# HiLab-git/WSL4MIS

Hardware: AMD Instinct MI355X
Metric: training slices/sec (256x256, bs64, unet_cct pCE+GatedCRF) (higher is better)
Workload: dtype f32; 1 GPU; unet_cct pce_gatedcrf r=5, 256x256x1 4-class synthetic scribble slices, batch 64/GPU, SGD+poly LR; global_batch=64, parallelism=dp1, crf_radius=5, conv_precision=f32

## Files before the change

include/wsl_hip.h:

```cpp
#ifndef WSL_HIP_H
#define WSL_HIP_H
#include <stddef.h>
#include <stdint.h>

#ifdef __cplusplus
extern "C" {
#endif

#define WSL_OK 0
#define WSL_EINVAL (-1)
#define WSL_EUNSUPPORTED (-2)
#define WSL_EHIP (-3)
#define WSL_EWORKSPACE (-4)

#define WSL_LEAKY_SLOPE 0.01f

int wsl_version(void);
const char* wsl_last_error(void);
const char* wsl_build_info(void);

#define WSL_PROF_FAMILIES 20
typedef struct WslProfRow {
  char name[48];
  int64_t calls;
  double ms, flops, bytes;
  double issued_flops;
} WslProfRow;
int wsl_prof_enable(int on);
int wsl_prof_report(WslProfRow* rows, int max_rows);

typedef struct WslSrc {
  const float* x;
  int64_t bs;
  int32_t C;
  int32_t _pad0;
  const float* scale;
  const float* shift;
  const uint8_t* emask;
  float emask_scale;
  float _pad1;
  const float* cmask;
} WslSrc;

int wsl_conv2d_fwd(const WslSrc* a, const WslSrc* b, const float* w, const float* bias, float* y, int64_t y_bs,
                   int N, int H, int W, int Co, int ks, int wmode, float* stat_part, float* stat_cnt, void* stream);
int wsl_conv2d_stat_blocks(int N, int H, int W, int Ci, int Co, int ks);
int wsl_conv2d_pack_weights(const float* w, float* packed, int Co, int Ci, int ks, int wmode_raw, void* stream);
int wsl_conv2d_fast_ok(const WslSrc* a, const WslSrc* b, const float* y, int64_t y_bs, int W);
int wsl_conv2d_wino_ok(int N, int H, int W, int Ca, int Cb, int Co, int ks);
int wsl_net_concurrent(int on);

int wsl_conv2d_wgrad(const WslSrc* a, const WslSrc* b, const float* dy, int64_t dy_bs, float* dw, float* db,
                     int N, int H, int W, int Co, int ks, void* ws, size_t ws_bytes, void* stream);
size_t wsl_conv2d_wgrad_ws_bytes(int N, int H, int W, int Ci, int Co, int ks);
typedef struct WslWgradPending {
  const float* part_dw;
  const float* part_db;
  float* dw;
  float* db;
  int Co, Ci, KK, nsplit;
} WslWgradPending;
int wsl_conv2d_wgrad_partial(const WslSrc* a, const WslSrc* b, const float* dy, int64_t dy_bs, float* dw, float* db, int N, int H,
                             int W, int Co, int ks, void* ws, size_t ws_bytes, WslWgradPending* pending, void* stream);
int wsl_wgrad_reduce_batch(const WslWgradPending* items, int n, void* stream);

int wsl_bn_stats_finalize(const float* stat_part, const float* stat_cnt, int nblk, int C, const float* gamma,
                          const float* beta, float eps, float momentum, float* running_mean, float* running_var,
                          int64_t* num_batches_tracked, float* mean, float* invstd, float* scale, float* shift,
                          void* stream);
int wsl_bn_eval_affine(const float* gamma, const float* beta, const float* running_mean, const float* running_var,
                       float eps, int C, float* scale, float* shift, void* stream);
int wsl_src_materialize(const WslSrc* s, float* out, int64_t out_bs, int N, int H, int W, void* stream);
int wsl_pool2_fwd(const WslSrc* s, float* out, int N, int H, int W, void* stream);

int wsl_feat_grad_combine(const WslSrc* f, const float* ga, int64_t ga_bs, const float* gb, int64_t gb_bs,
                          const float* gb_cmask, const float* gp, float* g, int N, int H, int W, void* stream);

int wsl_bnact_bwd(const float* g, int64_t g_bs, const float* y, const float* mean, const float* invstd,
                  const float* gamma, const float* beta, const uint8_t* emask, float emask_scale, float* dy,
                  float* dgamma, float* dbeta, int N, int C, int H, int W, void* ws, size_t ws_bytes, void* stream);
size_t wsl_bnact_bwd_ws_bytes(int N, int C, int H, int W);

int wsl_conv2d_dgrad_bn(const WslSrc* dy, const float* w, float* g, int64_t g_bs, int N, int H, int W, int Co, int ks,
                        int wmode, const float* bn_y, const float* bn_st, const uint8_t* bn_emask, float bn_emask_scale,
                        float* bn_part, int* fused, void* stream);
int wsl_feat_grad_combine_blocks(int N, int H, int W);
int wsl_feat_grad_combine_bn(const WslSrc* f, const float* ga, int64_t ga_bs, const float* gb, int64_t gb_bs,
                             const float* gb_cmask, const float* gp, float* g, int N, int H, int W, const float* bn_mean,
                             const float* bn_invstd, float* bn_part, void* stream);
int wsl_bnact_bwd_finish(const float* g, int64_t g_bs, const float* y, const float* mean, const float* invstd,
                         const float* gamma, const float* beta, const uint8_t* emask, float emask_scale, float* dy,
                         float* dgamma, float* dbeta, int N, int C, int H, int W, const float* part, int nblk,
                         int channel_major, void* ws, size_t ws_bytes, void* stream);
int wsl_conv2d_dgrad_bn_d(const WslSrc* dy, const float* w, float* g, int64_t g_bs, int N, int H, int W, int Co, int ks,
                          int wmode, const float* bn_y, const float* bn_st, const uint8_t* bn_emask, float bn_emask_scale,
                          float* bn_part, int* fused, void* stream);
int wsl_bnact_bwd_finish_d_amax(const float* dz, int64_t dz_bs, const float* y, const float* mean, const float* invstd,
                                const float* gamma, const float* beta, float* dy, float* dgamma, float* dbeta, int N, int C, int H,
                                int W, const float* part, int nblk, int channel_major, void* ws, size_t ws_bytes, uint32_t* dy_amax,
                                void* stream);

#define WSL_SP_ACT_EXP 4
#define WSL_SP_AMAX_SLOTS 64
int wsl_sp_conv2d_ok(const WslSrc* a, const WslSrc* b, const float* y, int64_t y_bs, int N, int H, int W, int Co, int ks);
size_t wsl_sp_weight_image_bytes(int Co, int Ci);
int wsl_sp_pack_weights(const float* w, void* image, uint32_t* w_amax, int Co, int Ci, int dgrad, void* stream);
int wsl_sp_conv2d_fwd(const WslSrc* a, const WslSrc* b, const void* image, const uint32_t* w_amax, const uint32_t* in_amax,
                      const float* bias, float* y, int64_t y_bs, int N, int H, int W, int Co, float* stat_part, float* stat_cnt,
                      void* stream);
int wsl_sp_conv2d_stat_blocks(int N, int H, int W, int Ci, int Co);
int wsl_sp_conv2d_dgrad_bn(const WslSrc* dy, const uint32_t* dy_amax, const void* image, const uint32_t* w_amax, float* g,
                           int64_t g_bs, int N, int H, int W, int Co, const float* bn_y, const float* bn_st,
                           const uint8_t* bn_emask, float bn_emask_scale, float* bn_part, int* fused, void* stream);
size_t wsl_sp_conv2d_wgrad_ws_bytes(int N, int H, int W, int Ci, int Co);
int wsl_sp_conv2d_wgrad_partial(const WslSrc* a, const WslSrc* b, const float* dy, int64_t dy_bs, const uint32_t* dy_amax,
                                float* dw, float* db, int N, int H, int W, int Co, void* ws, size_t ws_bytes,
                                WslWgradPending* pending, void* stream);
size_t wsl_bilinear_up2_fwd_amax_ws_bytes(int N, int C, int h, int w);
int wsl_bilinear_up2_fwd_amax(const float* u, float* out, int64_t out_bs, int N, int C, int h, int w, void* ws, size_t ws_bytes,
                              uint32_t* amax_slots, void* stream);
int wsl_sp_conv2d_wgrad_partial_amax(const WslSrc* a, const WslSrc* b, const float* dy, int64_t dy_bs, const uint32_t* dy_amax,
                                     const uint32_t* in_amax, float* dw, float* db, int N, int H, int W, int Co, void* ws,
                                     size_t ws_bytes, WslWgradPending* pending, void* stream);
size_t wsl_bnact_bwd_finish_ws_bytes(int N, int C, int H, int W, int with_amax);
int wsl_bnact_bwd_amax(const float* g, int64_t g_bs, const float* y, const float* mean, const float* invstd, const float* gamma,
                       const float* beta, const uint8_t* emask, float emask_scale, float* dy, float* dgamma, float* dbeta, int N,
                       int C, int H, int W, void* ws, size_t ws_bytes, uint32_t* dy_amax, void* stream);
int wsl_bnact_bwd_finish_amax(const float* g, int64_t g_bs, const float* y, const float* mean, const float* invstd,
                              const float* gamma, const float* beta, const uint8_t* emask, float emask_scale, float* dy,
                              float* dgamma, float* dbeta, int N, int C, int H, int W, const float* part, int nblk,
                              int channel_major, void* ws, size_t ws_bytes, uint32_t* dy_amax, void* stream);

int wsl_bilinear_up2_fwd(const float* u, float* out, int64_t out_bs, int N, int C, int h, int w, void* stream);
int wsl_bilinear_up2_bwd(const float* dout, int64_t dout_bs, float* du, int N, int C, int h, int w, void* stream);

int wsl_softmax_fwd(const float* z, float* s, int N, int C, int HW, void* stream);
int wsl_softmax_bwd(const float* s, const float* ds, float* dz, int N, int C, int HW, void* stream);

int wsl_ce_fwd_bwd(const float* z, const void* label, int label_i64, int ignore, float* loss, float* dz, float gscale,
                   int N, int C, int HW, void* ws, size_t ws_bytes, void* stream);
int wsl_mix_argmax(const float* s1, const float* s2, double beta, int64_t* pseudo, int N, int C, int HW, void* stream);
int wsl_pdice_fwd(const float* s, const void* target, int target_i64, int ignore, float* loss, float* sums, int N,
                  int C, int HW, void* ws, size_t ws_bytes, void* stream);
int wsl_pdice_bwd(const float* s, const void* target, int target_i64, int ignore, const float* sums,
                  const float* gout , float* ds, int N, int C, int HW, void* stream);

int wsl_head_fwd_bwd(const float* z1, const float* z2, const uint8_t* label, int ignore, double beta, float w_pse,
                     float gscale, float* out, int64_t* pseudo, float* dz1, float* dz2, int N, int C, int HW,
                     void* ws, size_t ws_bytes, void* stream);
size_t wsl_loss_ws_bytes(int N, int C, int HW);
int wsl_head_gatedcrf_fwd_bwd(const float* z1, const float* z2, const uint8_t* label, int ignore, double beta, const float* img,
                              int radius, float sigma_xy, float sigma_rgb, float weight, float crf_weight, float* out,
                              float* dz1, float* dz2, float* y, float* msg, int N, int C, int H, int W, void* ws,
                              size_t ws_bytes, void* stream);

int wsl_mixprob_fwd(const float* z1, const float* z2, double beta, float* y, int N, int C, int HW, void* stream);
int wsl_mixprob_bwd(const float* z1, const float* z2, double beta, const float* dy, float k, float* dz1, float* dz2,
                    int accumulate, int N, int C, int HW, void* stream);

int wsl_gatedcrf_fwd(const float* y, const float* img, float* msg, float* loss, int N, int C, int H, int W, int radius,
                     float sigma_xy, float sigma_rgb, float weight, void* ws, size_t ws_bytes, void* stream);
int wsl_gatedcrf_bwd(const float* msg, const float* gout, float gscale, float* dy, int N, int C, int H, int W,
                     void* stream);
#define WSL_REG_TV 1
#define WSL_REG_MS 2
#define WSL_REG_ENTROPY 3
#define WSL_REG_CLASS_VAR 4
int wsl_head_reg_fwd_bwd(const float* z, const uint8_t* label, int ignore, float w_ce, int reg_kind, float reg_weight,
                         const float* img, const float* zt, float cons_weight, float* out, float* dz, float* s, float* ds, int N,
                         int C, int H, int W, void* ws, size_t ws_bytes, void* stream);
int wsl_tv_fwd_bwd(const float* p, int n0, float* loss, float* dp, float gscale, int N, int C, int H, int W, void* ws,
                   size_t ws_bytes, void* stream);
int wsl_mumford_shah_fwd_bwd(const float* img, const float* p, float* loss, float* dp, float gscale, int N, int C, int H,
                             int W, void* ws, size_t ws_bytes, void* stream);
int wsl_class_variance_fwd_bwd(const float* img, const float* p, float* loss ,
                               float* dp, float w_inter, float w_intra, int N, int C, int H, int W,
                               void* ws, size_t ws_bytes, void* stream);
int wsl_softmax_mse_fwd_bwd(const float* a, const float* b, float* loss, float* da, float gscale, int N, int C, int HW,
                            void* ws, size_t ws_bytes, void* stream);

int wsl_rot90(const float* x, float* y, int planes, int H, int W, int k, void* stream);
int wsl_softmax_accum(const float* z, float* acc, float scale, int init, int N, int C, int HW, void* stream);
int wsl_ustm_consistency_fwd_bwd(const float* a, const float* b, const float* pmean, float threshold, float* loss, float* da,
                                 float gscale, int N, int C, int HW, void* ws, size_t ws_bytes, void* stream);
int wsl_entropy_fwd_bwd(const float* p, float* loss, float* dp, float gscale, int N, int C, int HW, int norm_classes,
                        void* ws, size_t ws_bytes, void* stream);
int wsl_axpy(float* dst, const float* src, float k, int64_t n, void* stream);

int wsl_sup_head_fwd_bwd(const float* z, const uint8_t* label, int ignore, float w_ce, float w_dice, float gscale, float* out,
                         float* dz, int N, int C, int HW, void* ws, size_t ws_bytes, void* stream);
int wsl_entropy_logits_fwd_bwd(const float* z, float* loss, float* dz, float gscale, int N, int C, int HW, int norm_classes,
                               void* ws, size_t ws_bytes, void* stream);

int wsl_sgd_step(float* p, const float* grad, float* buf, int64_t n, float lr, float momentum, float wd, int first,
                 float grad_scale, float* ema, float ema_alpha, void* stream);

typedef struct {
  const float* img;
  const uint8_t* lab;
  int h, w;
  int op, k, axis;
  int lab_cval;
  float img_cval;
  double m00, m01, m10, m11, off0, off1;
} WslAugSample;
int wsl_augment_batch(const WslAugSample* samples, int n, float* out_img, uint8_t* out_lab, int Ho, int Wo, void* stream);

size_t wsl_s2l_head_ws_bytes(int N, int C, int HW);
int wsl_s2l_head_fwd_bwd(const float* z, const uint8_t* scribble, const float* weight, int ignore, float thr_conf, float w_u,
                         float gscale, float* out, uint8_t* u_labels, float* dz, int N, int C, int HW, void* ws, size_t ws_bytes,
                         void* stream);
typedef struct WslS2lSlot {
  float* weight;
  int h, w;
} WslS2lSlot;
int wsl_s2l_ensemble_update(const float* z, const WslS2lSlot* slots, int n, int C, int Hn, int Wn, double alpha, void* stream);
typedef struct {
  const float* img;
  const uint8_t* mask;
  const uint8_t* scr;
  const float* weight;
  int h, w;
  int op, k, axis;
  int _pad;
  double m00, m01, m10, m11, off0, off1;
} WslAugSampleS2l;
int wsl_augment_batch_s2l(const WslAugSampleS2l* samples, int n, int C, float* out_img, uint8_t* out_mask, uint8_t* out_scr,
                          float* out_weight, int Ho, int Wo, void* stream);

size_t wsl_random_walker_ws_bytes(int N, int H, int W, int n_class);
int wsl_random_walker(const float* img, const uint8_t* seed, uint8_t* label_out, float* prob_out, int* iters_out, float* resid_out,
                      int N, int H, int W, int n_class, float beta, float tol, int max_iter, void* ws, size_t ws_bytes, void* stream);

int wsl_surface_u8(const uint8_t* vol, uint8_t* border, int D, int H, int W, void* stream);
int wsl_nearest_dist2(const int64_t* a_zyx, int na, const int64_t* b_zyx, int nb, int64_t* out, void* stream);

int wsl_nearest_dist2_sp(const int64_t* a_zyx, int na, const int64_t* b_zyx, int nb, double sz, double sy, double sx, double* out,
                         void* stream);

int wsl_noisy_copy(const float* x, const float* noise, float* out, int64_t n, int reps, float sigma, float clip, uint64_t seed,
                   void* stream);

int wsl_draw_masks(int n_masks, void* const* outs, const int64_t* numels, const float* keep_probs, const float* scales,
                   const int* is_f32, uint64_t seed, void* stream);

typedef struct WslNetDesc {
  int32_t in_chns, n_class;
  int32_t n_dec;
  int32_t N, H, W;
  int32_t precision;
  int32_t _pad;
} WslNetDesc;

typedef struct WslNetEntry {
  char name[96];
  int32_t kind;
  int32_t ndim;
  int64_t shape[4];
  int64_t offset;
} WslNetEntry;

int wsl_net_num_entries(const WslNetDesc* d);
int wsl_net_entry(const WslNetDesc* d, int i, WslNetEntry* out);
int64_t wsl_net_param_count(const WslNetDesc* d);
int64_t wsl_net_encoder_param_count(const WslNetDesc* d);
int64_t wsl_net_buffer_count(const WslNetDesc* d);
size_t wsl_net_ws_bytes(const WslNetDesc* d);

int wsl_net_forward(const WslNetDesc* d, const float* params, float* buffers, int64_t* nbt, const float* x,
                    const uint8_t* const* emasks, const float* const* cmasks, int training, float* logits_main,
                    float* logits_aux, void* ws, size_t ws_bytes, void* stream);
int wsl_net_backward(const WslNetDesc* d, const float* params, const float* x, const uint8_t* const* emasks,
                     const float* const* cmasks, const float* dlogits_main, const float* dlogits_aux, float* grads,
                     void* ws, size_t ws_bytes, int phase, void* stream);

int wsl_conv2d_dil_fwd(const WslSrc* a, const WslSrc* b, const float* w, const float* bias, float* y, int64_t y_bs, int N, int H,
                       int W, int Co, int ks, int dil, int wmode, float* stat_part, float* stat_cnt, void* stream);
int wsl_conv2d_dil_stat_blocks(int N, int H, int W, int Ci, int Co, int dil);
int wsl_conv2d_dil_wgrad(const WslSrc* a, const WslSrc* b, const float* dy, int64_t dy_bs, float* dw, float* db, int N, int H, int W,
                         int Co, int ks, int dil, void* ws, size_t ws_bytes, void* stream);
size_t wsl_conv2d_dil_wgrad_ws_bytes(int N, int H, int W, int Ci, int Co, int ks, int dil);
int wsl_conv2d_dil_wgrad_partial(const WslSrc* a, const WslSrc* b, const float* dy, int64_t dy_bs, float* dw, float* db, int N, int H,
                                 int W, int Co, int ks, int dil, void* ws, size_t ws_bytes, WslWgradPending* pending, void* stream);

typedef struct WslPNetDesc {
// ... 69 lines not shown
```

wsl4mis_amd/_lib.py:

```python
import ctypes as C
import os

import torch

_HERE = os.path.dirname(os.path.abspath(__file__))
LIB_PATH = os.path.join(_HERE, "csrc", "libwslhip.so")

c_fp = C.c_void_p


class WslSrc(C.Structure):
    _fields_ = [("x", c_fp), ("bs", C.c_int64), ("C", C.c_int32), ("_pad0", C.c_int32), ("scale", c_fp),
                ("shift", c_fp), ("emask", c_fp), ("emask_scale", C.c_float), ("_pad1", C.c_float), ("cmask", c_fp)]


WSL_PROF_FAMILIES = 20


class WslProfRow(C.Structure):
    _fields_ = [("name", C.c_char * 48), ("calls", C.c_int64), ("ms", C.c_double), ("flops", C.c_double),
                ("bytes", C.c_double), ("issued_flops", C.c_double)]


class WslNetDesc(C.Structure):
    _fields_ = [("in_chns", C.c_int32), ("n_class", C.c_int32), ("n_dec", C.c_int32), ("N", C.c_int32),
                ("H", C.c_int32), ("W", C.c_int32), ("precision", C.c_int32), ("_pad", C.c_int32)]


class WslWgradPending(C.Structure):
    _fields_ = [("part_dw", c_fp), ("part_db", c_fp), ("dw", c_fp), ("db", c_fp), ("Co", C.c_int32), ("Ci", C.c_int32),
                ("KK", C.c_int32), ("nsplit", C.c_int32)]


class WslUpBlockDesc(C.Structure):
    _fields_ = [("C1", C.c_int32), ("C2", C.c_int32), ("Co", C.c_int32), ("N", C.c_int32), ("h", C.c_int32), ("w", C.c_int32),
                ("dropout_p", C.c_float)]


class WslPNetDesc(C.Structure):
    _fields_ = [("in_chns", C.c_int32), ("n_class", C.c_int32), ("num_filters", C.c_int32), ("ratios", C.c_int32 * 5),
                ("N", C.c_int32), ("H", C.c_int32), ("W", C.c_int32)]


class WslDanDesc(C.Structure):
    _fields_ = [("num_classes", C.c_int32), ("n_channel", C.c_int32), ("ndf", C.c_int32), ("pool", C.c_int32),
                ("N", C.c_int32), ("H", C.c_int32), ("W", C.c_int32), ("_pad", C.c_int32)]


class WslNetEntry(C.Structure):
    _fields_ = [("name", C.c_char * 96), ("kind", C.c_int32), ("ndim", C.c_int32), ("shape", C.c_int64 * 4),
                ("offset", C.c_int64)]


class WslAugSample(C.Structure):
    _fields_ = [("img", c_fp), ("lab", c_fp), ("h", C.c_int32), ("w", C.c_int32), ("op", C.c_int32), ("k", C.c_int32),
                ("axis", C.c_int32), ("lab_cval", C.c_int32), ("img_cval", C.c_float), ("m00", C.c_double),
                ("m01", C.c_double), ("m10", C.c_double), ("m11", C.c_double), ("off0", C.c_double), ("off1", C.c_double)]


class WslS2lSlot(C.Structure):
    _fields_ = [("weight", c_fp), ("h", C.c_int32), ("w", C.c_int32)]


class WslAugSampleS2l(C.Structure):
    _fields_ = [("img", c_fp), ("mask", c_fp), ("scr", c_fp), ("weight", c_fp), ("h", C.c_int32), ("w", C.c_int32),
                ("op", C.c_int32), ("k", C.c_int32), ("axis", C.c_int32), ("_pad", C.c_int32), ("m00", C.c_double),
                ("m01", C.c_double), ("m10", C.c_double), ("m11", C.c_double), ("off0", C.c_double), ("off1", C.c_double)]


i32, i64, f32, f64, sz = C.c_int, C.c_int64, C.c_float, C.c_double, C.c_size_t
PS, PD, PE = C.POINTER(WslSrc), C.POINTER(WslNetDesc), C.POINTER(WslNetEntry)
PP = C.POINTER(c_fp)
PQ = C.POINTER(WslPNetDesc)
PDAN = C.POINTER(WslDanDesc)

_PROTOS = {
    "wsl_version": (i32, []),
    "wsl_last_error": (C.c_char_p, []),
    "wsl_build_info": (C.c_char_p, []),
    "wsl_prof_enable": (i32, [i32]),
    "wsl_prof_report": (i32, [C.POINTER(WslProfRow), i32]),
    "wsl_net_concurrent": (i32, [i32]),
    "wsl_conv2d_fwd": (i32, [PS, PS, c_fp, c_fp, c_fp, i64, i32, i32, i32, i32, i32, i32, c_fp, c_fp, c_fp]),
    "wsl_conv2d_stat_blocks": (i32, [i32, i32, i32, i32, i32, i32]),
    "wsl_conv2d_pack_weights": (i32, [c_fp, c_fp, i32, i32, i32, i32, c_fp]),
    "wsl_conv2d_fast_ok": (i32, [PS, PS, c_fp, i64, i32]),
    "wsl_conv2d_wino_ok": (i32, [i32, i32, i32, i32, i32, i32, i32]),
    "wsl_conv2d_wgrad": (i32, [PS, PS, c_fp, i64, c_fp, c_fp, i32, i32, i32, i32, i32, c_fp, sz, c_fp]),
    "wsl_conv2d_wgrad_ws_bytes": (sz, [i32, i32, i32, i32, i32, i32]),
    "wsl_conv2d_wgrad_partial": (i32, [PS, PS, c_fp, i64, c_fp, c_fp, i32, i32, i32, i32, i32, c_fp, sz,
                                       C.POINTER(WslWgradPending), c_fp]),
    "wsl_wgrad_reduce_batch": (i32, [C.POINTER(WslWgradPending), i32, c_fp]),
    "wsl_bn_stats_finalize": (i32, [c_fp, c_fp, i32, i32, c_fp, c_fp, f32, f32, c_fp, c_fp, c_fp, c_fp, c_fp, c_fp,
                                    c_fp, c_fp]),
    "wsl_bn_eval_affine": (i32, [c_fp, c_fp, c_fp, c_fp, f32, i32, c_fp, c_fp, c_fp]),
    "wsl_src_materialize": (i32, [PS, c_fp, i64, i32, i32, i32, c_fp]),
    "wsl_pool2_fwd": (i32, [PS, c_fp, i32, i32, i32, c_fp]),
    "wsl_feat_grad_combine": (i32, [PS, c_fp, i64, c_fp, i64, c_fp, c_fp, c_fp, i32, i32, i32, c_fp]),
    "wsl_bnact_bwd": (i32, [c_fp, i64, c_fp, c_fp, c_fp, c_fp, c_fp, c_fp, f32, c_fp, c_fp, c_fp, i32, i32, i32, i32,
                            c_fp, sz, c_fp]),
    "wsl_bnact_bwd_ws_bytes": (sz, [i32, i32, i32, i32]),
    "wsl_conv2d_dgrad_bn": (i32, [PS, c_fp, c_fp, i64, i32, i32, i32, i32, i32, i32, c_fp, c_fp, c_fp, f32, c_fp, C.POINTER(C.c_int), c_fp]),
    "wsl_conv2d_dgrad_bn_d": (i32, [PS, c_fp, c_fp, i64, i32, i32, i32, i32, i32, i32, c_fp, c_fp, c_fp, f32, c_fp, C.POINTER(C.c_int), c_fp]),
    "wsl_bnact_bwd_finish_d_amax": (i32, [c_fp, i64, c_fp, c_fp, c_fp, c_fp, c_fp, c_fp, c_fp, c_fp, i32, i32, i32, i32,
                                          c_fp, i32, i32, c_fp, sz, c_fp, c_fp]),
    "wsl_feat_grad_combine_blocks": (i32, [i32, i32, i32]),
    "wsl_feat_grad_combine_bn": (i32, [PS, c_fp, i64, c_fp, i64, c_fp, c_fp, c_fp, i32, i32, i32, c_fp, c_fp, c_fp, c_fp]),
    "wsl_bnact_bwd_finish": (i32, [c_fp, i64, c_fp, c_fp, c_fp, c_fp, c_fp, c_fp, f32, c_fp, c_fp, c_fp, i32, i32, i32, i32,
                                   c_fp, i32, i32, c_fp, sz, c_fp]),
    "wsl_sp_conv2d_ok": (i32, [PS, PS, c_fp, i64, i32, i32, i32, i32, i32]),
    "wsl_sp_weight_image_bytes": (sz, [i32, i32]),
    "wsl_sp_pack_weights": (i32, [c_fp, c_fp, c_fp, i32, i32, i32, c_fp]),
    "wsl_sp_conv2d_fwd": (i32, [PS, PS, c_fp, c_fp, c_fp, c_fp, c_fp, i64, i32, i32, i32, i32, c_fp, c_fp, c_fp]),
    "wsl_sp_conv2d_stat_blocks": (i32, [i32, i32, i32, i32, i32]),
    "wsl_sp_conv2d_dgrad_bn": (i32, [PS, c_fp, c_fp, c_fp, c_fp, i64, i32, i32, i32, i32, c_fp, c_fp, c_fp, f32, c_fp,
                                     C.POINTER(C.c_int), c_fp]),
    "wsl_sp_conv2d_wgrad_ws_bytes": (sz, [i32, i32, i32, i32, i32]),
    "wsl_sp_conv2d_wgrad_partial": (i32, [PS, PS, c_fp, i64, c_fp, c_fp, c_fp, i32, i32, i32, i32, c_fp, sz,
                                          C.POINTER(WslWgradPending), c_fp]),
    "wsl_sp_conv2d_wgrad_partial_amax": (i32, [PS, PS, c_fp, i64, c_fp, c_fp, c_fp, c_fp, i32, i32, i32, i32, c_fp, sz,
                                               C.POINTER(WslWgradPending), c_fp]),
    "wsl_bilinear_up2_fwd_amax_ws_bytes": (sz, [i32, i32, i32, i32]),
    "wsl_bilinear_up2_fwd_amax": (i32, [c_fp, c_fp, i64, i32, i32, i32, i32, c_fp, sz, c_fp, c_fp]),
    "wsl_bnact_bwd_finish_ws_bytes": (sz, [i32, i32, i32, i32, i32]),
    "wsl_bnact_bwd_amax": (i32, [c_fp, i64, c_fp, c_fp, c_fp, c_fp, c_fp, c_fp, f32, c_fp, c_fp, c_fp, i32, i32, i32, i32,
                                 c_fp, sz, c_fp, c_fp]),
    "wsl_bnact_bwd_finish_amax": (i32, [c_fp, i64, c_fp, c_fp, c_fp, c_fp, c_fp, c_fp, f32, c_fp, c_fp, c_fp, i32, i32, i32, i32,
                                        c_fp, i32, i32, c_fp, sz, c_fp, c_fp]),
    "wsl_bilinear_up2_fwd": (i32, [c_fp, c_fp, i64, i32, i32, i32, i32, c_fp]),
    "wsl_bilinear_up2_bwd": (i32, [c_fp, i64, c_fp, i32, i32, i32, i32, c_fp]),
    "wsl_softmax_fwd": (i32, [c_fp, c_fp, i32, i32, i32, c_fp]),
    "wsl_softmax_bwd": (i32, [c_fp, c_fp, c_fp, i32, i32, i32, c_fp]),
    "wsl_ce_fwd_bwd": (i32, [c_fp, c_fp, i32, i32, c_fp, c_fp, f32, i32, i32, i32, c_fp, sz, c_fp]),
    "wsl_mix_argmax": (i32, [c_fp, c_fp, f64, c_fp, i32, i32, i32, c_fp]),
    "wsl_pdice_fwd": (i32, [c_fp, c_fp, i32, i32, c_fp, c_fp, i32, i32, i32, c_fp, sz, c_fp]),
    "wsl_pdice_bwd": (i32, [c_fp, c_fp, i32, i32, c_fp, c_fp, c_fp, i32, i32, i32, c_fp]),
    "wsl_head_fwd_bwd": (i32, [c_fp, c_fp, c_fp, i32, f64, f32, f32, c_fp, c_fp, c_fp, c_fp, i32, i32, i32, c_fp, sz,
                               c_fp]),
    "wsl_loss_ws_bytes": (sz, [i32, i32, i32]),
    "wsl_mixprob_fwd": (i32, [c_fp, c_fp, f64, c_fp, i32, i32, i32, c_fp]),
    "wsl_mixprob_bwd": (i32, [c_fp, c_fp, f64, c_fp, f32, c_fp, c_fp, i32, i32, i32, i32, c_fp]),
    "wsl_gatedcrf_fwd": (i32, [c_fp, c_fp, c_fp, c_fp, i32, i32, i32, i32, i32, f32, f32, f32, c_fp, sz, c_fp]),
    "wsl_gatedcrf_bwd": (i32, [c_fp, c_fp, f32, c_fp, i32, i32, i32, i32, c_fp]),
    "wsl_head_reg_fwd_bwd": (i32, [c_fp, c_fp, i32, f32, i32, f32, c_fp, c_fp, f32, c_fp, c_fp, c_fp, c_fp, i32, i32, i32, i32, c_fp, sz, c_fp]),
    "wsl_tv_fwd_bwd": (i32, [c_fp, i32, c_fp, c_fp, f32, i32, i32, i32, i32, c_fp, sz, c_fp]),
    "wsl_mumford_shah_fwd_bwd": (i32, [c_fp, c_fp, c_fp, c_fp, f32, i32, i32, i32, i32, c_fp, sz, c_fp]),
    "wsl_class_variance_fwd_bwd": (i32, [c_fp, c_fp, c_fp, c_fp, f32, f32, i32, i32, i32, i32, c_fp, sz, c_fp]),
    "wsl_softmax_mse_fwd_bwd": (i32, [c_fp, c_fp, c_fp, c_fp, f32, i32, i32, i32, c_fp, sz, c_fp]),
    "wsl_rot90": (i32, [c_fp, c_fp, i32, i32, i32, i32, c_fp]),
    "wsl_softmax_accum": (i32, [c_fp, c_fp, f32, i32, i32, i32, i32, c_fp]),
    "wsl_ustm_consistency_fwd_bwd": (i32, [c_fp, c_fp, c_fp, f32, c_fp, c_fp, f32, i32, i32, i32, c_fp, sz, c_fp]),
    "wsl_entropy_fwd_bwd": (i32, [c_fp, c_fp, c_fp, f32, i32, i32, i32, i32, c_fp, sz, c_fp]),
    "wsl_axpy": (i32, [c_fp, c_fp, f32, i64, c_fp]),
    "wsl_sup_head_fwd_bwd": (i32, [c_fp, c_fp, i32, f32, f32, f32, c_fp, c_fp, i32, i32, i32, c_fp, sz, c_fp]),
    "wsl_entropy_logits_fwd_bwd": (i32, [c_fp, c_fp, c_fp, f32, i32, i32, i32, i32, c_fp, sz, c_fp]),
    "wsl_sgd_step": (i32, [c_fp, c_fp, c_fp, i64, f32, f32, f32, i32, f32, c_fp, f32, c_fp]),
    "wsl_surface_u8": (i32, [c_fp, c_fp, i32, i32, i32, c_fp]),
    "wsl_nearest_dist2": (i32, [c_fp, i32, c_fp, i32, c_fp, c_fp]),
    "wsl_nearest_dist2_sp": (i32, [c_fp, i32, c_fp, i32, f64, f64, f64, c_fp, c_fp]),
    "wsl_augment_batch": (i32, [C.POINTER(WslAugSample), i32, c_fp, c_fp, i32, i32, c_fp]),
    "wsl_s2l_head_ws_bytes": (sz, [i32, i32, i32]),
    "wsl_s2l_head_fwd_bwd": (i32, [c_fp, c_fp, c_fp, i32, f32, f32, f32, c_fp, c_fp, c_fp, i32, i32, i32, c_fp, sz, c_fp]),
    "wsl_s2l_ensemble_update": (i32, [c_fp, C.POINTER(WslS2lSlot), i32, i32, i32, i32, f64, c_fp]),
    "wsl_augment_batch_s2l": (i32, [C.POINTER(WslAugSampleS2l), i32, i32, c_fp, c_fp, c_fp, c_fp, i32, i32, c_fp]),
    "wsl_random_walker_ws_bytes": (sz, [i32, i32, i32, i32]),
    "wsl_random_walker": (i32, [c_fp, c_fp, c_fp, c_fp, c_fp, c_fp, i32, i32, i32, i32, f32, f32, i32, c_fp, sz, c_fp]),
    "wsl_noisy_copy": (i32, [c_fp, c_fp, c_fp, i64, i32, f32, f32, C.c_uint64, c_fp]),
    "wsl_head_gatedcrf_fwd_bwd": (i32, [c_fp, c_fp, c_fp, i32, f64, c_fp, i32, f32, f32, f32, f32, c_fp, c_fp, c_fp, c_fp, c_fp,
                                        i32, i32, i32, i32, c_fp, sz, c_fp]),
    "wsl_draw_masks": (i32, [i32, PP, C.POINTER(C.c_int64), C.POINTER(C.c_float), C.POINTER(C.c_float),
                             C.POINTER(C.c_int), C.c_uint64, c_fp]),
    "wsl_convt2x2_fwd": (i32, [c_fp, c_fp, c_fp, c_fp, i32, i32, i32, i32, i32, c_fp]),
    "wsl_convt2x2_dgrad": (i32, [c_fp, i64, c_fp, c_fp, i32, i32, i32, i32, i32, c_fp]),
    "wsl_convt2x2_wgrad_ws_bytes": (sz, [i32, i32, i32]),
    "wsl_convt2x2_wgrad": (i32, [c_fp, c_fp, i64, c_fp, c_fp, i32, i32, i32, i32, i32, c_fp, sz, c_fp]),
    "wsl_upblock_t_param_count": (i64, [C.POINTER(WslUpBlockDesc)]),
    "wsl_upblock_t_ws_bytes": (sz, [C.POINTER(WslUpBlockDesc)]),
    "wsl_upblock_t_forward": (i32, [C.POINTER(WslUpBlockDesc), c_fp, c_fp, c_fp, c_fp, c_fp, c_fp, i32, c_fp, c_fp, sz, c_fp]),
    "wsl_upblock_t_backward": (i32, [C.POINTER(WslUpBlockDesc), c_fp, c_fp, c_fp, c_fp, c_fp, c_fp, c_fp, c_fp, c_fp, sz, c_fp]),
    "wsl_conv2d_dil_fwd": (i32, [PS, PS, c_fp, c_fp, c_fp, i64, i32, i32, i32, i32, i32, i32, i32, c_fp, c_fp, c_fp]),
    "wsl_conv2d_dil_stat_blocks": (i32, [i32, i32, i32, i32, i32, i32]),
    "wsl_conv2d_dil_wgrad": (i32, [PS, PS, c_fp, i64, c_fp, c_fp, i32, i32, i32, i32, i32, i32, c_fp, sz, c_fp]),
    "wsl_conv2d_dil_wgrad_ws_bytes": (sz, [i32, i32, i32, i32, i32, i32, i32]),
    "wsl_conv2d_dil_wgrad_partial": (i32, [PS, PS, c_fp, i64, c_fp, c_fp, i32, i32, i32, i32, i32, i32, c_fp, sz,
                                           C.POINTER(WslWgradPending), c_fp]),
    "wsl_pnet_num_entries": (i32, [PQ]),
    "wsl_pnet_entry": (i32, [PQ, i32, PE]),
    "wsl_pnet_param_count": (i64, [PQ]),
    "wsl_pnet_block_param_count": (i64, [PQ]),
    "wsl_pnet_buffer_count": (i64, [PQ]),
    "wsl_pnet_ws_bytes": (sz, [PQ]),
    "wsl_pnet_forward": (i32, [PQ, c_fp, c_fp, c_fp, c_fp, PP, i32, c_fp, c_fp, sz, c_fp]),
    "wsl_pnet_backward": (i32, [PQ, c_fp, c_fp, PP, c_fp, c_fp, c_fp, sz, i32, c_fp]),
    "wsl_conv4s2_fwd": (i32, [c_fp, i32, c_fp, i32, i32, c_fp, c_fp, c_fp, c_fp, c_fp, c_fp, i32, i32, i32, i32, c_fp]),
    "wsl_conv4s2_dgrad": (i32, [c_fp, c_fp, c_fp, c_fp, c_fp, i32, i32, i32, i32, i32, c_fp]),
    "wsl_conv4s2_wgrad_ws_bytes": (sz, [i32, i32, i32, i32, i32]),
    "wsl_conv4s2_wgrad": (i32, [c_fp, i32, c_fp, c_fp, c_fp, c_fp, c_fp, c_fp, i32, i32, i32, i32, i32, c_fp, sz, c_fp]),
    "wsl_dan_head_ws_bytes": (sz, [i32, i32]),
    "wsl_dan_head_fwd_bwd": (i32, [c_fp, c_fp, c_fp, c_fp, i32, f32, c_fp, c_fp, c_fp, c_fp, c_fp, i32, i32, i32, i32, c_fp, sz, c_fp]),
    "wsl_adam_step": (i32, [c_fp, c_fp, c_fp, c_fp, i64, f32, f32, f32, f32, i32, f32, c_fp]),
    "wsl_dan_num_entries": (i32, [PDAN]),
    "wsl_dan_entry": (i32, [PDAN, i32, PE]),
    "wsl_dan_param_count": (i64, [PDAN]),
    "wsl_dan_buffer_count": (i64, [PDAN]),
    "wsl_dan_ws_bytes": (sz, [PDAN]),
    "wsl_dan_forward": (i32, [PDAN, c_fp, c_fp, c_fp, PP, i32, c_fp, f32, c_fp, c_fp, c_fp, sz, c_fp]),
    "wsl_dan_backward": (i32, [PDAN, c_fp, c_fp, c_fp, PP, c_fp, i32, c_fp, c_fp, c_fp, sz, c_fp]),
    "wsl_net_num_entries": (i32, [PD]),
    "wsl_net_entry": (i32, [PD, i32, PE]),
    "wsl_net_param_count": (i64, [PD]),
    "wsl_net_encoder_param_count": (i64, [PD]),
    "wsl_net_buffer_count": (i64, [PD]),
    "wsl_net_ws_bytes": (sz, [PD]),
    "wsl_net_forward": (i32, [PD, c_fp, c_fp, c_fp, c_fp, PP, PP, i32, c_fp, c_fp, c_fp, sz, c_fp]),
    "wsl_net_backward": (i32, [PD, c_fp, c_fp, PP, PP, c_fp, c_fp, c_fp, c_fp, sz, i32, c_fp]),
}


_DEBUG_PROTOS = {
    "wsl_debug_conv_plan": (i32, [i32, i32, i32]),
    "wsl_debug_conv_wino": (i32, [i32]),
    "wsl_debug_wgrad_workgroups": (i32, [i32]),
    "wsl_debug_net_decisions": (i32, [PD, c_fp, sz, i32, i32, c_fp, c_fp]),
    "wsl_debug_mfma4_probe": (i32, [c_fp, c_fp, c_fp, c_fp]),
    "wsl_debug_lds_dma_probe": (i32, [c_fp, c_fp, c_fp]),
    "wsl_debug_pk_probe": (i32, [c_fp, c_fp, c_fp]),
    "wsl_debug_mfma_stream": (i32, [i32, i32, i32, c_fp, c_fp]),
}


class WslError(RuntimeError):
    pass


def bind(cdll, strict=True):
    missing = []
    for name, (res, args) in _PROTOS.items():
        try:
            fn = getattr(cdll, name)
        except AttributeError:
            missing.append(name)
            continue
        fn.restype, fn.argtypes = res, args
    for name, (res, args) in _DEBUG_PROTOS.items():
        if hasattr(cdll, name):
            fn = getattr(cdll, name)
            fn.restype, fn.argtypes = res, args
    if missing and strict:
        raise WslError(f"library lacks symbols declared in include/wsl_hip.h: {missing}")
    return missing


_lib = None


def lib():
    global _lib
    if _lib is None:
        if not os.path.exists(LIB_PATH):
            raise WslError(f"{LIB_PATH} not found: run wsl4mis_amd/csrc/build.sh (hipcc, gfx950). "
                           "There is no CPU fallback.")
        cdll = C.CDLL(LIB_PATH)
        bind(cdll, strict=os.path.abspath(LIB_PATH) == os.path.join(_HERE, "csrc", "libwslhip.so"))
        if b"HOST-EMULATION" in cdll.wsl_build_info():
            raise WslError("refusing to use a host-emulation build as the product library")
        _lib = cdll
    return _lib


_test_emul = False


def use_library_for_tests(cdll):
    global _lib, _test_emul
    bind(cdll, strict=False)
    if b"HOST-EMULATION" not in cdll.wsl_build_info():
        raise WslError("use_library_for_tests expects the emulation build")
    _lib, _test_emul = cdll, True


def _reset_for_tests():
    global _lib, _test_emul
    _lib, _test_emul = None, False


def is_test_emulation():
    return _test_emul


def check(rc, cdll=None):
    if rc != 0:
        l = cdll or lib()
        raise WslError(f"wsl error {rc}: {l.wsl_last_error().decode()}")


def source_sha256():
    import hashlib
    cs = os.path.join(_HERE, "csrc")
    names = sorted(f for f in os.listdir(cs) if f.endswith((".hip", ".h")))
    h = hashlib.sha256()
    for f in [os.path.join(cs, n) for n in names] + [os.path.join(os.path.dirname(_HERE), "include", "wsl_hip.h")]:
        with open(f, "rb") as fh:
            h.update(fh.read())
    return h.hexdigest()


def library_sha256(cdll=None):
    info = (cdll or lib()).wsl_build_info().decode()
    return info.rsplit("sha256:", 1)[1].strip() if "sha256:" in info else None


def declared_symbols():
    return list(_PROTOS)
```

wsl4mis_amd/csrc/wsl_bn.hip:

```cpp
#include <stdlib.h>

#include "wsl_rt.h"

namespace wsl {

constexpr int kChunk = 4096;

constexpr int kFinalizeWideFrom = 2048;
static inline int finalize_threads(int nblk) { return nblk >= kFinalizeWideFrom ? 1024 : kThreads; }
template <int NV>
__device__ __forceinline__ void finalize_merge_waves(double (&v)[NV], double* red) {
  const int nw = blockDim.x >> 6, w = threadIdx.x >> 6;
#pragma unroll
  for (int m = 32; m >= 1; m >>= 1)
#pragma unroll
    for (int k = 0; k < NV; ++k) v[k] += __shfl_xor(v[k], m);
  if ((threadIdx.x & 63) == 0)
#pragma unroll
    for (int k = 0; k < NV; ++k) red[k * 16 + w] = v[k];
  __syncthreads();
#pragma unroll
  for (int k = 0; k < NV; ++k) {
    double t[16];
#pragma unroll
// ... 216 lines not shown
    float* dst = bn_part + (((int64_t)n * gridDim.x + blockIdx.x) * f.C + c) * 2;
    dst[0] = s1;
    dst[1] = s2;
  }
}

struct BnBwdP {
  const float* g;
  int64_t g_bs;
  const float* y;
  const float* mean;
  const float* invstd;
  const float* gamma;
  const float* beta;
  const uint8_t* emask;
  float es;
  int C, HW, chunks;
  int g_is_d = 0;
};

__device__ __forceinline__ float bn_dz(const BnBwdP& p, int n, int c, int i, float sc, float sh, float mean, float invstd,
                                       float* xhat) {
  const int64_t idx = ((int64_t)n * p.C + c) * p.HW + i;
  const float yv = p.y[idx];
  float d = p.g[n * p.g_bs + (int64_t)c * p.HW + i];
  *xhat = (yv - mean) * invstd;
  if (p.g_is_d) return d;
  if (p.emask) d = p.emask[idx] ? d * p.es : 0.f;
  const float z = fmaf(yv, sc, sh);
  return z > 0.f ? d : WSL_LEAKY_SLOPE * d;
}

__global__ __launch_bounds__(256) void bnact_bwd_reduce_kernel(BnBwdP p, float* part) {
  __shared__ float red[8];
  const int c = blockIdx.y, n = blockIdx.z;
  const float mean = p.mean[c], invstd = p.invstd[c];
  const float sc = p.gamma[c] * invstd, sh = fmaf(-mean, sc, p.beta[c]);
  float s1 = 0.f, s2 = 0.f;
  const int base = blockIdx.x * kChunk;
  for (int i = base + threadIdx.x; i < base + kChunk && i < p.HW; i += kThreads) {
    float xh;
    const float d = bn_dz(p, n, c, i, sc, sh, mean, invstd, &xh);
    s1 += d;
    s2 = fmaf(d, xh, s2);
  }
  s1 = block_sum(s1, red);
  s2 = block_sum(s2, red + 4);
  if (threadIdx.x == 0) {
    float* dst = part + (((int64_t)n * p.chunks + blockIdx.x) * p.C + c) * 2;
    dst[0] = s1;
    dst[1] = s2;
  }
}

__device__ __forceinline__ void bn_dz4(const BnBwdP& p, int n, int c, int i, float sc, float sh, float mean, float invstd,
                                       float (&d)[4], float (&xh)[4]) {
  const int64_t idx = ((int64_t)n * p.C + c) * p.HW + i;
  const float4 yv = *reinterpret_cast<const float4*>(p.y + idx);
  const float4 gv = *reinterpret_cast<const float4*>(p.g + n * p.g_bs + (int64_t)c * p.HW + i);
  const float y4[4] = {yv.x, yv.y, yv.z, yv.w};
  float g4[4] = {gv.x, gv.y, gv.z, gv.w};
  if (p.g_is_d) {
#pragma unroll
    for (int k = 0; k < 4; ++k) xh[k] = (y4[k] - mean) * invstd, d[k] = g4[k];
    return;
  }
  if (p.emask) {
    const uint32_t m = *reinterpret_cast<const uint32_t*>(p.emask + idx);
#pragma unroll
    for (int k = 0; k < 4; ++k) g4[k] = ((m >> (8 * k)) & 0xffu) ? g4[k] * p.es : 0.f;
  }
#pragma unroll
  for (int k = 0; k < 4; ++k) {
    const float z = fmaf(y4[k], sc, sh);
    xh[k] = (y4[k] - mean) * invstd;
    d[k] = z > 0.f ? g4[k] : WSL_LEAKY_SLOPE * g4[k];
  }
}

__global__ __launch_bounds__(256) void bnact_bwd_reduce4_kernel(BnBwdP p, float* part) {
  __shared__ float red[8];
  const int c = blockIdx.y, n = blockIdx.z;
  const float mean = p.mean[c], invstd = p.invstd[c];
  const float sc = p.gamma[c] * invstd, sh = fmaf(-mean, sc, p.beta[c]);
  float s1 = 0.f, s2 = 0.f;
  const int base = blockIdx.x * kChunk;
  for (int i = base + 4 * threadIdx.x; i < base + kChunk && i < p.HW; i += 4 * kThreads) {
    float d[4], xh[4];
    bn_dz4(p, n, c, i, sc, sh, mean, invstd, d, xh);
#pragma unroll
    for (int k = 0; k < 4; ++k) {
      s1 += d[k];
      s2 = fmaf(d[k], xh[k], s2);
    }
  }
  s1 = block_sum(s1, red);
  s2 = block_sum(s2, red + 4);
  if (threadIdx.x == 0) {
    float* dst = part + (((int64_t)n * p.chunks + blockIdx.x) * p.C + c) * 2;
    dst[0] = s1;
    dst[1] = s2;
  }
}

__device__ __forceinline__ void amax_block_store(float m, uint32_t* pmax) {
  __shared__ float mred[4];
#pragma unroll
  for (int k = 32; k >= 1; k >>= 1) m = fmaxf(m, __shfl_xor(m, k));
  if ((threadIdx.x & 63) == 0) mred[threadIdx.x >> 6] = m;
  __syncthreads();
  if (threadIdx.x == 0) {
    m = fmaxf(fmaxf(mred[0], mred[1]), fmaxf(mred[2], mred[3]));
    uint32_t u;
    memcpy(&u, &m, 4);
    pmax[((int64_t)blockIdx.z * gridDim.y + blockIdx.y) * gridDim.x + blockIdx.x] = u;
  }
}
__global__ __launch_bounds__(256) void amax_fold_kernel(const uint32_t* pmax, int n, uint32_t* slots) {
  __shared__ uint32_t ured[4];
  uint32_t u = 0u;
  for (int i = blockIdx.x + WSL_SP_AMAX_SLOTS * threadIdx.x; i < n; i += WSL_SP_AMAX_SLOTS * kThreads) {
    const uint32_t v = pmax[i];
    u = v > u ? v : u;
  }
#pragma unroll
  for (int k = 32; k >= 1; k >>= 1) {
    const uint32_t o = (uint32_t)__shfl_xor((int)u, k);
    u = o > u ? o : u;
  }
  if ((threadIdx.x & 63) == 0) ured[threadIdx.x >> 6] = u;
  __syncthreads();
  if (threadIdx.x == 0) {
    const uint32_t a = ured[0] > ured[1] ? ured[0] : ured[1], b = ured[2] > ured[3] ? ured[2] : ured[3];
    slots[blockIdx.x] = a > b ? a : b;
  }
}

__global__ __launch_bounds__(256) void bnact_bwd_apply4_kernel(BnBwdP p, const float* coef, float* dy, uint32_t* pmax) {
  const int c = blockIdx.y, n = blockIdx.z;
  const float mean = p.mean[c], invstd = p.invstd[c];
  const float sc = p.gamma[c] * invstd, sh = fmaf(-mean, sc, p.beta[c]);
  const float c1 = coef[2 * c], c2 = coef[2 * c + 1];
  const int base = blockIdx.x * kChunk;
  float m = 0.f;
  for (int i = base + 4 * threadIdx.x; i < base + kChunk && i < p.HW; i += 4 * kThreads) {
    float d[4], xh[4];
    bn_dz4(p, n, c, i, sc, sh, mean, invstd, d, xh);
    const float4 v = make_float4(sc * (d[0] - c1 - xh[0] * c2), sc * (d[1] - c1 - xh[1] * c2), sc * (d[2] - c1 - xh[2] * c2),
                                 sc * (d[3] - c1 - xh[3] * c2));
    *reinterpret_cast<float4*>(dy + ((int64_t)n * p.C + c) * p.HW + i) = v;
    if (pmax) m = fmaxf(fmaxf(m, fmaxf(fabsf(v.x), fabsf(v.y))), fmaxf(fabsf(v.z), fabsf(v.w)));
  }
  if (pmax) amax_block_store(m, pmax);
}

__global__ __launch_bounds__(1024) void bnact_bwd_finalize_kernel(const float* part, int nblk, int C, int64_t sb, int64_t sc,
                                                                  double count, float* dgamma, float* dbeta, float* coef) {
  __shared__ double red[2 * 16];
  const int c = blockIdx.x;
  double acc[2] = {0, 0};
#pragma unroll 8
  for (int b = threadIdx.x; b < nblk; b += blockDim.x) {
    const float2 v = *reinterpret_cast<const float2*>(part + ((int64_t)b * sb + (int64_t)c * sc) * 2);
    acc[0] += v.x;
    acc[1] += v.y;
  }
  finalize_merge_waves<2>(acc, red);
  const double s1 = acc[0], s2 = acc[1];
  if (threadIdx.x == 0) {
    if (dbeta) dbeta[c] = (float)s1;
    if (dgamma) dgamma[c] = (float)s2;
    coef[2 * c] = (float)(s1 / count);
    coef[2 * c + 1] = (float)(s2 / count);
  }
}

__global__ __launch_bounds__(256) void bnact_bwd_apply_kernel(BnBwdP p, const float* coef, float* dy, uint32_t* pmax) {
  const int c = blockIdx.y, n = blockIdx.z;
  const float mean = p.mean[c], invstd = p.invstd[c];
  const float sc = p.gamma[c] * invstd, sh = fmaf(-mean, sc, p.beta[c]);
  const float c1 = coef[2 * c], c2 = coef[2 * c + 1];
  const int base = blockIdx.x * kChunk;
  float m = 0.f;
  for (int i = base + threadIdx.x; i < base + kChunk && i < p.HW; i += kThreads) {
    float xh;
    const float d = bn_dz(p, n, c, i, sc, sh, mean, invstd, &xh);
    const float v = sc * (d - c1 - xh * c2);
    dy[((int64_t)n * p.C + c) * p.HW + i] = v;
    m = fmaxf(m, fabsf(v));
  }
  if (pmax) amax_block_store(m, pmax);
}

__device__ __forceinline__ void lerp_coord(int dst, float scale, int in, int* i0, int* i1, float* l) {
  const float src = scale * (float)dst;
  int a = (int)src;
  if (a > in - 1) a = in - 1;
  *i0 = a;
  *i1 = a + (a < in - 1 ? 1 : 0);
  *l = src - (float)a;
}

__global__ __launch_bounds__(256) void bilinear_up2_fwd_kernel(const float* u, float* out, int64_t out_bs, int C, int h,
                                                               int w) {
  const int c = blockIdx.y, n = blockIdx.z, Ho = 2 * h, Wo = 2 * w;
  const float sy = Ho > 1 ? (float)(h - 1) / (float)(Ho - 1) : 0.f, sx = Wo > 1 ? (float)(w - 1) / (float)(Wo - 1) : 0.f;
  const float* src = u + ((int64_t)n * C + c) * h * w;
  const int base = blockIdx.x * kChunk;
  for (int o = base + threadIdx.x; o < base + kChunk && o < Ho * Wo; o += kThreads) {
    const int oy = o / Wo, ox = o - oy * Wo;
    int y0, y1, x0, x1;
    float ly, lx;
    lerp_coord(oy, sy, h, &y0, &y1, &ly);
    lerp_coord(ox, sx, w, &x0, &x1, &lx);
    const float top = (1.f - lx) * src[y0 * w + x0] + lx * src[y0 * w + x1];
    const float bot = (1.f - lx) * src[y1 * w + x0] + lx * src[y1 * w + x1];
    out[n * out_bs + (int64_t)c * Ho * Wo + o] = (1.f - ly) * top + ly * bot;
  }
}

__global__ __launch_bounds__(256) void bilinear_up2_bwd_kernel(const float* dout, int64_t dout_bs, float* du, int C,
                                                               int h, int w) {
  const int c = blockIdx.y, n = blockIdx.z, Ho = 2 * h, Wo = 2 * w;
  const float sy = Ho > 1 ? (float)(h - 1) / (float)(Ho - 1) : 0.f, sx = Wo > 1 ? (float)(w - 1) / (float)(Wo - 1) : 0.f;
  const float* g = dout + n * dout_bs + (int64_t)c * Ho * Wo;
  const int base = blockIdx.x * kChunk;
  for (int e = base + threadIdx.x; e < base + kChunk && e < h * w; e += kThreads) {
    const int i = e / w, j = e - i * w;
    float wy[5], wx[5];
#pragma unroll
    for (int k = 0; k < 5; ++k) {
      const int Y = 2 * i - 2 + k, X = 2 * j - 2 + k;
      wy[k] = 0.f, wx[k] = 0.f;
      if (Y >= 0 && Y < Ho) {
        int a, b;
        float l;
        lerp_coord(Y, sy, h, &a, &b, &l);
        wy[k] = (a == i ? 1.f - l : 0.f) + (b == i ? l : 0.f);
      }
      if (X >= 0 && X < Wo) {
        int a, b;
        float l;
        lerp_coord(X, sx, w, &a, &b, &l);
        wx[k] = (a == j ? 1.f - l : 0.f) + (b == j ? l : 0.f);
      }
    }
    float acc = 0.f;
#pragma unroll
    for (int ky = 0; ky < 5; ++ky) {
      if (wy[ky] != 0.f) {
        const int Y = 2 * i - 2 + ky;
        float row = 0.f;
#pragma unroll
        for (int kx = 0; kx < 5; ++kx)
          if (wx[kx] != 0.f) row = fmaf(wx[kx], g[(int64_t)Y * Wo + 2 * j - 2 + kx], row);
        acc = fmaf(wy[ky], row, acc);
      }
    }
    du[((int64_t)n * C + c) * h * w + e] = acc;
  }
}

__global__ __launch_bounds__(256) void bilinear_up2_fwdc_kernel(const float* u, float* out, int64_t out_bs, int C, int h,
                                                                int w, int lw, int rows_per_wg) {
  const int c = blockIdx.y, n = blockIdx.z, Ho = 2 * h, Wo = 2 * w;
  const float sy = Ho > 1 ? (float)(h - 1) / (float)(Ho - 1) : 0.f, sx = Wo > 1 ? (float)(w - 1) / (float)(Wo - 1) : 0.f;
  const float* src = u + ((int64_t)n * C + c) * h * w;
  float* dst = out + n * out_bs + (int64_t)c * Ho * Wo;
  const int ox = threadIdx.x & (Wo - 1), r0 = threadIdx.x >> lw, rgroups = kThreads >> lw;
  int x0, x1;
  float lx;
  lerp_coord(ox, sx, w, &x0, &x1, &lx);
  const int per = (rows_per_wg + rgroups - 1) / rgroups;
  const int base = blockIdx.x * rows_per_wg + r0 * per;
  int end = base + per;
  if (end > blockIdx.x * rows_per_wg + rows_per_wg) end = blockIdx.x * rows_per_wg + rows_per_wg;
  if (end > Ho) end = Ho;
  int ya = -1, yb = -1;
  float ha = 0.f, hb = 0.f;
  for (int oy = base; oy < end; ++oy) {
    int y0, y1;
    float ly;
    lerp_coord(oy, sy, h, &y0, &y1, &ly);
    float top, bot;
    if (y0 == ya) top = ha;
    else if (y0 == yb) top = hb;
    else {
      const float* s0 = src + y0 * w;
      top = (1.f - lx) * s0[x0] + lx * s0[x1];
    }
    if (y1 == y0) bot = top;
    else if (y1 == yb) bot = hb;
    else if (y1 == ya) bot = ha;
    else {
      const float* s1 = src + y1 * w;
      bot = (1.f - lx) * s1[x0] + lx * s1[x1];
    }
    ya = y0, ha = top, yb = y1, hb = bot;
    dst[(int64_t)oy * Wo + ox] = (1.f - ly) * top + ly * bot;
  }
}

constexpr int kUpFR = 32;
__global__ __launch_bounds__(256) void bilinear_up2_fwd4_kernel(const float* u, float* out, int64_t out_bs, int C, int h, int w,
                                                                int lq, uint32_t* pmax) {
  __shared__ __attribute__((aligned(16))) float st[(kUpFR / 2 + 3) * 128];
// ... 130 lines not shown
  int l = 0;
  while ((1 << l) < v) ++l;
  return l;
}

}

using namespace wsl;

extern "C" int wsl_bn_stats_finalize(const float* stat_part, const float* stat_cnt, int nblk, int C, const float* gamma,
                                     const float* beta, float eps, float momentum, float* running_mean,
                                     float* running_var, int64_t* nbt, float* mean, float* invstd, float* scale,
                                     float* shift, void* stream) {
  WSL_REQUIRE(stat_part && stat_cnt && gamma && beta && mean && invstd && scale && shift, "bn_stats_finalize: null");
  WSL_REQUIRE(nblk > 0 && C > 0, "bn_stats_finalize: bad sizes");
  ProfScope ps(PF_BN_FINALIZE, 0.0, 4.0 * (3.0 * nblk * C + 8.0 * C), stream);
  WSL_LAUNCH(bn_finalize_kernel, dim3(C), dim3(finalize_threads(nblk)), 0, stream, stat_part, stat_cnt, nblk, C, gamma, beta, eps,
             momentum, running_mean, running_var, nbt, mean, invstd, scale, shift);
  return check_launch("bn_finalize_kernel");
}

extern "C" int wsl_bn_eval_affine(const float* gamma, const float* beta, const float* running_mean,
                                  const float* running_var, float eps, int C, float* scale, float* shift, void* stream) {
  WSL_REQUIRE(gamma && beta && running_mean && running_var && scale && shift && C > 0, "bn_eval_affine: bad args");
  WSL_LAUNCH(bn_eval_affine_kernel, dim3(cdiv(C, 256)), dim3(256), 0, stream, gamma, beta, running_mean, running_var,
             eps, C, scale, shift);
  return check_launch("bn_eval_affine_kernel");
}

extern "C" int wsl_src_materialize(const WslSrc* s, float* out, int64_t out_bs, int N, int H, int W, void* stream) {
  WSL_REQUIRE(s && s->x && out && N > 0 && H > 0 && W > 0 && s->C > 0, "src_materialize: bad args");
  WSL_LAUNCH(src_materialize_kernel, dim3(cdiv(H * W, kChunk), s->C, N), dim3(kThreads), 0, stream, *s, out, out_bs,
             H * W);
  return check_launch("src_materialize_kernel");
}

extern "C" int wsl_pool2_fwd(const WslSrc* s, float* out, int N, int H, int W, void* stream) {
  WSL_REQUIRE(s && s->x && out && N > 0 && H > 1 && W > 1 && s->C > 0, "pool2_fwd: bad args");
  ProfScope ps(PF_POOL_FANIN, 0.0, 5.0 * (double)N * s->C * H * W, stream);
  WSL_LAUNCH(pool2_fwd_kernel, dim3(cdiv((H / 2) * (W / 2), kChunk), s->C, N), dim3(kThreads), 0, stream, *s, out, H, W);
  return check_launch("pool2_fwd_kernel");
}

extern "C" int wsl_feat_grad_combine(const WslSrc* f, const float* ga, int64_t ga_bs, const float* gb, int64_t gb_bs,
                                     const float* gb_cmask, const float* gp, float* g, int N, int H, int W, void* stream) {
  WSL_REQUIRE(f && g && N > 0 && H > 0 && W > 0 && f->C > 0, "feat_grad_combine: bad args");
  WSL_REQUIRE(!gp || f->x, "feat_grad_combine: pool routing needs the feature map");
  ProfScope ps(PF_POOL_FANIN, 0.0, (double)N * f->C * H * W * (4.0 * (ga ? 1 : 0) + 4.0 * (gb ? 1 : 0) + (gp ? 5.0 : 0.0) + 4.0), stream);
  WSL_LAUNCH(feat_grad_combine_kernel, dim3(cdiv(((H + 1) / 2) * ((W + 1) / 2), kChunk), f->C, N), dim3(kThreads), 0,
             stream, *f, ga, ga_bs, gb, gb_bs, gb_cmask, gp, g, H, W);
  return check_launch("feat_grad_combine_kernel");
}

extern "C" size_t wsl_bnact_bwd_ws_bytes(int N, int C, int H, int W) {
  if (N <= 0 || C <= 0 || H <= 0 || W <= 0) return 0;
  return sizeof(float) * ((size_t)N * cdiv(H * W, 256) * C * 2 + 2 * (size_t)C);
}

extern "C" int wsl_bnact_bwd_amax(const float* g, int64_t g_bs, const float* y, const float* mean, const float* invstd,
                                  const float* gamma, const float* beta, const uint8_t* emask, float emask_scale, float* dy,
                                  float* dgamma, float* dbeta, int N, int C, int H, int W, void* ws, size_t ws_bytes,
                                  uint32_t* dy_amax, void* stream) {
  WSL_REQUIRE(g && y && mean && invstd && gamma && beta && dy && ws, "bnact_bwd: null argument");
  WSL_REQUIRE(N > 0 && C > 0 && H > 0 && W > 0, "bnact_bwd: bad shape");
  if (ws_bytes < wsl_bnact_bwd_ws_bytes(N, C, H, W)) {
    set_error("bnact_bwd: workspace %zu < %zu", ws_bytes, wsl_bnact_bwd_ws_bytes(N, C, H, W));
    return WSL_EWORKSPACE;
  }
  BnBwdP p{g, g_bs, y, mean, invstd, gamma, beta, emask, emask_scale, C, H * W, cdiv(H * W, kChunk)};
  ProfScope ps(PF_BN_BWD, 0.0, (double)N * C * H * W * (20.0 + (emask ? 2.0 : 0.0)), stream);
  float* part = static_cast<float*>(ws);
  float* coef = part + (size_t)N * p.chunks * C * 2;
  dim3 grid(p.chunks, C, N);
  auto al16 = [](const void* q) { return (reinterpret_cast<uintptr_t>(q) & 15) == 0; };
  static const bool vec_on = (WSL_TUNE("WSL_BN_VEC", 1) != 0);
  const bool vec = vec_on && (H * W) % 4 == 0 && (g_bs % 4) == 0 && al16(g) && al16(y) && al16(dy) &&
                   (!emask || (reinterpret_cast<uintptr_t>(emask) & 3) == 0);
  if (vec) WSL_LAUNCH(bnact_bwd_reduce4_kernel, grid, dim3(kThreads), 0, stream, p, part);
  else WSL_LAUNCH(bnact_bwd_reduce_kernel, grid, dim3(kThreads), 0, stream, p, part);
  WSL_LAUNCH(bnact_bwd_finalize_kernel, dim3(C), dim3(finalize_threads(N * p.chunks)), 0, stream, part, N * p.chunks, C, (int64_t)C, (int64_t)1,
             (double)N * H * W, dgamma, dbeta, coef);
  uint32_t* pmax = dy_amax ? reinterpret_cast<uint32_t*>(part) : nullptr;
  if (vec) WSL_LAUNCH(bnact_bwd_apply4_kernel, grid, dim3(kThreads), 0, stream, p, coef, dy, pmax);
  else WSL_LAUNCH(bnact_bwd_apply_kernel, grid, dim3(kThreads), 0, stream, p, coef, dy, pmax);
  if (dy_amax) WSL_LAUNCH(amax_fold_kernel, dim3(WSL_SP_AMAX_SLOTS), dim3(kThreads), 0, stream, pmax, N * p.chunks * C, dy_amax);
  return check_launch("bnact_bwd");
}

extern "C" int wsl_bnact_bwd(const float* g, int64_t g_bs, const float* y, const float* mean, const float* invstd,
                             const float* gamma, const float* beta, const uint8_t* emask, float emask_scale, float* dy,
                             float* dgamma, float* dbeta, int N, int C, int H, int W, void* ws, size_t ws_bytes,
                             void* stream) {
  return wsl_bnact_bwd_amax(g, g_bs, y, mean, invstd, gamma, beta, emask, emask_scale, dy, dgamma, dbeta, N, C, H, W, ws, ws_bytes,
                            nullptr, stream);
}

extern "C" size_t wsl_bnact_bwd_finish_ws_bytes(int N, int C, int H, int W, int with_amax) {
  if (N <= 0 || C <= 0 || H <= 0 || W <= 0) return 0;
  return sizeof(float) * (2 * (size_t)C + (with_amax ? (size_t)N * cdiv(H * W, kChunk) * C : 0));
}

static int bnact_bwd_finish_impl(const float* g, int64_t g_bs, const float* y, const float* mean, const float* invstd,
                                 const float* gamma, const float* beta, const uint8_t* emask, float emask_scale, float* dy,
                                 float* dgamma, float* dbeta, int N, int C, int H, int W, const float* part, int nblk,
                                 int channel_major, void* ws, size_t ws_bytes, uint32_t* dy_amax, int g_is_d, void* stream) {
  WSL_REQUIRE(g && y && mean && invstd && gamma && beta && dy && ws && part, "bnact_bwd_finish: null argument");
  WSL_REQUIRE(N > 0 && C > 0 && H > 0 && W > 0 && nblk > 0, "bnact_bwd_finish: bad shape");
  if (ws_bytes < wsl_bnact_bwd_finish_ws_bytes(N, C, H, W, dy_amax != nullptr)) {
    set_error("bnact_bwd_finish: workspace %zu < %zu", ws_bytes, wsl_bnact_bwd_finish_ws_bytes(N, C, H, W, dy_amax != nullptr));
    return WSL_EWORKSPACE;
  }
  BnBwdP p{g, g_bs, y, mean, invstd, gamma, beta, emask, emask_scale, C, H * W, cdiv(H * W, kChunk)};
  p.g_is_d = g_is_d;
  ProfScope ps(PF_BN_BWD, 0.0, (double)N * C * H * W * (12.0 + (emask && !g_is_d ? 1.0 : 0.0)), stream);
  float* coef = static_cast<float*>(ws);
  dim3 grid(p.chunks, C, N);
  auto al16 = [](const void* q) { return (reinterpret_cast<uintptr_t>(q) & 15) == 0; };
  const bool vec = (H * W) % 4 == 0 && (g_bs % 4) == 0 && al16(g) && al16(y) && al16(dy) &&
                   (!emask || (reinterpret_cast<uintptr_t>(emask) & 3) == 0);
  WSL_LAUNCH(bnact_bwd_finalize_kernel, dim3(C), dim3(finalize_threads(nblk)), 0, stream, part, nblk, C,
             channel_major ? (int64_t)1 : (int64_t)C, channel_major ? (int64_t)nblk : (int64_t)1, (double)N * H * W, dgamma, dbeta,
             coef);
  uint32_t* pmax = dy_amax ? reinterpret_cast<uint32_t*>(coef + 2 * (size_t)C) : nullptr;
  if (vec) WSL_LAUNCH(bnact_bwd_apply4_kernel, grid, dim3(kThreads), 0, stream, p, coef, dy, pmax);
  else WSL_LAUNCH(bnact_bwd_apply_kernel, grid, dim3(kThreads), 0, stream, p, coef, dy, pmax);
  if (dy_amax) WSL_LAUNCH(amax_fold_kernel, dim3(WSL_SP_AMAX_SLOTS), dim3(kThreads), 0, stream, pmax, N * p.chunks * C, dy_amax);
  return check_launch("bnact_bwd_finish");
}

extern "C" int wsl_bnact_bwd_finish_amax(const float* g, int64_t g_bs, const float* y, const float* mean, const float* invstd,
                                         const float* gamma, const float* beta, const uint8_t* emask, float emask_scale, float* dy,
                                         float* dgamma, float* dbeta, int N, int C, int H, int W, const float* part, int nblk,
                                         int channel_major, void* ws, size_t ws_bytes, uint32_t* dy_amax, void* stream) {
  return bnact_bwd_finish_impl(g, g_bs, y, mean, invstd, gamma, beta, emask, emask_scale, dy, dgamma, dbeta, N, C, H, W, part, nblk,
                               channel_major, ws, ws_bytes, dy_amax, 0, stream);
}

extern "C" int wsl_bnact_bwd_finish_d_amax(const float* d, int64_t d_bs, const float* y, const float* mean, const float* invstd,
                                           const float* gamma, const float* beta, float* dy, float* dgamma, float* dbeta, int N, int C,
                                           int H, int W, const float* part, int nblk, int channel_major, void* ws, size_t ws_bytes,
                                           uint32_t* dy_amax, void* stream) {
  return bnact_bwd_finish_impl(d, d_bs, y, mean, invstd, gamma, beta, nullptr, 1.f, dy, dgamma, dbeta, N, C, H, W, part, nblk,
                               channel_major, ws, ws_bytes, dy_amax, 1, stream);
}

extern "C" int wsl_bnact_bwd_finish(const float* g, int64_t g_bs, const float* y, const float* mean, const float* invstd,
                                    const float* gamma, const float* beta, const uint8_t* emask, float emask_scale, float* dy,
                                    float* dgamma, float* dbeta, int N, int C, int H, int W, const float* part, int nblk,
                                    int channel_major, void* ws, size_t ws_bytes, void* stream) {
  return wsl_bnact_bwd_finish_amax(g, g_bs, y, mean, invstd, gamma, beta, emask, emask_scale, dy, dgamma, dbeta, N, C, H, W, part,
                                   nblk, channel_major, ws, ws_bytes, nullptr, stream);
}

extern "C" int wsl_feat_grad_combine_blocks(int N, int H, int W) {
  return N > 0 && H > 0 && W > 0 ? N * cdiv(((H + 1) / 2) * ((W + 1) / 2), kChunk) : 0;
}

extern "C" int wsl_feat_grad_combine_bn(const WslSrc* f, const float* ga, int64_t ga_bs, const float* gb, int64_t gb_bs,
                                        const float* gb_cmask, const float* gp, float* g, int N, int H, int W,
                                        const float* bn_mean, const float* bn_invstd, float* bn_part, void* stream) {
  WSL_REQUIRE(f && f->x && f->scale && f->shift && !f->emask && !f->cmask && g && N > 0 && H > 0 && W > 0 && f->C > 0,
              "feat_grad_combine_bn: the feature must be a plain BatchNorm + LeakyReLU source");
  WSL_REQUIRE(bn_mean && bn_invstd && bn_part, "feat_grad_combine_bn: null BatchNorm argument");
  ProfScope ps(PF_POOL_FANIN, 0.0, (double)N * f->C * H * W * (4.0 * (ga ? 1 : 0) + 4.0 * (gb ? 1 : 0) + (gp ? 1.0 : 0.0) + 8.0), stream);
  WSL_LAUNCH(feat_grad_combine_bn_kernel, dim3(cdiv(((H + 1) / 2) * ((W + 1) / 2), kChunk), f->C, N), dim3(kThreads), 0,
             stream, *f, ga, ga_bs, gb, gb_bs, gb_cmask, gp, g, H, W, bn_mean, bn_invstd, bn_part);
  return check_launch("feat_grad_combine_bn_kernel");
}

extern "C" size_t wsl_bilinear_up2_fwd_amax_ws_bytes(int N, int C, int h, int w) {
  return N > 0 && C > 0 && h > 0 && w > 0 ? sizeof(uint32_t) * (size_t)N * C * cdiv(2 * h, kUpFR) : 0;
}

extern "C" int wsl_bilinear_up2_fwd_amax(const float* u, float* out, int64_t out_bs, int N, int C, int h, int w, void* ws, size_t ws_bytes,
                                         uint32_t* amax_slots, void* stream) {
  WSL_REQUIRE(u && out && N > 0 && C > 0 && h > 0 && w > 0, "bilinear_up2_fwd: bad args");
  WSL_REQUIRE(out_bs >= (int64_t)C * 4 * h * w, "bilinear_up2_fwd: out batch stride too small");
  if (amax_slots && (!ws || ws_bytes < wsl_bilinear_up2_fwd_amax_ws_bytes(N, C, h, w))) {
    set_error("bilinear_up2_fwd_amax: workspace %zu < %zu", ws ? ws_bytes : (size_t)0, wsl_bilinear_up2_fwd_amax_ws_bytes(N, C, h, w));
    return WSL_EWORKSPACE;
  }
  ProfScope ps(PF_BILINEAR, 0.0, 20.0 * (double)N * C * h * w, stream);
  if (up2_fast_ok(out, out_bs, w) && (reinterpret_cast<uintptr_t>(u) & 15) == 0) {
    const dim3 grid(cdiv(2 * h, kUpFR), C, N);
    uint32_t* pmax = amax_slots ? static_cast<uint32_t*>(ws) : nullptr;
    WSL_LAUNCH(bilinear_up2_fwd4_kernel, grid, dim3(kThreads), 0, stream, u, out, out_bs, C, h, w, ilog2(2 * w) - 2, pmax);
    if (amax_slots) WSL_LAUNCH(amax_fold_kernel, dim3(WSL_SP_AMAX_SLOTS), dim3(kThreads), 0, stream, pmax, (int)(grid.x * grid.y * grid.z), amax_slots);
    return check_launch("bilinear_up2_fwd4_kernel");
  }
  if (amax_slots) {
    WSL_REQUIRE(((int64_t)N * C * h * w) % 4 == 0 && (reinterpret_cast<uintptr_t>(u) & 15) == 0, "bilinear_up2_fwd_amax: source not float4-aligned");
    if (hipMemsetAsync(amax_slots, 0, WSL_SP_AMAX_SLOTS * sizeof(uint32_t), (hipStream_t)stream) != hipSuccess) {
      set_error("bilinear_up2_fwd_amax: clearing the slots failed");
      return WSL_EHIP;
    }
    WSL_LAUNCH(amax_tensor_kernel, dim3(256), dim3(kThreads), 0, stream, u, (int64_t)N * C * h * w / 4, amax_slots);
  }
  if (up2_fast_ok(out, out_bs, w)) {
    const int lw = ilog2(2 * w);
    int rows = 8192 / (2 * w);
    if (rows < (kThreads >> lw)) rows = kThreads >> lw;
    WSL_LAUNCH(bilinear_up2_fwdc_kernel, dim3(cdiv(2 * h, rows), C, N), dim3(kThreads), 0, stream, u, out, out_bs, C, h, w,
               lw, rows);
    return check_launch("bilinear_up2_fwdc_kernel");
  }
  WSL_LAUNCH(bilinear_up2_fwd_kernel, dim3(cdiv(4 * h * w, kChunk), C, N), dim3(kThreads), 0, stream, u, out, out_bs, C,
             h, w);
  return check_launch("bilinear_up2_fwd_kernel");
}

extern "C" int wsl_bilinear_up2_fwd(const float* u, float* out, int64_t out_bs, int N, int C, int h, int w, void* stream) {
  return wsl_bilinear_up2_fwd_amax(u, out, out_bs, N, C, h, w, nullptr, 0, nullptr, stream);
}

extern "C" int wsl_bilinear_up2_bwd(const float* dout, int64_t dout_bs, float* du, int N, int C, int h, int w,
                                    void* stream) {
  WSL_REQUIRE(dout && du && N > 0 && C > 0 && h > 0 && w > 0, "bilinear_up2_bwd: bad args");
  WSL_REQUIRE(dout_bs >= (int64_t)C * 4 * h * w, "bilinear_up2_bwd: dout batch stride too small");
  ProfScope ps(PF_BILINEAR, 0.0, 20.0 * (double)N * C * h * w, stream);
  if (up2_fast_ok(dout, dout_bs, w)) {
    const int ltj = ilog2(w < 64 ? w : 64);
    if (h % 32 == 0) {
      WSL_LAUNCH(bilinear_up2_bwd4_kernel<32>, dim3((w >> ltj) * (h / 32), C, N), dim3(kThreads), 0, stream, dout, dout_bs, du, C, h, w, ltj);
    } else {
      WSL_LAUNCH(bilinear_up2_bwd4_kernel<16>, dim3((w >> ltj) * cdiv(h, 16), C, N), dim3(kThreads), 0, stream, dout, dout_bs, du, C, h, w, ltj);
    }
    return check_launch("bilinear_up2_bwd4_kernel");
  }
  WSL_LAUNCH(bilinear_up2_bwd_kernel, dim3(cdiv(h * w, kChunk), C, N), dim3(kThreads), 0, stream, dout, dout_bs, du, C,
             h, w);
  return check_launch("bilinear_up2_bwd_kernel");
}
```

wsl4mis_amd/csrc/wsl_conv.hip:

```cpp
#include <stdio.h>
#include <stdlib.h>

#include "wsl_rt.h"

namespace wsl {

struct TileSrc {
  WslSrc a, b;
  int H, W, Ci;
};

__device__ __forceinline__ float tile_value(const TileSrc& t, int n, int c, int gy, int gx) {
  if (c >= t.Ci || gy < 0 || gy >= t.H || gx < 0 || gx >= t.W) return 0.f;
  const int64_t hw = (int64_t)t.H * t.W;
  const int64_t off = (int64_t)gy * t.W + gx;
  if (c < t.a.C) return src_value(t.a, n, c, n * t.a.bs + c * hw + off, ((int64_t)n * t.a.C + c) * hw + off);
  c -= t.a.C;
  return src_value(t.b, n, c, n * t.b.bs + c * hw + off, ((int64_t)n * t.b.C + c) * hw + off);
}

struct ConvP {
  TileSrc in;
  const float* w;
  const float* bias;
// ... 361 lines not shown
    constexpr int PER = C::PP * (C::KK + 1) * 4;
    float* mine = red + (wave * 64 + lane) * PER;
#pragma unroll
    for (int j = 0; j < C::PP; ++j) {
#pragma unroll
      for (int t = 0; t < C::KK; ++t)
#pragma unroll
        for (int r = 0; r < 4; ++r) mine[(j * (C::KK + 1) + t) * 4 + r] = acc[j][t][r];
#pragma unroll
      for (int r = 0; r < 4; ++r) mine[(j * (C::KK + 1) + C::KK) * 4 + r] = accb[j][r];
    }
    __syncthreads();
    if (wk == 0) {
#pragma unroll
      for (int j = 0; j < C::PP; ++j) {
#pragma unroll
        for (int t = 0; t <= C::KK; ++t)
#pragma unroll
          for (int r = 0; r < 4; ++r) {
            float s = 0.f;
            for (int k = 0; k < WK; ++k) s += red[((k * C::WP + wp) * 64 + lane) * PER + (j * (C::KK + 1) + t) * 4 + r];
            if (t < C::KK) acc[j][t][r] = s; else accb[j][r] = s;
          }
      }
    }
  }
  if (wk == 0) {
#pragma unroll
    for (int j = 0; j < C::PP; ++j) {
      const int pr = wp * C::PP + j, cot = pr / C::IBT, cit = pr % C::IBT;
      const int ci = ci0 + cit * 16 + (lane & 15);
#pragma unroll
      for (int r = 0; r < 4; ++r) {
        const int co = co0 + cot * 16 + (lane >> 4) * 4 + r;
        if (co < p.Co && ci < Ci) {
#pragma unroll
          for (int t = 0; t < C::KK; ++t)
            p.part_dw[(((int64_t)split * C::KK + t) * p.Co + co) * Ci + ci] = acc[j][t][r];
        }
        if (want_db && cit == 0 && (lane & 15) == 0 && co < p.Co) p.part_db[(int64_t)split * p.Co + co] = accb[j][r];
      }
    }
  }
}

template <int SG>
__global__ __launch_bounds__(256) void wgrad_reduce_kernel(const float* part_dw, const float* part_db, float* dw,
                                                           float* db, int Co, int Ci, int KK, int nsplit) {
  __shared__ float red[kThreads];
  constexpr int EPB = kThreads / SG;
  const int64_t E = (int64_t)KK * Co * Ci;
  const int64_t total = E + (db ? Co : 0);
  const int el = threadIdx.x % EPB, sg = threadIdx.x / EPB;
  const int64_t e = (int64_t)blockIdx.x * EPB + el;
  float s = 0.f;
  if (e < total) {
    const float* src = e < E ? part_dw + e : part_db + (e - E);
    const int64_t stride = e < E ? E : Co;
    for (int k = sg; k < nsplit; k += SG) s += src[k * stride];
  }
  red[threadIdx.x] = s;
  __syncthreads();
  if (sg == 0 && e < total) {
    float t = 0.f;
#pragma unroll
    for (int k = 0; k < SG; ++k) t += red[k * EPB + el];
    if (e < E) {
      const int tap = (int)(e / ((int64_t)Co * Ci));
      const int64_t rem = e - (int64_t)tap * Co * Ci;
      dw[rem * KK + tap] = t;
    } else {
      db[e - E] = t;
    }
  }
}

#ifdef WSL_EXPERIMENTS
static std::atomic<int> g_forced_wgrad_wgs{0};
int forced_wgrad_wgs() { return g_forced_wgrad_wgs.load(); }
#endif
struct WgPlan {
  int th, tw, cb, ib, wk, nsplit, items, tiles_x, tiles_y, co_blocks, ci_blocks;
};
static WgPlan wgrad_plan(int N, int H, int W, int Ci, int Co, bool v2 = false, bool wide = false) {
  WgPlan g;
  const bool small = (Co <= 16 || Ci <= 16);
  if (small) {
    g.cb = g.ib = 16, g.wk = 4;
    if (W >= 64) g.th = v2 ? 4 : 8, g.tw = 64; else if (W >= 32) g.th = v2 ? 4 : 8, g.tw = 32; else g.th = v2 ? 8 : 16, g.tw = 16;
  } else {
    g.cb = g.ib = 32, g.wk = 1;
    if (wide) g.cb = 64;
    if (W >= 32) g.th = v2 ? 4 : 8, g.tw = 32; else g.th = v2 ? 8 : 16, g.tw = 16;
  }
  g.tiles_x = cdiv(W, g.tw), g.tiles_y = cdiv(H, g.th);
  g.items = N * g.tiles_x * g.tiles_y;
  g.co_blocks = cdiv(Co, g.cb), g.ci_blocks = cdiv(Ci, g.ib);
  static const int wgs = WSL_TUNE("WSL_WGRAD_WGS", 768);
  int want = (forced_wgrad_wgs() > 0 ? forced_wgrad_wgs() : wide ? 512 : wgs) / (g.co_blocks * g.ci_blocks);
  if (want < 1) want = 1;
  g.nsplit = g.items < want ? g.items : want;
  return g;
}

template <int KS, int TH, int TW, int CB, int IB, int WK>
static int launch_wgrad(WgradP& p, const WgPlan& g, void* stream) {
  using C = WgradCfg<KS, TH, TW, CB, IB, WK>;
  auto kern = wgrad_mfma_kernel<KS, TH, TW, CB, IB, WK>;
  static bool attr_done = false;
  if (!attr_done) {
    (void)WSL_SET_MAX_DYN_SMEM(kern, C::SMEM);
    attr_done = true;
  }
  dim3 grid(g.co_blocks * g.ci_blocks, g.nsplit);
  const double px = (double)p.N * p.in.H * p.in.W;
  void* tok = prof_begin(PF_WGRAD_DIRECT, 2.0 * px * p.Co * p.in.Ci * KS * KS, 4.0 * px * (p.Co + p.in.Ci), stream);
  WSL_LAUNCH(kern, grid, dim3(kThreads), C::SMEM, stream, p);
  prof_end(tok, stream);
  return check_launch("wgrad_mfma_kernel");
}

template <int KS>
static int dispatch_wgrad(WgradP& p, const WgPlan& g, void* stream) {
#define WSL_CASE(TH_, TW_, CB_, WK_) \
  if (g.th == TH_ && g.tw == TW_ && g.cb == CB_) return launch_wgrad<KS, TH_, TW_, CB_, CB_, WK_>(p, g, stream);
  WSL_CASE(8, 64, 16, 4)
  WSL_CASE(8, 32, 16, 4)
  WSL_CASE(16, 16, 16, 4)
  WSL_CASE(8, 32, 32, 1)
  WSL_CASE(16, 16, 32, 1)
#undef WSL_CASE
  set_error("wgrad: no kernel for tile %dx%d cb %d", g.th, g.tw, g.cb);
  return WSL_EUNSUPPORTED;
}

}

namespace wsl {
bool conv2_eligible(const WslSrc& a, const WslSrc* b, const float* y, int64_t y_bs, int W, int Ci);
int conv2_pack(const float* w, float* wp, int Co, int Ci, int ks, int wmode, void* stream);
int conv2_fwd(const WslSrc& a, const WslSrc* b, const float* wp, const float* bias, float* y, int64_t y_bs, int N, int H,
              int W, int Co, int ks, int is_dgrad, int th, int tw, int co_t, float* stat_part, float* stat_cnt,
              int slots, void* stream, const BnBwdEpi* bn = nullptr, int* bn_done = nullptr);
int wgrad_small_kind(const WslSrc& a, const WslSrc* b, int H, int W, int Co, int ks);
int wgrad_small_launch(int kind, const WslSrc& a, const float* dy, int64_t dy_bs, float* part_dw, float* part_db, int N,
                       int H, int W, int nsplit, void* stream);
bool conv_cls_eligible(const WslSrc& a, const WslSrc* b, const float* y, int64_t y_bs, int H, int W, int Co, int ks,
                       const float* stat_part);
bool conv_nk16_eligible(const WslSrc& a, const WslSrc* b, const float* y, int64_t y_bs, int H, int W, int Co, int ks, int th, int tw);
int conv_nk16_launch(const WslSrc& a, const float* wp, const float* bias, float* y, int64_t y_bs, int N, int H, int W, bool dgrad,
                     float* stat_part, float* stat_cnt, int slots, const BnBwdEpi* bn, int* bn_done, void* stream);
int conv_cls_launch(const WslSrc& a, const float* wp, const float* bias, float* y, int64_t y_bs, int N, int H, int W,
                    void* stream);
int wino_pack(const float* w, float* u, int Co, int Ci, int dgrad, void* stream);
int wino_fwd(const WslSrc& a, const WslSrc* b, const float* u, const float* bias, float* y, int64_t y_bs, int N, int H,
             int W, int Co, int is_dgrad, float* stat_part, float* stat_cnt, int slots, void* stream,
             const BnBwdEpi* bn = nullptr, int* bn_done = nullptr);
bool wgrad2_eligible(const WslSrc& a, const WslSrc* b, const float* dy, int64_t dy_bs, int W);
bool wgrad2s_wide_ok(const WslSrc& a, const WslSrc* b, int H, int W, int Co, int ks);
bool wgrad_wino_ok(const WslSrc& a, const WslSrc* b, int H, int W, int Co, int ks, int th, int tw, int cb, int ib);
int wgrad2_launch(const WslSrc& a, const WslSrc* b, const float* dy, int64_t dy_bs, float* part_dw, float* part_db, int N,
                  int H, int W, int Co, int ks, int th, int tw, int cb, int ib, int nsplit, int items, int tiles_x,
                  int tiles_y, int co_blocks, int ci_blocks, void* stream);
}

using namespace wsl;

#ifdef WSL_EXPERIMENTS
extern "C" int wsl_debug_conv_plan(int th, int tw, int co_t) {
  g_forced_plan[1] = tw, g_forced_plan[2] = co_t, g_forced_plan[0] = th > 0 ? th : 0;
  return WSL_OK;
}

extern "C" int wsl_debug_wgrad_workgroups(int n) {
  g_forced_wgrad_wgs = n > 0 ? n : 0;
  return WSL_OK;
}

extern "C" int wsl_debug_conv_wino(int on) {
  g_wino = on < 0 ? -1 : (on > 2 ? 2 : on);
  return WSL_OK;
}
#endif

extern "C" int wsl_conv2d_wino_ok(int N, int H, int W, int Ca, int Cb, int Co, int ks) {
  if (N <= 0 || Ca <= 0 || Cb < 0) return 0;
  if (Cb > 0 && (Ca % 8)) return 0;
  return fwd_plan(N, H, W, Co, Ca + Cb, ks).wino ? 1 : 0;
}

extern "C" int wsl_conv2d_pack_weights(const float* w, float* packed, int Co, int Ci, int ks, int wmode_raw, void* stream) {
  WSL_REQUIRE(w && packed && Co > 0 && Ci > 0 && (ks == 1 || ks == 3) && wmode_raw >= 0 && wmode_raw <= 3,
              "conv2d_pack_weights: bad args");
  if (wmode_raw >= 2) {
    WSL_REQUIRE(ks == 3, "conv2d_pack_weights: the Winograd image exists for 3x3 filters only");
    return wino_pack(w, packed, Co, Ci, wmode_raw == 3, stream);
  }
  return conv2_pack(w, packed, Co, Ci, ks, wmode_raw, stream);
}

extern "C" int wsl_conv2d_fast_ok(const WslSrc* a, const WslSrc* b, const float* y, int64_t y_bs, int W) {
  if (!a) return 0;
  const int Ci = a->C + ((b && b->C > 0) ? b->C : 0);
  return conv2_eligible(*a, b, y, y_bs, W, Ci) ? 1 : 0;
}

extern "C" int wsl_conv2d_stat_blocks(int N, int H, int W, int Ci, int Co, int ks) {
  if (N <= 0 || H <= 0 || W <= 0 || Co <= 0) return 0;
  const FwdPlan f = fwd_plan(N, H, W, Co, Ci, ks);
  return N * cdiv(H, f.th) * cdiv(W, f.tw);
}

static int conv2d_fwd_impl(const WslSrc* a, const WslSrc* b, const float* w, const float* bias, float* y, int64_t y_bs, int N,
                           int H, int W, int Co, int ks, int wmode, float* stat_part, float* stat_cnt, void* stream,
                           const BnBwdEpi* bn, int* bn_done) {
  if (bn_done) *bn_done = 0;
  WSL_REQUIRE(a && w && y, "conv2d_fwd: null argument");
  WSL_REQUIRE(N > 0 && H > 0 && W > 0 && Co > 0, "conv2d_fwd: bad shape N=%d H=%d W=%d Co=%d", N, H, W, Co);
  WSL_REQUIRE(ks == 1 || ks == 3, "conv2d_fwd: kernel size %d not built (1 and 3 are)", ks);
  WSL_REQUIRE(wmode >= 0 && wmode <= 5, "conv2d_fwd: wmode %d", wmode);
  WSL_REQUIRE((stat_part == nullptr) == (stat_cnt == nullptr), "conv2d_fwd: stat_part and stat_cnt come together");
  if (int rc = check_src(a, H * W, "conv2d_fwd(a)")) return rc;
  ConvP p;
  p.in.a = *a;
  if (b && b->C > 0) {
    if (int rc = check_src(b, H * W, "conv2d_fwd(b)")) return rc;
    p.in.b = *b;
  } else {
    p.in.b = WslSrc{};
  }
  p.in.H = H, p.in.W = W, p.in.Ci = a->C + p.in.b.C;
  WSL_REQUIRE(y_bs >= (int64_t)Co * H * W, "conv2d_fwd: y batch stride too small");
  p.w = w, p.bias = bias, p.y = y, p.y_bs = y_bs, p.N = N, p.Co = Co, p.wmode = wmode;
  p.stat_part = stat_part, p.stat_cnt = stat_cnt;
  p.slots = 1;
  const FwdPlan f = fwd_plan(N, H, W, Co, p.in.Ci, ks);
  if (wmode >= 2) {
    if (!conv2_eligible(p.in.a, &p.in.b, y, y_bs, W, p.in.Ci)) {
      set_error("conv2d_fwd: packed weights (wmode %d) need W %% 4 == 0 and 16-byte aligned tensors", wmode);
      return WSL_EINVAL;
    }
    if (wmode >= 4) {
      WSL_REQUIRE(f.wino, "conv2d_fwd: wmode %d needs wsl_conv2d_wino_ok() != 0 for this layer", wmode);
      return wino_fwd(p.in.a, &p.in.b, w, bias, y, y_bs, N, H, W, Co, wmode == 5, stat_part, stat_cnt, p.slots, stream, bn, bn_done);
    }
    static const bool nk_on = (WSL_TUNE("WSL_CONV_NK16", 1) != 0);
    if (nk_on && conv_nk16_eligible(p.in.a, &p.in.b, y, y_bs, H, W, Co, ks, f.th, f.tw))
      return conv_nk16_launch(p.in.a, w, bias, y, y_bs, N, H, W, wmode == 3, stat_part, stat_cnt, p.slots, bn, bn_done,
                              stream);
    static const bool cls_on = (WSL_TUNE("WSL_CONV_CLS", 1) != 0);
    if (cls_on && wmode == 2 && conv_cls_eligible(p.in.a, &p.in.b, y, y_bs, H, W, Co, ks, stat_part))
      return conv_cls_launch(p.in.a, w, bias, y, y_bs, N, H, W, stream);
    return conv2_fwd(p.in.a, &p.in.b, w, bias, y, y_bs, N, H, W, Co, ks, wmode == 3, f.th, f.tw, f.co_t, stat_part,
                     stat_cnt, p.slots, stream, bn, bn_done);
  }
  p.tiles_x = cdiv(W, f.tw), p.tiles_y = cdiv(H, f.th);
  p.vec_ok = (W % 4 == 0) && (y_bs % 4 == 0) && ((reinterpret_cast<uintptr_t>(y) & 15) == 0);
  return ks == 3 ? dispatch_conv<3>(p, f, stream) : dispatch_conv<1>(p, f, stream);
}

extern "C" int wsl_conv2d_fwd(const WslSrc* a, const WslSrc* b, const float* w, const float* bias, float* y,
                              int64_t y_bs, int N, int H, int W, int Co, int ks, int wmode, float* stat_part,
                              float* stat_cnt, void* stream) {
  return conv2d_fwd_impl(a, b, w, bias, y, y_bs, N, H, W, Co, ks, wmode, stat_part, stat_cnt, stream, nullptr, nullptr);
}

static int dgrad_bn_impl(const WslSrc* dy, const float* w, float* g, int64_t g_bs, int N, int H, int W, int Co, int ks, int wmode,
                         const float* bn_y, const float* bn_st, const uint8_t* bn_emask, float bn_emask_scale, float* bn_part, int* fused,
                         bool allow_d, void* stream) {
  WSL_REQUIRE(bn_y && bn_st && bn_part && fused, "conv2d_dgrad_bn: null BatchNorm argument");
  WSL_REQUIRE(wmode == 1 || wmode == 3 || wmode == 5, "conv2d_dgrad_bn: wmode %d is not a data-gradient mode", wmode);
  BnBwdEpi e;
  e.y = bn_y, e.st = bn_st, e.emask = bn_emask, e.es = bn_emask_scale, e.part = bn_part, e.store_d = allow_d;
  if (g_bs != (int64_t)Co * H * W || (W & 3) || (reinterpret_cast<uintptr_t>(bn_y) & 15) ||
      (bn_emask && (reinterpret_cast<uintptr_t>(bn_emask) & 3)))
    e.part = nullptr;
  return conv2d_fwd_impl(dy, nullptr, w, nullptr, g, g_bs, N, H, W, Co, ks, wmode, nullptr, nullptr, stream, &e, fused);
}

extern "C" int wsl_conv2d_dgrad_bn(const WslSrc* dy, const float* w, float* g, int64_t g_bs, int N, int H, int W, int Co,
                                   int ks, int wmode, const float* bn_y, const float* bn_st, const uint8_t* bn_emask,
                                   float bn_emask_scale, float* bn_part, int* fused, void* stream) {
  return dgrad_bn_impl(dy, w, g, g_bs, N, H, W, Co, ks, wmode, bn_y, bn_st, bn_emask, bn_emask_scale, bn_part, fused, false, stream);
}

extern "C" int wsl_conv2d_dgrad_bn_d(const WslSrc* dy, const float* w, float* g, int64_t g_bs, int N, int H, int W, int Co,
                                     int ks, int wmode, const float* bn_y, const float* bn_st, const uint8_t* bn_emask,
                                     float bn_emask_scale, float* bn_part, int* fused, void* stream) {
  return dgrad_bn_impl(dy, w, g, g_bs, N, H, W, Co, ks, wmode, bn_y, bn_st, bn_emask, bn_emask_scale, bn_part, fused, true, stream);
}

extern "C" size_t wsl_conv2d_wgrad_ws_bytes(int N, int H, int W, int Ci, int Co, int ks) {
  if (N <= 0 || H <= 0 || W <= 0 || Ci <= 0 || Co <= 0) return 0;
  const WgPlan g = wgrad_plan(N, H, W, Ci, Co), g2 = wgrad_plan(N, H, W, Ci, Co, true), g3 = wgrad_plan(N, H, W, Ci, Co, true, true);
  int ns = g.nsplit > g2.nsplit ? g.nsplit : g2.nsplit;
  if (g3.nsplit > ns) ns = g3.nsplit;
  return sizeof(float) * (size_t)ns * ((size_t)ks * ks * Co * Ci + Co);
}

static int wgrad_stage1(const WslSrc* a, const WslSrc* b, const float* dy, int64_t dy_bs, float* dw, float* db, int N, int H, int W,
                        int Co, int ks, void* ws, size_t ws_bytes, void* stream, WslWgradPending* out) {
  WSL_REQUIRE(a && dy && dw && ws, "conv2d_wgrad: null argument");
  WSL_REQUIRE(N > 0 && H > 0 && W > 0 && Co > 0, "conv2d_wgrad: bad shape");
  WSL_REQUIRE(ks == 1 || ks == 3, "conv2d_wgrad: kernel size %d not built (1 and 3 are)", ks);
  if (int rc = check_src(a, H * W, "conv2d_wgrad(a)")) return rc;
  WgradP p;
  p.in.a = *a;
  if (b && b->C > 0) {
    if (int rc = check_src(b, H * W, "conv2d_wgrad(b)")) return rc;
    p.in.b = *b;
  } else {
    p.in.b = WslSrc{};
  }
  p.in.H = H, p.in.W = W, p.in.Ci = a->C + p.in.b.C;
  const int Ci = p.in.Ci;
  WSL_REQUIRE(dy_bs >= (int64_t)Co * H * W, "conv2d_wgrad: dy batch stride too small");
  const bool v2 = wgrad2_eligible(p.in.a, &p.in.b, dy, dy_bs, W);
  const bool wide = v2 && wgrad2s_wide_ok(p.in.a, &p.in.b, H, W, Co, ks);
  WgPlan g = wgrad_plan(N, H, W, Ci, Co, v2, wide);
  if (v2 && g.cb == 32 && wgrad_wino_ok(p.in.a, &p.in.b, H, W, Co, ks, g.th, g.tw, g.cb, g.ib)) {
    static const int wgs_env = WSL_TUNE("WSL_WGRAD_WINO_WGS", 0);
    const int wgs = wgs_env > 0 ? wgs_env : 512;
    int want = wgs / (g.co_blocks * g.ci_blocks);
    if (want < 1) want = 1;
    if (want < g.nsplit) g.nsplit = want;
  }
  const size_t need = wsl_conv2d_wgrad_ws_bytes(N, H, W, Ci, Co, ks);
  if (ws_bytes < need) {
    set_error("conv2d_wgrad: workspace %zu < %zu", ws_bytes, need);
    return WSL_EWORKSPACE;
  }
  const int KK = ks * ks;
  WSL_REQUIRE(sizeof(float) * (size_t)g.nsplit * ((size_t)KK * Co * Ci + Co) <= ws_bytes, "conv2d_wgrad: %d splits do not fit the workspace", g.nsplit);
  p.dy = dy, p.dy_bs = dy_bs, p.N = N, p.Co = Co;
  p.part_dw = static_cast<float*>(ws);
  p.part_db = p.part_dw + (size_t)g.nsplit * KK * Co * Ci;
  p.tiles_x = g.tiles_x, p.tiles_y = g.tiles_y, p.items = g.items, p.nsplit = g.nsplit, p.co_blocks = g.co_blocks;
  static const bool small_on = (WSL_TUNE("WSL_WGRAD_SMALL", 1) != 0);
  const int small_kind = (v2 && small_on) ? wgrad_small_kind(p.in.a, &p.in.b, H, W, Co, ks) : 0;
  if (small_kind) {
    if (int rc = wgrad_small_launch(small_kind, p.in.a, dy, dy_bs, p.part_dw, p.part_db, N, H, W, g.nsplit, stream)) return rc;
  } else if (v2) {
    if (int rc = wgrad2_launch(p.in.a, &p.in.b, dy, dy_bs, p.part_dw, p.part_db, N, H, W, Co, ks, g.th, g.tw, g.cb, g.ib,
                               g.nsplit, g.items, g.tiles_x, g.tiles_y, g.co_blocks, g.ci_blocks, stream))
      return rc;
  } else if (int rc = (ks == 3 ? dispatch_wgrad<3>(p, g, stream) : dispatch_wgrad<1>(p, g, stream))) {
    return rc;
  }
  out->part_dw = p.part_dw, out->part_db = p.part_db, out->dw = dw, out->db = db;
  out->Co = Co, out->Ci = Ci, out->KK = KK, out->nsplit = g.nsplit;
  return WSL_OK;
}

extern "C" int wsl_conv2d_wgrad_partial(const WslSrc* a, const WslSrc* b, const float* dy, int64_t dy_bs, float* dw, float* db,
                                        int N, int H, int W, int Co, int ks, void* ws, size_t ws_bytes, WslWgradPending* pending,
                                        void* stream) {
  WSL_REQUIRE(pending, "conv2d_wgrad_partial: null pending record");
  return wgrad_stage1(a, b, dy, dy_bs, dw, db, N, H, W, Co, ks, ws, ws_bytes, stream, pending);
}

namespace wsl {
constexpr int kReduceMax = 40;
struct ReduceTable {
  int n;
  int _pad;
  struct E {
    const float* pdw;
    const float* pdb;
    float* dw;
    float* db;
    int Co, Ci, KK, nsplit;
    int64_t blk0;
  } e[kReduceMax];
};

__global__ __launch_bounds__(256) void wgrad_reduce_batch_kernel(ReduceTable t) {
  __shared__ float red[kThreads];
  constexpr int SG = 8, EPB = kThreads / SG;
  int li = 0;
  for (int i = 1; i < t.n; ++i) li = (int64_t)blockIdx.x >= t.e[i].blk0 ? i : li;
  const ReduceTable::E& L = t.e[li];
  const int64_t E = (int64_t)L.KK * L.Co * L.Ci;
  const int64_t total = E + (L.db ? L.Co : 0);
  const int el = threadIdx.x % EPB, sg = threadIdx.x / EPB;
  const int64_t e = ((int64_t)blockIdx.x - L.blk0) * EPB + el;
  float s = 0.f;
  if (e < total) {
    const float* src = e < E ? L.pdw + e : L.pdb + (e - E);
    const int64_t stride = e < E ? E : L.Co;
    for (int k = sg; k < L.nsplit; k += SG) s += src[k * stride];
  }
  red[threadIdx.x] = s;
  __syncthreads();
  if (sg == 0 && e < total) {
    float v = 0.f;
#pragma unroll
    for (int k = 0; k < SG; ++k) v += red[k * EPB + el];
    if (e < E) {
      const int tap = (int)(e / ((int64_t)L.Co * L.Ci));
      const int64_t rem = e - (int64_t)tap * L.Co * L.Ci;
      L.dw[rem * L.KK + tap] = v;
    } else {
      L.db[e - E] = v;
    }
  }
}

__global__ __launch_bounds__(256) void wgrad_reduce_batch4_kernel(ReduceTable t) {
  __shared__ float4 red[kThreads];
  constexpr int SG = 8, EPB = kThreads / SG;
  int li = 0;
  for (int i = 1; i < t.n; ++i) li = (int64_t)blockIdx.x >= t.e[i].blk0 ? i : li;
  const ReduceTable::E& L = t.e[li];
  const int64_t E = (int64_t)L.KK * L.Co * L.Ci;
  const int64_t total = E + (L.db ? L.Co : 0);
  const int el = threadIdx.x % EPB, sg = threadIdx.x / EPB;
  const int64_t e = (((int64_t)blockIdx.x - L.blk0) * EPB + el) * 4;
  float4 s = make_float4(0.f, 0.f, 0.f, 0.f);
  if (e < total) {
    const float* src = e < E ? L.pdw + e : L.pdb + (e - E);
    const int64_t stride = e < E ? E : L.Co;
#pragma unroll 4
    for (int k = sg; k < L.nsplit; k += SG) {
      const float4 v = *reinterpret_cast<const float4*>(src + k * stride);
      s.x += v.x, s.y += v.y, s.z += v.z, s.w += v.w;
    }
  }
  red[threadIdx.x] = s;
  __syncthreads();
  if (sg == 0 && e < total) {
    float v[4] = {0.f, 0.f, 0.f, 0.f};
#pragma unroll
    for (int k = 0; k < SG; ++k) {
      const float4 r = red[k * EPB + el];
      v[0] += r.x, v[1] += r.y, v[2] += r.z, v[3] += r.w;
    }
    if (e < E) {
      const int64_t CC = (int64_t)L.Co * L.Ci;
      const int tap = (int)(e / CC);
      const int64_t rem = e - (int64_t)tap * CC;
#pragma unroll
      for (int q = 0; q < 4; ++q) L.dw[(rem + q) * L.KK + tap] = v[q];
// ... 55 lines not shown
```

wsl4mis_amd/csrc/wsl_conv4.hip:

```cpp
#include <type_traits>

#include "wsl_rt.h"

namespace wsl {

struct WgSmallP {
  const float* a;
  int64_t a_bs;
  const float* a_scale;
  const float* a_shift;
  const float* b;
  int64_t b_bs;
  float* part_dw;
  float* part_db;
  int N, H, W, tiles_x, tiles_y, items, nsplit;
};

template <int CBN>
struct WgSmallCfg {
  static constexpr int TH = 8, TW = 64, ROWP = TW + 8, ROWS = TH + 2, ROWP4 = ROWP / 4, S = TH * TW;
  static constexpr int PD = S / 4, GD = 256 / PD, ND = 16 / GD;
  static constexpr int PB = ROWS * ROWP4, NBF4 = CBN * PB, NB = (NBF4 + 255) / 256;
  static constexpr int PLA = ((S - 2 + 31) / 32) * 32 + 2;
  static constexpr int PLB = ROWS * ROWP + 4;
// ... 219 lines not shown
  const float* bias;
  float* y;
  int64_t y_bs;
  int N, H, W, tiles_x, tiles_y, items;
};

struct ClsCfg {
  static constexpr int TH = 8, TW = 64, ROWP = TW + 8, ROWS = TH + 2, ROWP4 = ROWP / 4, POS = ROWS * ROWP4, KC = 8;
  static constexpr int PLANE = ROWS * ROWP;
  static constexpr size_t SMEM = sizeof(float) * (2 * KC * PLANE + 32);
  static_assert(POS <= 256, "one float4 position per thread");
};

__global__ __launch_bounds__(256, 2) void conv_cls_kernel(ClsP p) {
  using C = ClsCfg;
  WSL_DYN_SMEM(smem);
  float* in_b = reinterpret_cast<float*>(smem);
  float2* tab = reinterpret_cast<float2*>(in_b + 2 * C::KC * C::PLANE);
  const int tid = threadIdx.x, lane = tid & 63, wave = tid >> 6;
  const int H = p.H, W = p.W, HW = H * W;
  const bool has_scale = p.scale != nullptr;
  if (tid < 16) tab[tid] = has_scale ? make_float2(p.scale[tid], p.shift[tid]) : make_float2(1.f, 0.f);

  float wreg[9 * 16];
#pragma unroll
  for (int k = 0; k < 9 * 16; ++k) wreg[k] = p.wp[k * 4 + (lane & 3)];
  const float bias = p.bias ? p.bias[lane & 3] : 0.f;

  const int pty = tid / C::ROWP4, ptx4 = tid - pty * C::ROWP4;
  const bool owner = tid < C::POS;
  const int loff = pty * C::ROWP + ptx4 * 4;
  const int nwg = (int)gridDim.x, bx = (int)blockIdx.x;
  const bool interleaved = (nwg & 7) == 0;
  const int it0 = interleaved ? (bx & 7) * (nwg >> 3) + (bx >> 3) : (int)((int64_t)bx * p.items / nwg);
  const int it1 = interleaved ? p.items : (int)((int64_t)(bx + 1) * p.items / nwg);
  const int step = interleaved ? nwg : 1;

  float4 pre[C::KC];
  bool pok = false;
  auto tile_of = [&](int item, int& n, int& y0, int& x0) {
    int q = item;
    const int tx = q % p.tiles_x;
    q /= p.tiles_x;
    const int ty = q % p.tiles_y;
    n = q / p.tiles_y, y0 = ty * C::TH, x0 = tx * C::TW;
  };
  auto issue = [&](int item, int ch) __attribute__((always_inline)) {
    int n, y0, x0;
    tile_of(item, n, y0, x0);
    const int gy = y0 + pty - 1, gx = x0 + ptx4 * 4 - 4;
    pok = owner && gy >= 0 && gy < H && gx >= 0 && gx < W;
    const uint32_t off = pok ? (uint32_t)(gy * W + gx) : 0u;
    const float* xb = p.x + n * p.x_bs + (int64_t)ch * C::KC * HW;
#pragma unroll
    for (int i = 0; i < C::KC; ++i) pre[i] = *reinterpret_cast<const float4*>(xb + (int64_t)i * HW + off);
  };
  auto commit = [&](int ch) __attribute__((always_inline)) {
    float* in_t = in_b + ch * (C::KC * C::PLANE);
    if (owner) {
#pragma unroll
      for (int i = 0; i < C::KC; ++i) {
        wsl_v2f lo = {pre[i].x, pre[i].y}, hi = {pre[i].z, pre[i].w};
        if (has_scale) {
          const float2 t = tab[ch * C::KC + i];
          xform_bn_leaky(lo, hi, t.x, t.y);
        }
        if (!pok) lo = wsl_v2f{0.f, 0.f}, hi = wsl_v2f{0.f, 0.f};
        *reinterpret_cast<float4*>(in_t + i * C::PLANE + loff) = make_float4(lo[0], lo[1], hi[0], hi[1]);
      }
    }
  };

  v4f acc[2];
  auto mfma_half = [&](auto ch_tag) __attribute__((always_inline)) {
    constexpr int CH = decltype(ch_tag)::value;
    const float* in_t = in_b + CH * (C::KC * C::PLANE);
#pragma unroll
    for (int cc = 0; cc < C::KC; ++cc)
#pragma unroll
      for (int ky = 0; ky < 3; ++ky) {
        float av[2][3];
#pragma unroll
        for (int rr = 0; rr < 2; ++rr)
#pragma unroll
          for (int kx = 0; kx < 3; ++kx) av[rr][kx] = in_t[cc * C::PLANE + (wave * 2 + rr + ky) * C::ROWP + lane + kx + 3];
#pragma unroll
        for (int kx = 0; kx < 3; ++kx)
#pragma unroll
          for (int rr = 0; rr < 2; ++rr) acc[rr] = WSL_MFMA4(av[rr][kx], wreg[(ky * 3 + kx) * 16 + CH * C::KC + cc], acc[rr]);
      }
  };

  if (it0 < it1) issue(it0, 0);
  __syncthreads();
  for (int item = it0; item < it1; item += step) {
    acc[0] = v4f{bias, bias, bias, bias}, acc[1] = acc[0];
    commit(0);
    issue(item, 1);
    __syncthreads();
    mfma_half(std::integral_constant<int, 0>{});
    commit(1);
    if (item + step < it1) issue(item + step, 0);
    __syncthreads();
    mfma_half(std::integral_constant<int, 1>{});
    int n, y0, x0;
    tile_of(item, n, y0, x0);
    float* yb = p.y + n * p.y_bs + (int64_t)(lane & 3) * HW + (int64_t)(y0 + wave * 2) * W + x0 + (lane >> 2) * 4;
#pragma unroll
    for (int rr = 0; rr < 2; ++rr)
      *reinterpret_cast<float4*>(yb + rr * W) = make_float4(acc[rr][0], acc[rr][1], acc[rr][2], acc[rr][3]);
  }
}

bool conv_cls_eligible(const WslSrc& a, const WslSrc* b, const float* y, int64_t y_bs, int H, int W, int Co, int ks,
                       const float* stat_part) {
  if (ks != 3 || Co != 4 || a.C != 16 || (b && b->C > 0) || a.emask || a.cmask || stat_part) return false;
  if ((H % 8) || (W % 64) || (reinterpret_cast<uintptr_t>(a.x) & 15) || (a.bs & 3)) return false;
  return (reinterpret_cast<uintptr_t>(y) & 15) == 0 && (y_bs & 3) == 0;
}

int conv_cls_launch(const WslSrc& a, const float* wp, const float* bias, float* y, int64_t y_bs, int N, int H, int W,
                    void* stream) {
  ClsP p;
  p.x = a.x, p.x_bs = a.bs, p.scale = a.scale, p.shift = a.shift, p.wp = wp, p.bias = bias, p.y = y, p.y_bs = y_bs;
  p.N = N, p.H = H, p.W = W, p.tiles_x = W / 64, p.tiles_y = H / 8, p.items = N * p.tiles_x * p.tiles_y;
  static bool attr_done = false;
  if (!attr_done) {
    (void)WSL_SET_MAX_DYN_SMEM(conv_cls_kernel, ClsCfg::SMEM);
    attr_done = true;
  }
  int wgs = forced_wgrad_wgs() > 0 ? forced_wgrad_wgs() : 2 * device_cu_count();
  if (wgs > p.items) wgs = p.items;
  const double px = (double)N * H * W;
  void* tok = prof_begin(0, 2.0 * px * 4 * 16 * 9, 4.0 * px * (16 + 4), stream);
  WSL_LAUNCH(conv_cls_kernel, dim3(wgs), dim3(kThreads), ClsCfg::SMEM, stream, p);
  prof_end(tok, stream);
  return check_launch("conv_cls_kernel");
}

struct NkP {
  const float* x;
  int64_t x_bs;
  const float* wp;
  const float* bias;
  float* y;
  int64_t y_bs;
  int N, H, W, tiles_x, tiles_y, items;
  float* stat_part;
  float* stat_cnt;
  int slots;
  BnBwdEpi bn;
};

template <int CI, int TH_ = 8, int TW_ = 64>
struct NkCfg {
  static constexpr int TH = TH_, TW = TW_, SEGW = TW / 16;
  static constexpr int PADL = 4, ROWP = TW + 2 * PADL, ROWS = TH + 2, ROWP4 = ROWP / 4, POS = ROWS * ROWP4;
  static constexpr int PLANE = ((ROWS * ROWP - 16 + 31) / 32) * 32 + 16;
  static constexpr int NG = CI == 4 ? 9 : 3;
  static constexpr size_t SMEM = sizeof(float) * (CI * PLANE + 8 * 16);
  static_assert(POS <= 256 && (CI == 1 || CI == 4) && TH * TW == 512, "one float4 position per thread");
};

constexpr int kNk16MinW = 2;
template <int CI, int TH = 8, int TW = 64, bool NHWC = false>
__global__ __launch_bounds__(256, kNk16MinW) void conv_nk16_kernel(NkP p) {
  using C = NkCfg<CI, TH, TW>;
  WSL_DYN_SMEM(smem);
  float* in_t = reinterpret_cast<float*>(smem);
  float* red = in_t + CI * C::PLANE;
  const int tid = threadIdx.x, lane = tid & 63, wave = tid >> 6;
  const int H = p.H, W = p.W, HW = H * W;
  const int c16 = lane & 15, k4 = lane >> 4;

  float bw[C::NG];
  int aoff[C::NG];
#pragma unroll
  for (int g = 0; g < C::NG; ++g) {
    if (CI == 4) {
      bw[g] = p.wp[(g * 4 + k4) * 16 + c16];
      aoff[g] = k4 * C::PLANE + (g / 3) * C::ROWP + (g % 3);
    } else {
      const int tap = 4 * g + k4;
      bw[g] = tap < 9 ? p.wp[tap * 16 + c16] : 0.f;
      aoff[g] = tap < 9 ? (tap / 3) * C::ROWP + (tap % 3) : 0;
    }
  }
  const float bias = p.bias ? p.bias[c16] : 0.f;

  const int pty = tid / C::ROWP4, ptx4 = tid - pty * C::ROWP4;
  const bool owner = tid < C::POS;
  const int loff = pty * C::ROWP + ptx4 * 4;
  const int it0 = (int)((int64_t)blockIdx.x * p.items / gridDim.x), it1 = (int)((int64_t)(blockIdx.x + 1) * p.items / gridDim.x);
  float4 pre[CI];
  bool pok = false;
  auto tile_of = [&](int item, int& n, int& y0, int& x0) {
    int q = item;
    const int tx = q % p.tiles_x;
    q /= p.tiles_x;
    const int ty = q % p.tiles_y;
    n = q / p.tiles_y, y0 = ty * C::TH, x0 = tx * C::TW;
  };
  auto issue = [&](int item) __attribute__((always_inline)) {
    int n, y0, x0;
    tile_of(item, n, y0, x0);
    const int gy = y0 + pty - 1, gx = x0 + ptx4 * 4 - C::PADL;
    pok = owner && gy >= 0 && gy < H && gx >= 0 && gx < W;
    const uint32_t off = pok ? (uint32_t)(gy * W + gx) : 0u;
    const float* xb = p.x + n * p.x_bs;
#pragma unroll
    for (int i = 0; i < CI; ++i) pre[i] = *reinterpret_cast<const float4*>(xb + (int64_t)i * HW + off);
  };
  auto commit = [&]() __attribute__((always_inline)) {
    if (owner) {
#pragma unroll
      for (int i = 0; i < CI; ++i)
        *reinterpret_cast<float4*>(in_t + i * C::PLANE + loff) = pok ? pre[i] : make_float4(0.f, 0.f, 0.f, 0.f);
    }
  };

  if (it0 < it1) issue(it0);
  for (int item = it0; item < it1; ++item) {
    commit();
    __syncthreads();
    if (item + 1 < it1) issue(item + 1);
    int n, y0, x0;
    tile_of(item, n, y0, x0);
    v4f acc[8];
#pragma unroll
    for (int sg = 0; sg < 8; ++sg) {
      acc[sg] = v4f{bias, bias, bias, bias};
      const float* ab = in_t + ((8 * wave + sg) / C::SEGW) * C::ROWP + (C::PADL - 1) + 16 * ((8 * wave + sg) % C::SEGW) + c16;
#pragma unroll
      for (int g = 0; g < C::NG; ++g) acc[sg] = WSL_MFMA16(ab[aoff[g]], bw[g], acc[sg]);
    }
    if constexpr (NHWC) {
      float* yb = p.y + n * p.y_bs + ((int64_t)y0 * W + x0 + 4 * k4) * 16 + c16;
#pragma unroll
      for (int sg = 0; sg < 8; ++sg)
#pragma unroll
        for (int r = 0; r < 4; ++r)
          yb[((int64_t)((8 * wave + sg) / C::SEGW) * W + 16 * ((8 * wave + sg) % C::SEGW) + r) * 16] = acc[sg][r];
    } else {
    float* yb = p.y + n * p.y_bs + (int64_t)c16 * HW + (int64_t)y0 * W + x0 + 4 * k4;
#pragma unroll
    for (int sg = 0; sg < 8; ++sg)
      *reinterpret_cast<float4*>(yb + ((8 * wave + sg) / C::SEGW) * W + 16 * ((8 * wave + sg) % C::SEGW)) =
          make_float4(acc[sg][0], acc[sg][1], acc[sg][2], acc[sg][3]);
    }

    if (p.bn.part) {
      const float mean = p.bn.st[c16], invstd = p.bn.st[16 + c16], sc = p.bn.st[32 + c16], sh = p.bn.st[48 + c16];
      const int64_t base = ((int64_t)n * 16 + c16) * HW + (int64_t)y0 * W + x0 + 4 * k4;
      BnBwdAcc ba;
#pragma unroll
      for (int sg = 0; sg < 8; ++sg)
        bn_bwd_acc4(p.bn, base + ((8 * wave + sg) / C::SEGW) * W + 16 * ((8 * wave + sg) % C::SEGW), acc[sg][0], acc[sg][1], acc[sg][2], acc[sg][3], mean, invstd, sc,
                    sh, ba);
      float s1[1], s2[1];
      bn_bwd_fold(ba, s1[0], s2[0]);
      bn_bwd_store<1, 16>(p.bn, s1, s2, red, 0, 16, item, p.items);
    } else if (p.stat_part) {
      constexpr float cnt = (float)(C::TH * C::TW);
      float* red1 = red;
      float* red2 = red + 64;
      float bs = 0.f;
#pragma unroll
      for (int sg = 0; sg < 8; ++sg) bs += (acc[sg][0] + acc[sg][1]) + (acc[sg][2] + acc[sg][3]);
      bs += __shfl_xor(bs, 16);
      bs += __shfl_xor(bs, 32);
      if (lane < 16) red1[wave * 16 + lane] = bs;
      __syncthreads();
      const float mean_b = (red1[c16] + red1[16 + c16] + red1[32 + c16] + red1[48 + c16]) / cnt;
      float q = 0.f;
#pragma unroll
      for (int sg = 0; sg < 8; ++sg)
#pragma unroll
        for (int e = 0; e < 4; ++e) {
          const float d = acc[sg][e] - mean_b;
          q = fmaf(d, d, q);
        }
      q += __shfl_xor(q, 16);
      q += __shfl_xor(q, 32);
      if (lane < 16) red2[wave * 16 + lane] = q;
      __syncthreads();
      if (wave == 0 && lane < 16) {
        float* dst = p.stat_part + ((int64_t)lane * ((int64_t)p.items * p.slots) + (int64_t)item * p.slots) * 2;
        dst[0] = red1[lane] + red1[16 + lane] + red1[32 + lane] + red1[48 + lane];
        dst[1] = red2[lane] + red2[16 + lane] + red2[32 + lane] + red2[48 + lane];
        if (lane < p.slots) p.stat_cnt[item * p.slots + lane] = lane == 0 ? cnt : 0.f;
      }
    }
    __syncthreads();
  }
}

bool conv_nk16_eligible(const WslSrc& a, const WslSrc* b, const float* y, int64_t y_bs, int H, int W, int Co, int ks, int th, int tw) {
  if (ks != 3 || Co != 16 || (a.C != 1 && a.C != 4) || (b && b->C > 0) || a.scale || a.emask || a.cmask) return false;
  if (th != 8 || tw != 64 || (H % 8) || (W % 64) || (reinterpret_cast<uintptr_t>(a.x) & 15) || (a.bs & 3)) return false;
  return (reinterpret_cast<uintptr_t>(y) & 15) == 0 && (y_bs & 3) == 0 && (int64_t)16 * H * W < (int64_t(1) << 31);
}

template <int CI, int TH, int TW>
static int launch_nk16(NkP& p, bool dgrad, void* stream) {
  using C = NkCfg<CI, TH, TW>;
  auto kern = conv_nk16_kernel<CI, TH, TW>;
  p.tiles_x = p.W / TW, p.tiles_y = p.H / TH;
  static bool attr_done = false;
  if (!attr_done) {
    (void)WSL_SET_MAX_DYN_SMEM(kern, C::SMEM);
    attr_done = true;
  }
  int wgs = kNk16MinW * device_cu_count();
  if (wgs > p.items) wgs = p.items;
  const double px = (double)p.N * p.H * p.W;
  void* tok = prof_begin(dgrad ? PF_CONV_DGRAD : PF_CONV_FWD, 2.0 * px * CI * 16 * 9, 4.0 * px * (16 + CI) + bn_epi_bytes(p.bn, px * 16), stream);
  WSL_LAUNCH(kern, dim3(wgs), dim3(kThreads), C::SMEM, stream, p);
  prof_end(tok, stream);
  return check_launch("conv_nk16_kernel");
}

int conv_nk16_launch(const WslSrc& a, const float* wp, const float* bias, float* y, int64_t y_bs, int N, int H, int W, bool dgrad,
                     float* stat_part, float* stat_cnt, int slots, const BnBwdEpi* bn, int* bn_done, void* stream) {
  NkP p;
  p.x = a.x, p.x_bs = a.bs, p.wp = wp, p.bias = bias, p.y = y, p.y_bs = y_bs;
  p.N = N, p.H = H, p.W = W, p.tiles_x = W / 64, p.tiles_y = H / 8, p.items = N * p.tiles_x * p.tiles_y;
  p.stat_part = stat_part, p.stat_cnt = stat_cnt, p.slots = slots;
  const bool bn_ok = bn && bn->part;
  if (bn_ok) p.bn = *bn;
  if (bn_done) *bn_done = bn_ok ? 1 : 0;
#ifdef WSL_EXPERIMENTS
  static const int nhwc = WSL_TUNE("WSL_NK16_NHWC", 0);
  if (nhwc) {
    auto kern = a.C == 4 ? conv_nk16_kernel<4, 8, 64, true> : conv_nk16_kernel<1, 8, 64, true>;
    p.tiles_x = W / 64, p.tiles_y = H / 8;
    int wgs = kNk16MinW * device_cu_count();
    if (wgs > p.items) wgs = p.items;
    WSL_LAUNCH(kern, dim3(wgs), dim3(kThreads), (a.C == 4 ? NkCfg<4>::SMEM : NkCfg<1>::SMEM), stream, p);
    return check_launch("conv_nk16_kernel(nhwc probe)");
  }
  static const int wide = WSL_TUNE("WSL_NK16_WIDE", 0);
  if (wide && W % 128 == 0) return a.C == 4 ? launch_nk16<4, 4, 128>(p, dgrad, stream) : launch_nk16<1, 4, 128>(p, dgrad, stream);
#endif
  return a.C == 4 ? launch_nk16<4, 8, 64>(p, dgrad, stream) : launch_nk16<1, 8, 64>(p, dgrad, stream);
}

#ifdef WSL_EXPERIMENTS
#ifndef WSL_HOST_EMUL
template <int SHAPE>
__global__ __launch_bounds__(256) void mfma_stream_kernel(float* out, int iters) {
  typedef float v4 __attribute__((ext_vector_type(4)));
  typedef float v16 __attribute__((ext_vector_type(16)));
  const float a = 1.0f + threadIdx.x * 1e-6f, b = 0.5f;
  float r = 0.f;
  if (SHAPE == 1) {
    v16 acc[4];
    for (int i = 0; i < 4; ++i) for (int k = 0; k < 16; ++k) acc[i][k] = 0.f;
    for (int it = 0; it < iters; ++it) {
#pragma unroll
      for (int u = 0; u < 4; ++u)
#pragma unroll
        for (int i = 0; i < 4; ++i) acc[i] = __builtin_amdgcn_mfma_f32_32x32x2f32(a, b, acc[i], 0, 0, 0);
    }
    for (int i = 0; i < 4; ++i) r += acc[i][0];
  } else {
    v4 acc[16];
    for (int i = 0; i < 16; ++i) acc[i] = v4{0.f, 0.f, 0.f, 0.f};
    for (int it = 0; it < iters; ++it) {
#pragma unroll
      for (int i = 0; i < 16; ++i)
        acc[i] = SHAPE == 0 ? __builtin_amdgcn_mfma_f32_16x16x4f32(a, b, acc[i], 0, 0, 0) : __builtin_amdgcn_mfma_f32_4x4x1f32(a, b, acc[i], 0, 0, 0);
    }
    for (int i = 0; i < 16; ++i) r += acc[i][0];
  }
  if (r == 123.456f) out[0] = r;
}

template <int MODE, int K>
__global__ __launch_bounds__(512) void mfma_valu_mix_kernel(float* out, int iters) {
  typedef float v4 __attribute__((ext_vector_type(4)));
  const float a = 1.0f + threadIdx.x * 1e-6f, b = 0.5f;
  v4 acc[16];
  for (int i = 0; i < 16; ++i) acc[i] = v4{0.f, 0.f, 0.f, 0.f};
  float x[8];
  for (int i = 0; i < 8; ++i) x[i] = a + i;
  const bool mfma_wave = MODE == 0 || (threadIdx.x >> 6) < 4;
  const bool valu_wave = MODE == 0 || (threadIdx.x >> 6) >= 4;
  if (mfma_wave && valu_wave) {
    for (int it = 0; it < iters; ++it) {
#pragma unroll
      for (int i = 0; i < 16; ++i) {
        acc[i] = __builtin_amdgcn_mfma_f32_16x16x4f32(a, b, acc[i], 0, 0, 0);
#pragma unroll
        for (int k = 0; k < K; ++k) x[k & 7] = __builtin_fmaf(x[k & 7], 1.0001f, 0.5f);
        __builtin_amdgcn_sched_group_barrier(0x008, 1, 0);
        __builtin_amdgcn_sched_group_barrier(0x002, K, 0);
      }
    }
  } else if (mfma_wave) {
    for (int it = 0; it < iters; ++it) {
#pragma unroll
      for (int i = 0; i < 16; ++i) acc[i] = __builtin_amdgcn_mfma_f32_16x16x4f32(a, b, acc[i], 0, 0, 0);
    }
  } else {
    for (int it = 0; it < iters; ++it) {
#pragma unroll
      for (int i = 0; i < 16 * K; ++i) x[i & 7] = __builtin_fmaf(x[i & 7], 1.0001f, 0.5f);
    }
  }
  float r = 0.f;
  for (int i = 0; i < 16; ++i) r += acc[i][0];
  for (int i = 0; i < 8; ++i) r += x[i];
  if (r == 123.456f) out[0] = r;
}

template <int K>
__global__ __launch_bounds__(256) void mfma_pk_mix_kernel(float* out, int iters) {
  typedef float v4 __attribute__((ext_vector_type(4)));
  const float a = 1.0f + threadIdx.x * 1e-6f, b = 0.5f;
  v4 acc[16];
  for (int i = 0; i < 16; ++i) acc[i] = v4{0.f, 0.f, 0.f, 0.f};
  wsl_v2f x[8];
  for (int i = 0; i < 8; ++i) x[i] = wsl_v2f{a + i, a - i};
  for (int it = 0; it < iters; ++it) {
#pragma unroll
    for (int i = 0; i < 16; ++i) {
      acc[i] = __builtin_amdgcn_mfma_f32_16x16x4f32(a, b, acc[i], 0, 0, 0);
#pragma unroll
      for (int k = 0; k < K; ++k)
        asm volatile("v_pk_add_f32 %0, %0, %0 op_sel:[0,1] op_sel_hi:[0,1] neg_hi:[0,1]" : "+v"(x[k & 7]));
      __builtin_amdgcn_sched_group_barrier(0x008, 1, 0);
      __builtin_amdgcn_sched_group_barrier(0x002, K, 0);
    }
  }
  float r = 0.f;
  for (int i = 0; i < 16; ++i) r += acc[i][0];
  for (int i = 0; i < 8; ++i) r += x[i][0] + x[i][1];
  if (r == 123.456f) out[0] = r;
}
#endif

#ifndef WSL_HOST_EMUL
__global__ void lds_dma_probe_kernel(const float* g, float* out) {
  __shared__ __attribute__((aligned(16))) float lds[2048];
  typedef __attribute__((address_space(1))) const void* gptr_t;
  typedef __attribute__((address_space(3))) void* lptr_t;
  for (int i = threadIdx.x; i < 2048; i += 256) lds[i] = -1.f;
  __syncthreads();
  const int wave = threadIdx.x >> 6;
  if ((threadIdx.x & 63) != 5)
    __builtin_amdgcn_global_load_lds((gptr_t)(g + threadIdx.x * 4), (lptr_t)(lds + wave * 256 + 8), 16, 0, 0);
  __builtin_amdgcn_s_waitcnt(0);
  __syncthreads();
  for (int i = threadIdx.x; i < 2048; i += 256) out[i] = lds[i];
}
#endif

#ifndef WSL_HOST_EMUL
__global__ void pk_probe_kernel(const float* in, float* out) {
  const int t = threadIdx.x;
  const float* d = in + 20 * t;
  wsl_v2f lo[4], hi[4], a[4], b[4], q1, q2, m[4];
  for (int i = 0; i < 4; ++i) lo[i] = wsl_v2f{d[4 * i], d[4 * i + 1]}, hi[i] = wsl_v2f{d[4 * i + 2], d[4 * i + 3]};
  const wsl_v2f r0 = {d[16], d[17]}, r1 = {d[18], d[19]};
  wino_btdb_pk(lo, hi, a, b);
  wino_aya_pk(r0, r1, q1, q2, m);
  const wsl_v2f q[4] = {r0, q1, q2, r1};
  float* o = out + 32 * t;
  for (int xi = 0; xi < 16; ++xi) o[xi] = wino_pick(a, b, xi), o[16 + xi] = wino_pick(q, m, xi);
}
#endif

#ifndef WSL_HOST_EMUL
__global__ void mfma4_probe_kernel(const float* a, const float* b, float* d) {
  typedef float v4 __attribute__((ext_vector_type(4)));
  v4 acc = {0.f, 0.f, 0.f, 0.f};
  acc = __builtin_amdgcn_mfma_f32_4x4x1f32(a[threadIdx.x], b[threadIdx.x], acc, 0, 0, 0);
  for (int r = 0; r < 4; ++r) d[threadIdx.x * 4 + r] = acc[r];
}
#endif

#endif

}

#ifdef WSL_EXPERIMENTS
extern "C" int wsl_debug_lds_dma_probe(const float* g, float* out, void* stream) {
#ifndef WSL_HOST_EMUL
  WSL_LAUNCH(wsl::lds_dma_probe_kernel, dim3(1), dim3(256), 0, stream, g, out);
  return wsl::check_launch("lds_dma_probe_kernel");
#else
  (void)g, (void)out, (void)stream;
  return WSL_EUNSUPPORTED;
#endif
}

extern "C" int wsl_debug_mfma_stream(int shape, int blocks, int iters, float* out, void* stream) {
// ... 48 lines not shown
```

wsl4mis_amd/csrc/wsl_debug.h:

```cpp
#pragma once
#ifdef __cplusplus
extern "C" {
#endif

struct WslNetDesc;
int wsl_debug_net_decisions(const struct WslNetDesc* d, const void* ws, size_t ws_bytes, int which, int index, unsigned char* out,
                            void* stream);

int wsl_debug_net_ws_region(const struct WslNetDesc* d, int index, char* name, size_t name_len, size_t* off_floats, size_t* n_floats);

int wsl_debug_sp_conv_residency(int N, int H, int W, int Ci, int Co, int want_bn_epilogue, int* tile_h, int* tile_w, int* co_t,
                                size_t* lds_bytes, int* per_cu);

int wsl_debug_conv_plan(int th, int tw, int co_t);
int wsl_debug_conv_wino(int on);
int wsl_debug_wgrad_workgroups(int n);

int wsl_debug_mfma4_probe(const float* a, const float* b, float* d, void* stream);
int wsl_debug_mfma_stream(int shape, int blocks, int iters, float* out, void* stream);
int wsl_debug_pk_probe(const float* in, float* out, void* stream);
int wsl_debug_lds_dma_probe(const float* g, float* out, void* stream);
#ifdef __cplusplus
}
#endif
```

wsl4mis_amd/csrc/wsl_net.hip:

```cpp
#include <initializer_list>

#include "wsl_seq.h"

namespace wsl {

int sp_pack_table(const PackTable& t, const int64_t* img_off_bytes, const float* params, void* imgf, void* imgd, uint32_t* amax,
                  int with_dgrad, void* stream);

static const int kFt[5] = {16, 32, 64, 128, 256};
static const float kDrop[5] = {0.05f, 0.1f, 0.2f, 0.3f, 0.5f};
constexpr int kSpMaxLayers = 40;

struct BlockRef { ConvRef c1, c2; BnRef b1, b2; };
struct BlkWs { size_t y1, y2, st1, st2; };

struct Plan {
  WslNetDesc d;
  int H[5], W[5];
  BlockRef enc[5];
  struct Dec { ConvRef c1x1[4]; BlockRef blk[4]; ConvRef out; } dec[2];
  int64_t n_param, n_enc_param, n_buf, n_bn;
  BlkWs wenc[5];
  size_t pooled[5];
  struct DecWs { size_t u[4], up[4], dcat[4], glow4; BlkWs blk[4]; } wdec[2];
  struct Scratch { size_t tmp_g, tmp_g1, tmp_dy, tmp_du, tmp_gpool, stat_part, stat_cnt, wg_ws, bn_ws, bn_coef; } scr[2];
  size_t packf, packd;
  size_t winof, winod;
  size_t spf, spd, sp_wmax, sp_dymax, sp_upmax;
  int sp;
  size_t wg_bytes, bn_bytes, bn_coef_bytes, total_floats;
  struct Region { char name[48]; size_t off, n; } regs[192];
  int nregs;
  bool want_regions = false, regs_overflow = false;
};

static void plan_block(BlockRef& k, int Ci, int Co, int64_t& po, int64_t& bo, int64_t& nbn) {
  plan_conv(k.c1, Ci, Co, 3, po);
  plan_bn(k.b1, Co, po, bo, nbn);
  plan_conv(k.c2, Co, Co, 3, po);
  plan_bn(k.b2, Co, po, bo, nbn);
}

static size_t layer_need(const Plan& P, const ConvRef& c, int l, size_t& max_stat, size_t& max_cnt, size_t& nb) {
  const int N = P.d.N, H = P.H[l], W = P.W[l];
  nb = wsl_conv2d_stat_blocks(N, H, W, c.Ci, c.Co, 3);
  size_t wgb = wsl_conv2d_wgrad_ws_bytes(N, H, W, c.Ci, c.Co, 3);
  if (P.sp) {
    const size_t nb2 = wsl_sp_conv2d_stat_blocks(N, H, W, c.Ci, c.Co);
    const size_t wgb2 = wsl_sp_conv2d_wgrad_ws_bytes(N, H, W, c.Ci, c.Co);
    nb = nb2 > nb ? nb2 : nb, wgb = wgb2 > wgb ? wgb2 : wgb;
  }
  if (nb * c.Co * 2 > max_stat) max_stat = nb * c.Co * 2;
  if (nb > max_cnt) max_cnt = nb;
  return (wgb + 255) & ~(size_t)255;
}

template <class B>
static void plan_scratch(B& b, Plan& P, int k, size_t big, size_t small, size_t max_stat, size_t max_cnt) {
  Plan::Scratch& S = P.scr[k];
  S.tmp_g = b.take(big, "tmp_g"), S.tmp_g1 = b.take(big, "tmp_g1"), S.tmp_dy = b.take(big, "tmp_dy");
  S.tmp_du = b.take(small, "tmp_du"), S.tmp_gpool = b.take(small, "tmp_gpool");
  S.stat_part = b.take(max_stat, "stat_part"), S.stat_cnt = b.take(max_cnt, "stat_cnt");
  S.wg_ws = b.take((P.wg_bytes + 3) / 4, "wg_ws"), S.bn_ws = b.take((P.bn_bytes + 3) / 4, "bn_ws");
  S.bn_coef = b.take((P.bn_coef_bytes + 3) / 4, "bn_coef");
}

static int make_plan(const WslNetDesc* d, Plan& P) {
  WSL_REQUIRE(d, "net: null descriptor");
  WSL_REQUIRE(d->n_dec == 1 || d->n_dec == 2, "net: n_dec must be 1 (unet) or 2 (unet_cct)");
  WSL_REQUIRE(d->in_chns > 0 && d->n_class > 0 && d->n_class <= 8, "net: bad channel counts");
  WSL_REQUIRE(d->N > 0 && d->H >= 16 && d->W >= 16 && d->H % 16 == 0 && d->W % 16 == 0,
              "net: N=%d H=%d W=%d (H, W must be multiples of 16)", d->N, d->H, d->W);
  WSL_REQUIRE(d->precision == 0 || d->precision == 1, "net: precision %d (0 = f32, 1 = split f16 x 3)", d->precision);
  P.d = *d;
  P.sp = d->precision;
  for (int l = 0; l < 5; ++l) P.H[l] = d->H >> l, P.W[l] = d->W >> l;
  int64_t po = 0, bo = 0, nbn = 0;
  plan_block(P.enc[0], d->in_chns, kFt[0], po, bo, nbn);
  for (int l = 1; l < 5; ++l) plan_block(P.enc[l], kFt[l - 1], kFt[l], po, bo, nbn);
  P.n_enc_param = po;
  for (int k = 0; k < d->n_dec; ++k) {
    for (int i = 0; i < 4; ++i) {
      const int c1 = kFt[4 - i], c2 = kFt[3 - i];
      plan_conv(P.dec[k].c1x1[i], c1, c2, 1, po);
      plan_block(P.dec[k].blk[i], 2 * c2, c2, po, bo, nbn);
    }
    plan_conv(P.dec[k].out, kFt[0], d->n_class, 3, po);
  }
  P.n_param = po, P.n_buf = bo, P.n_bn = nbn;
  {
    int li = 0;
    for (int l = 0; l < 5; ++l) P.enc[l].c1.li = li++, P.enc[l].c2.li = li++;
    for (int k = 0; k < d->n_dec; ++k) {
      for (int i = 0; i < 4; ++i) P.dec[k].c1x1[i].li = li++, P.dec[k].blk[i].c1.li = li++, P.dec[k].blk[i].c2.li = li++;
      P.dec[k].out.li = li++;
    }
  }

  Bump B0;
  P.nregs = 0;
  struct Named {
    Bump& b;
    Plan& P;
    const char* tag = "";
    int i0 = 0, i1 = 0;
    size_t& off;
    size_t take(size_t n, const char* what = "") {
      const size_t o = b.take(n);
      if (P.want_regions) {
        if (P.nregs < 192) {
          Plan::Region& r = P.regs[P.nregs++];
          snprintf(r.name, sizeof(r.name), "%s[%d,%d].%s", tag, i0, i1, what);
          r.off = o, r.n = n;
        } else {
          P.regs_overflow = true;
        }
      }
      return o;
    }
  } B{B0, P, "", 0, 0, B0.off};
  const size_t N = d->N;
  size_t max_stat = 0, max_cnt = 0;
  size_t wg_enc = 0, wg_dec = 0;
  P.bn_bytes = 0;
  auto wg_add = [](size_t& acc, size_t bytes) { acc += (bytes + 255) & ~(size_t)255; };
  size_t* wg_acc = &wg_enc;
  auto plan_blkws = [&](BlkWs& w, const BlockRef& k, int l) {
    const size_t e = N * k.c1.Co * P.H[l] * P.W[l];
    w.y1 = B.take(e, "y1"), w.y2 = B.take(e, "y2");
    w.st1 = B.take(4 * k.c1.Co, "st1"), w.st2 = B.take(4 * k.c1.Co, "st2");
    for (const ConvRef* c : {&k.c1, &k.c2}) {
      size_t nb;
      *wg_acc += layer_need(P, *c, l, max_stat, max_cnt, nb);
      size_t nbb = nb;
      for (int co_alt : {c->Ci, c->Co}) {
        const size_t a = wsl_conv2d_stat_blocks(d->N, P.H[l], P.W[l], c->Co, co_alt, 3), a1 = wsl_conv2d_stat_blocks(d->N, P.H[l], P.W[l], c->Co, co_alt, 1);
        nbb = a > nbb ? a : nbb, nbb = a1 > nbb ? a1 : nbb;
      }
      const size_t fan = wsl_feat_grad_combine_blocks(d->N, P.H[l], P.W[l]);
      nbb = fan > nbb ? fan : nbb;
      const size_t pb = sizeof(float) * (nbb * c->Co * 2 + 2 * (size_t)c->Co);
      if (pb > P.bn_bytes) P.bn_bytes = pb;
    }
    const size_t bb = wsl_bnact_bwd_ws_bytes(d->N, k.c1.Co, P.H[l], P.W[l]);
    if (bb > P.bn_bytes) P.bn_bytes = bb;
  };
  for (int l = 0; l < 5; ++l) {
    B.tag = "enc", B.i0 = l, B.i1 = 0;
    plan_blkws(P.wenc[l], P.enc[l], l);
    P.pooled[l] = l ? B.take(N * kFt[l - 1] * P.H[l] * P.W[l], "pooled") : 0;
  }
  for (int k = 0; k < d->n_dec; ++k) {
    wg_dec = 0, wg_acc = &wg_dec;
    for (int i = 0; i < 4; ++i) {
      const int l = 3 - i, c2 = kFt[l];
      B.tag = "dec", B.i0 = k, B.i1 = i;
      P.wdec[k].u[i] = B.take(N * c2 * P.H[l + 1] * P.W[l + 1], "u");
      P.wdec[k].up[i] = B.take(N * c2 * P.H[l] * P.W[l], "up");
      P.wdec[k].dcat[i] = B.take(N * 2 * c2 * P.H[l] * P.W[l], "dcat");
      plan_blkws(P.wdec[k].blk[i], P.dec[k].blk[i], l);
      wg_add(wg_dec, wsl_conv2d_wgrad_ws_bytes(d->N, P.H[l + 1], P.W[l + 1], kFt[l + 1], c2, 1));
    }
    P.wdec[k].glow4 = B.take(N * kFt[4] * P.H[4] * P.W[4], "glow4");
    wg_add(wg_dec, wsl_conv2d_wgrad_ws_bytes(d->N, P.H[0], P.W[0], kFt[0], d->n_class, 3));
  }
  P.wg_bytes = wg_enc > wg_dec ? wg_enc : wg_dec;
  const size_t big = N * kFt[0] * P.H[0] * P.W[0];
  P.bn_coef_bytes = 0;
  for (int l = 0; l < 5; ++l) {
    const size_t b = wsl_bnact_bwd_finish_ws_bytes(d->N, kFt[l], P.H[l], P.W[l], 1);
    if (b > P.bn_coef_bytes) P.bn_coef_bytes = b;
  }
  if (P.sp)
    for (int l = 0; l < 4; ++l) {
      const size_t b = wsl_bilinear_up2_fwd_amax_ws_bytes(d->N, kFt[l], P.H[l + 1], P.W[l + 1]);
      if (b > P.bn_coef_bytes) P.bn_coef_bytes = b;
    }
  for (int k = 0; k < d->n_dec; ++k) {
    B.tag = "scratch", B.i0 = k, B.i1 = 0;
    plan_scratch(B, P, k, big, big / 4, max_stat, max_cnt);
  }
  if (d->n_dec == 1) P.scr[1] = P.scr[0];
  B.tag = "images", B.i0 = 0, B.i1 = 0;
  P.packf = B.take(P.n_param, "packf"), P.packd = B.take(P.n_param, "packd");
  P.winof = B.take(2 * P.n_param, "winof"), P.winod = B.take(2 * P.n_param, "winod");
  P.spf = P.spd = P.sp_wmax = P.sp_dymax = P.sp_upmax = 0;
  if (P.sp) {
    P.spf = B.take(P.n_param * 10 / 9 + 64, "spf"), P.spd = B.take(P.n_param * 10 / 9 + 64, "spd");
    P.sp_wmax = B.take(kSpMaxLayers, "sp_wmax"), P.sp_dymax = B.take((size_t)P.n_bn * WSL_SP_AMAX_SLOTS, "sp_dymax");
    P.sp_upmax = B.take((size_t)d->n_dec * 4 * WSL_SP_AMAX_SLOTS, "sp_upmax");
  }
  P.total_floats = B.off;
  return WSL_OK;
}

struct Ctx {
  const Plan& P;
  const float* params;
  float* buffers;
  int64_t* nbt;
  float* grads;
  float* ws;
  void* stream;
  int training;
  int si = 0;
  WgBatch* wb = nullptr;
  const Plan::Scratch& S() const { return P.scr[si]; }
};

static int wgrad_layer(const Ctx& c, const WslSrc* a, const WslSrc* b, const float* dy, int64_t dy_bs, float* dw, float* db, int H,
                       int W, int Co, int ks, const uint32_t* dy_amax = nullptr, const uint32_t* raw_amax = nullptr) {
  const int N = c.P.d.N, Ci = a->C + (b ? b->C : 0);
  const bool sp = c.P.sp && dy_amax && ks == 3 && wsl_sp_conv2d_ok(a, b, nullptr, 0, N, H, W, Co, 3) &&
                  !(reinterpret_cast<uintptr_t>(dy) & 15) && !(dy_bs & 3) && Co % 32 == 0 && a->C % 32 == 0 && (!b || b->C % 32 == 0);
  const size_t need = ((sp ? wsl_sp_conv2d_wgrad_ws_bytes(N, H, W, Ci, Co) : wsl_conv2d_wgrad_ws_bytes(N, H, W, Ci, Co, ks)) + 255) &
                      ~(size_t)255;
  return wgrad_push(c.wb, "net", c.ws + c.S().wg_ws, need, [&](void* ws, size_t n, WslWgradPending* q) {
    return sp ? wsl_sp_conv2d_wgrad_partial_amax(a, b, dy, dy_bs, dy_amax, raw_amax, dw, db, N, H, W, Co, ws, n, q, c.stream)
              : wsl_conv2d_wgrad_partial(a, b, dy, dy_bs, dw, db, N, H, W, Co, ks, ws, n, q, c.stream);
  });
}

static WslSrc act_src(const Ctx& c, size_t y, size_t st, int C, int HW, const uint8_t* emask, float es, const float* cmask) {
  return act_src(c.ws + y, C, (int64_t)C * HW, c.ws + st + 2 * C, c.ws + st + 3 * C, emask, es, cmask);
}

static size_t sp_img_off(const ConvRef& cv) { return 4 * (size_t)((10 * cv.w + 35) / 36); }
static const uint32_t* sp_wmax(const Ctx& c, const ConvRef& cv) { return reinterpret_cast<const uint32_t*>(c.ws + c.P.sp_wmax) + cv.li; }
static uint32_t* sp_dymax(const Ctx& c, const BnRef& bn) {
  return c.P.sp ? reinterpret_cast<uint32_t*>(c.ws + c.P.sp_dymax) + (size_t)bn.nbt * WSL_SP_AMAX_SLOTS : nullptr;
}
static uint32_t* sp_upmax(const Ctx& c, int k, int i) {
  return c.P.sp ? reinterpret_cast<uint32_t*>(c.ws + c.P.sp_upmax) + (size_t)(k * 4 + i) * WSL_SP_AMAX_SLOTS : nullptr;
}
static bool sp_takes(const Ctx& c, const ConvRef& cv, const WslSrc* a, const WslSrc* b, const float* y, int64_t y_bs, int H, int W,
                     int Co) {
  return c.P.sp && cv.ks == 3 && wsl_sp_conv2d_ok(a, b, y, y_bs, c.P.d.N, H, W, Co, 3);
}

static int conv_any(const Ctx& c, const ConvRef& cv, int dgrad, const WslSrc* a, const WslSrc* b, const float* bias,
                    float* y, int64_t y_bs, int H, int W, float* stp, float* stc, const uint32_t* in_amax = nullptr) {
  const int N = c.P.d.N, Co = dgrad ? cv.Ci : cv.Co;
  if ((!dgrad || in_amax) && sp_takes(c, cv, a, b, y, y_bs, H, W, Co))
    return wsl_sp_conv2d_fwd(a, b, c.ws + (dgrad ? c.P.spd : c.P.spf) + sp_img_off(cv), sp_wmax(c, cv), in_amax, bias,
                             y, y_bs, N, H, W, Co, stp, stc, c.stream);
  if (wsl_conv2d_fast_ok(a, b, y, y_bs, W)) {
    if (wsl_conv2d_wino_ok(N, H, W, a->C, b ? b->C : 0, Co, cv.ks))
      return wsl_conv2d_fwd(a, b, c.ws + (dgrad ? c.P.winod : c.P.winof) + 2 * cv.w, bias, y, y_bs, N, H, W, Co, cv.ks,
                            dgrad ? 5 : 4, stp, stc, c.stream);
    return wsl_conv2d_fwd(a, b, c.ws + (dgrad ? c.P.packd : c.P.packf) + cv.w, bias, y, y_bs, N, H, W, Co, cv.ks,
                          dgrad ? 3 : 2, stp, stc, c.stream);
  }
  return wsl_conv2d_fwd(a, b, c.params + cv.w, bias, y, y_bs, N, H, W, Co, cv.ks, dgrad, stp, stc, c.stream);
}

struct GStats {
  int nblk = 0;
  int channel_major = 0;
  int g_is_d = 0;
};

static int conv_dgrad_bn(const Ctx& c, const ConvRef& cv, const float* dy, float* g, int H, int W, size_t y, size_t st,
                         const uint8_t* emask, float es, GStats* gs, const uint32_t* dy_amax = nullptr) {
  const int N = c.P.d.N, Cg = cv.Ci;
  const WslSrc dys = raw_src(dy, cv.Co, (int64_t)cv.Co * H * W);
  const int64_t g_bs = (int64_t)Cg * H * W;
  if (dy_amax && sp_takes(c, cv, &dys, nullptr, g, g_bs, H, W, Cg)) {
    int fused = 0;
    WSL_TRY(wsl_sp_conv2d_dgrad_bn(&dys, dy_amax, c.ws + c.P.spd + sp_img_off(cv), sp_wmax(c, cv), g, g_bs, N, H, W, Cg, c.ws + y,
                                   c.ws + st, emask, es, c.ws + c.S().bn_ws, &fused, c.stream));
    gs->nblk = fused ? wsl_sp_conv2d_stat_blocks(N, H, W, cv.Co, Cg) : 0;
    gs->channel_major = 1;
    gs->g_is_d = 0;
    return WSL_OK;
  }
  const float* w = c.params + cv.w;
  int wmode = 1;
  if (wsl_conv2d_fast_ok(&dys, nullptr, g, g_bs, W)) {
    if (wsl_conv2d_wino_ok(N, H, W, cv.Co, 0, Cg, cv.ks)) w = c.ws + c.P.winod + 2 * cv.w, wmode = 5;
    else w = c.ws + c.P.packd + cv.w, wmode = 3;
  }
  int fused = 0;
  WSL_TRY(wsl_conv2d_dgrad_bn_d(&dys, w, g, g_bs, N, H, W, Cg, cv.ks, wmode, c.ws + y, c.ws + st, emask, es, c.ws + c.S().bn_ws,
                                &fused, c.stream));
  gs->nblk = fused ? wsl_conv2d_stat_blocks(N, H, W, cv.Co, Cg, cv.ks) : 0;
  gs->channel_major = 1;
  gs->g_is_d = fused == 2;
  return WSL_OK;
}

static int bn_bwd(const Ctx& c, const float* g, int64_t g_bs, size_t y, size_t st, const BnRef& bn, const uint8_t* emask, float es,
                  float* dy, int H, int W, const GStats& gs) {
  const Plan& P = c.P;
  const int C = bn.C;
  const float* s = c.ws + st;
  if (gs.nblk && gs.g_is_d)
    return wsl_bnact_bwd_finish_d_amax(g, g_bs, c.ws + y, s, s + C, c.params + bn.gamma, c.params + bn.beta, dy, c.grads + bn.gamma,
                                       c.grads + bn.beta, P.d.N, C, H, W, c.ws + c.S().bn_ws, gs.nblk, gs.channel_major,
                                       c.ws + c.S().bn_coef, P.bn_coef_bytes, sp_dymax(c, bn), c.stream);
  if (gs.nblk)
    return wsl_bnact_bwd_finish_amax(g, g_bs, c.ws + y, s, s + C, c.params + bn.gamma, c.params + bn.beta, emask, es, dy,
                                     c.grads + bn.gamma, c.grads + bn.beta, P.d.N, C, H, W, c.ws + c.S().bn_ws, gs.nblk,
                                     gs.channel_major, c.ws + c.S().bn_coef, P.bn_coef_bytes, sp_dymax(c, bn), c.stream);
  return wsl_bnact_bwd_amax(g, g_bs, c.ws + y, s, s + C, c.params + bn.gamma, c.params + bn.beta, emask, es, dy, c.grads + bn.gamma,
                            c.grads + bn.beta, P.d.N, C, H, W, c.ws + c.S().bn_ws, P.bn_bytes, sp_dymax(c, bn), c.stream);
}

static int pack_all(const Ctx& c, int with_dgrad) {
  const Plan& P = c.P;
  PackTable t;
  t.n = 0;
  auto one = [&](const ConvRef& cv, int l, int ca = 0, int cb = 0) {
    int skip = 0;
    if (cv.ks == 3) {
      const int N = P.d.N, H = P.H[l], W = P.W[l];
      if (wsl_conv2d_wino_ok(N, H, W, ca ? ca : cv.Ci, cb, cv.Co, 3)) skip |= 1;
      if (wsl_conv2d_wino_ok(N, H, W, cv.Co, 0, cv.Ci, 3)) skip |= 2;
    }
    t.e[t.n++] = PackEntry{cv.w, cv.Co, cv.Ci, cv.ks * cv.ks, skip};
  };
  for (int l = 0; l < 5; ++l) one(P.enc[l].c1, l), one(P.enc[l].c2, l);
  for (int k = 0; k < P.d.n_dec; ++k) {
    for (int i = 0; i < 4; ++i) {
      const int l = 3 - i;
      one(P.dec[k].c1x1[i], l + 1), one(P.dec[k].blk[i].c1, l, kFt[l], kFt[l]), one(P.dec[k].blk[i].c2, l);
    }
    one(P.dec[k].out, 0);
  }
  WSL_TRY(conv2_pack_table(t, c.params, c.ws + P.packf, c.ws + P.packd, with_dgrad, c.stream));
  WSL_TRY(wino_pack_table(t, c.params, c.ws + P.winof, c.ws + P.winod, with_dgrad, c.stream));
  if (P.sp) {
    WSL_REQUIRE(t.n <= kSpMaxLayers, "net: %d conv layers exceed the split path's table (%d)", t.n, kSpMaxLayers);
    int64_t off[kSpMaxLayers];
    for (int i = 0; i < t.n; ++i) off[i] = 4 * (int64_t)(4 * ((10 * t.e[i].w + 35) / 36));
    if (hipMemsetAsync(c.ws + P.sp_wmax, 0, kSpMaxLayers * sizeof(float), (hipStream_t)c.stream) != hipSuccess ||
        (with_dgrad && hipMemsetAsync(c.ws + P.sp_dymax, 0, (size_t)P.n_bn * WSL_SP_AMAX_SLOTS * sizeof(float), (hipStream_t)c.stream) != hipSuccess)) {
      set_error("net: clearing the split path's maxima failed");
      return WSL_EHIP;
    }
    WSL_TRY(sp_pack_table(t, off, c.params, c.ws + P.spf, c.ws + P.spd, reinterpret_cast<uint32_t*>(c.ws + P.sp_wmax), with_dgrad,
                          c.stream));
  }
  return WSL_OK;
}

static int conv_bn_fwd(const Ctx& c, const ConvRef& cv, const BnRef& bn, const WslSrc* a, const WslSrc* b, size_t y,
                       size_t st, int H, int W, const uint32_t* raw_amax = nullptr) {
  const Plan& P = c.P;
  const int N = P.d.N, C = cv.Co;
  float* stp = c.training ? c.ws + c.S().stat_part : nullptr;
  float* stc = c.training ? c.ws + c.S().stat_cnt : nullptr;
  WSL_TRY(conv_any(c, cv, 0, a, b, c.params + cv.b, c.ws + y, (int64_t)C * H * W, H, W, stp, stc, raw_amax));
  float* s = c.ws + st;
  const int nblk = !c.training ? 0
                   : sp_takes(c, cv, a, b, c.ws + y, (int64_t)C * H * W, H, W, C) ? wsl_sp_conv2d_stat_blocks(N, H, W, cv.Ci, C)
                                                                                  : wsl_conv2d_stat_blocks(N, H, W, cv.Ci, C, cv.ks);
  return bn_fwd(c.training, stp, stc, nblk, bn, c.params, c.buffers, c.nbt, s, s + C, s + 2 * C, s + 3 * C, c.stream);
}

static int block_fwd(const Ctx& c, const BlockRef& k, const BlkWs& w, const WslSrc* a, const WslSrc* b, int l,
                     const uint8_t* emask, float es, const uint32_t* raw_amax = nullptr) {
  const int H = c.P.H[l], W = c.P.W[l], C = k.c1.Co;
  WSL_TRY(conv_bn_fwd(c, k.c1, k.b1, a, b, w.y1, w.st1, H, W, raw_amax));
  const WslSrc mid = act_src(c, w.y1, w.st1, C, H * W, c.training ? emask : nullptr, es, nullptr);
  return conv_bn_fwd(c, k.c2, k.b2, &mid, nullptr, w.y2, w.st2, H, W);
}

static int block_bwd(const Ctx& c, const BlockRef& k, const BlkWs& w, const WslSrc* a, const WslSrc* b, int l,
                     const uint8_t* emask, float es, const float* g, int64_t g_bs, const GStats& gs, float* dgrad_out,
                     const uint32_t* raw_amax = nullptr) {
  const Plan& P = c.P;
  const int H = P.H[l], W = P.W[l], C = k.c1.Co;
  const int64_t CHW = (int64_t)C * H * W;
  float* dy = c.ws + c.S().tmp_dy;
  float* g1 = c.ws + c.S().tmp_g1;
  WSL_TRY(bn_bwd(c, g, g_bs, w.y2, w.st2, k.b2, nullptr, 1.f, dy, H, W, gs));
  const WslSrc mid = act_src(c, w.y1, w.st1, C, H * W, emask, es, nullptr);
  WSL_TRY(wgrad_layer(c, &mid, nullptr, dy, CHW, c.grads + k.c2.w, c.grads + k.c2.b, H, W, C, 3, sp_dymax(c, k.b2)));
  GStats g1s;
  WSL_TRY(conv_dgrad_bn(c, k.c2, dy, g1, H, W, w.y1, w.st1, emask, es, &g1s, sp_dymax(c, k.b2)));
  WSL_TRY(bn_bwd(c, g1, CHW, w.y1, w.st1, k.b1, emask, es, dy, H, W, g1s));
  WSL_TRY(wgrad_layer(c, a, b, dy, CHW, c.grads + k.c1.w, c.grads + k.c1.b, H, W, C, 3, sp_dymax(c, k.b1), raw_amax));
  if (dgrad_out) {
    const WslSrc dys1 = raw_src(dy, C, CHW);
    WSL_TRY(conv_any(c, k.c1, 1, &dys1, nullptr, nullptr, dgrad_out, (int64_t)k.c1.Ci * H * W, H, W, nullptr, nullptr,
                     sp_dymax(c, k.b1)));
  }
  return WSL_OK;
}

static WslSrc feat_src(const Ctx& c, int l, const float* cmask) {
  return act_src(c, c.P.wenc[l].y2, c.P.wenc[l].st2, kFt[l], c.P.H[l] * c.P.W[l], nullptr, 1.f, cmask);
}

static int decoder_fwd(const Ctx& c, int k, const float* const* cmasks, float* logits) {
  const Plan& P = c.P;
  const int N = P.d.N;
  for (int i = 0; i < 4; ++i) {
    const int l = 3 - i, c1 = kFt[l + 1], c2 = kFt[l];
    const int h = P.H[l + 1], w = P.W[l + 1], H = P.H[l], W = P.W[l];
    const WslSrc low = i == 0 ? feat_src(c, 4, cmasks ? cmasks[4] : nullptr)
                              : act_src(c, P.wdec[k].blk[i - 1].y2, P.wdec[k].blk[i - 1].st2, c1, h * w, nullptr, 1.f, nullptr);
    const ConvRef& cv = P.dec[k].c1x1[i];
    WSL_TRY(conv_any(c, cv, 0, &low, nullptr, c.params + cv.b, c.ws + P.wdec[k].u[i], (int64_t)c2 * h * w, h, w, nullptr,
                     nullptr));
    WSL_TRY(wsl_bilinear_up2_fwd_amax(c.ws + P.wdec[k].u[i], c.ws + P.wdec[k].up[i], (int64_t)c2 * H * W, N, c2, h, w,
                                      c.ws + c.S().bn_coef, P.bn_coef_bytes, sp_upmax(c, k, i), c.stream));
    const WslSrc skip = feat_src(c, l, cmasks ? cmasks[l] : nullptr);
    const WslSrc up = raw_src(c.ws + P.wdec[k].up[i], c2, (int64_t)c2 * H * W);
    WSL_TRY(block_fwd(c, P.dec[k].blk[i], P.wdec[k].blk[i], &skip, &up, l, nullptr, 1.f, sp_upmax(c, k, i)));
  }
  const WslSrc last = act_src(c, P.wdec[k].blk[3].y2, P.wdec[k].blk[3].st2, kFt[0], P.H[0] * P.W[0], nullptr, 1.f, nullptr);
  const ConvRef& oc = P.dec[k].out;
  return conv_any(c, oc, 0, &last, nullptr, c.params + oc.b, logits, (int64_t)oc.Co * P.H[0] * P.W[0], P.H[0], P.W[0], nullptr,
                  nullptr);
}

static int decoder_bwd(const Ctx& c, int k, const float* const* cmasks, const float* dlogits) {
  const Plan& P = c.P;
  const int N = P.d.N, H0 = P.H[0], W0 = P.W[0];
  float* g = c.ws + c.S().tmp_g;
  const ConvRef& oc = P.dec[k].out;
  const WslSrc last = act_src(c, P.wdec[k].blk[3].y2, P.wdec[k].blk[3].st2, kFt[0], H0 * W0, nullptr, 1.f, nullptr);
  WSL_TRY(wgrad_layer(c, &last, nullptr, dlogits, (int64_t)oc.Co * H0 * W0, c.grads + oc.w, c.grads + oc.b, H0, W0, oc.Co, 3));
  GStats gs;
  WSL_TRY(conv_dgrad_bn(c, oc, dlogits, g, H0, W0, P.wdec[k].blk[3].y2, P.wdec[k].blk[3].st2, nullptr, 1.f, &gs));
  for (int i = 3; i >= 0; --i) {
    const int l = 3 - i, c1 = kFt[l + 1], c2 = kFt[l];
    const int h = P.H[l + 1], w = P.W[l + 1], H = P.H[l], W = P.W[l];
    const WslSrc skip = feat_src(c, l, cmasks ? cmasks[l] : nullptr);
    const WslSrc up = raw_src(c.ws + P.wdec[k].up[i], c2, (int64_t)c2 * H * W);
    float* dcat = c.ws + P.wdec[k].dcat[i];
    WSL_TRY(block_bwd(c, P.dec[k].blk[i], P.wdec[k].blk[i], &skip, &up, l, nullptr, 1.f, g, (int64_t)c2 * H * W, gs, dcat, sp_upmax(c, k, i)));
    float* du = c.ws + c.S().tmp_du;
    WSL_TRY(wsl_bilinear_up2_bwd(dcat + (int64_t)c2 * H * W, (int64_t)2 * c2 * H * W, du, N, c2, h, w, c.stream));
    const WslSrc low = i == 0 ? feat_src(c, 4, cmasks ? cmasks[4] : nullptr)
                              : act_src(c, P.wdec[k].blk[i - 1].y2, P.wdec[k].blk[i - 1].st2, c1, h * w, nullptr, 1.f, nullptr);
    const ConvRef& cv = P.dec[k].c1x1[i];
    WSL_TRY(wgrad_layer(c, &low, nullptr, du, (int64_t)c2 * h * w, c.grads + cv.w, c.grads + cv.b, h, w, c2, 1));
    if (i == 0) {
      const WslSrc dus = raw_src(du, c2, (int64_t)c2 * h * w);
      WSL_TRY(conv_any(c, cv, 1, &dus, nullptr, nullptr, c.ws + P.wdec[k].glow4, (int64_t)c1 * h * w, h, w, nullptr, nullptr));
    } else {
      WSL_TRY(conv_dgrad_bn(c, cv, du, g, h, w, P.wdec[k].blk[i - 1].y2, P.wdec[k].blk[i - 1].st2, nullptr, 1.f, &gs));
    }
  }
  return wgrad_flush(c.wb, c.stream);
}

static int encoder_bwd(const Ctx& c, const float* x, const uint8_t* const* emasks, const float* const* cmasks) {
  const Plan& P = c.P;
  const int N = P.d.N;
  const bool dual = P.d.n_dec == 2;
  float* g = c.ws + c.S().tmp_g;
  float* gpool = c.ws + c.S().tmp_gpool;
  for (int l = 4; l >= 0; --l) {
    const int C = kFt[l], H = P.H[l], W = P.W[l];
    const WslSrc f = feat_src(c, l, nullptr);
    const float *ga, *gb = nullptr;
    int64_t bs;
    if (l == 4) {
      ga = c.ws + P.wdec[0].glow4, bs = (int64_t)C * H * W;
      if (dual) gb = c.ws + P.wdec[1].glow4;
    } else {
      const int i = 3 - l;
      ga = c.ws + P.wdec[0].dcat[i], bs = (int64_t)2 * C * H * W;
      if (dual) gb = c.ws + P.wdec[1].dcat[i];
    }
    const float* st2 = c.ws + P.wenc[l].st2;
    WSL_TRY(wsl_feat_grad_combine_bn(&f, ga, bs, gb, bs, dual ? cmasks[l] : nullptr, l < 4 ? gpool : nullptr, g, N, H, W, st2,
                                     st2 + C, c.ws + c.S().bn_ws, c.stream));
    GStats gs;
    gs.nblk = wsl_feat_grad_combine_blocks(N, H, W), gs.channel_major = 0;
    const WslSrc in = l == 0 ? raw_src(x, P.d.in_chns, (int64_t)P.d.in_chns * H * W)
                             : raw_src(c.ws + P.pooled[l], kFt[l - 1], (int64_t)kFt[l - 1] * H * W);
    WSL_TRY(block_bwd(c, P.enc[l], P.wenc[l], &in, nullptr, l, emasks[l], 1.f / (1.f - kDrop[l]), g, (int64_t)C * H * W, gs,
                      l > 0 ? gpool : nullptr));
  }
  return wgrad_flush(c.wb, c.stream);
}

}

using namespace wsl;

static int enumerate_entries(const Plan& P, int want, WslNetEntry* out) {
  EntryWalk e{want, out};
  auto block = [&](const char* pre, const BlockRef& k) {
    e.conv(pre, ".0", k.c1), e.bn(pre, ".1", k.b1), e.conv(pre, ".4", k.c2), e.bn(pre, ".5", k.b2);
  };
  char pre[96];
  block("encoder.in_conv.conv_conv", P.enc[0]);
  for (int l = 1; l < 5; ++l) {
    snprintf(pre, sizeof(pre), "encoder.down%d.maxpool_conv.1.conv_conv", l);
    block(pre, P.enc[l]);
  }
  for (int k = 0; k < P.d.n_dec; ++k) {
    const char* dn = P.d.n_dec == 1 ? "decoder" : (k == 0 ? "main_decoder" : "aux_decoder1");
    for (int i = 0; i < 4; ++i) {
      snprintf(pre, sizeof(pre), "%s.up%d.conv1x1", dn, i + 1);
      e.conv(pre, "", P.dec[k].c1x1[i]);
      snprintf(pre, sizeof(pre), "%s.up%d.conv.conv_conv", dn, i + 1);
      block(pre, P.dec[k].blk[i]);
    }
    snprintf(pre, sizeof(pre), "%s.out_conv", dn);
    e.conv(pre, "", P.dec[k].out);
  }
  return e.idx;
}

extern "C" int wsl_net_num_entries(const WslNetDesc* d) {
  Plan P;
  if (make_plan(d, P)) return -1;
  return enumerate_entries(P, -1, nullptr);
}
extern "C" int wsl_net_entry(const WslNetDesc* d, int i, WslNetEntry* out) {
  Plan P;
  WSL_TRY(make_plan(d, P));
  WSL_REQUIRE(out && i >= 0, "net_entry: bad args");
  const int n = enumerate_entries(P, i, out);
  WSL_REQUIRE(i < n, "net_entry: index %d out of %d", i, n);
  return WSL_OK;
}
extern "C" int64_t wsl_net_param_count(const WslNetDesc* d) {
  Plan P;
  return make_plan(d, P) ? -1 : P.n_param;
}
extern "C" int64_t wsl_net_encoder_param_count(const WslNetDesc* d) {
  Plan P;
  return make_plan(d, P) ? -1 : P.n_enc_param;
}
extern "C" int64_t wsl_net_buffer_count(const WslNetDesc* d) {
  Plan P;
  return make_plan(d, P) ? -1 : P.n_buf;
}
extern "C" size_t wsl_net_ws_bytes(const WslNetDesc* d) {
  Plan P;
  return make_plan(d, P) ? 0 : P.total_floats * sizeof(float);
}

extern "C" int wsl_net_forward(const WslNetDesc* d, const float* params, float* buffers, int64_t* nbt, const float* x,
                               const uint8_t* const* emasks, const float* const* cmasks, int training, float* logits_main,
                               float* logits_aux, void* ws, size_t ws_bytes, void* stream) {
  Plan P;
  WSL_TRY(make_plan(d, P));
  WSL_REQUIRE(params && buffers && x && logits_main && ws, "net_forward: null argument");
  WSL_REQUIRE(d->n_dec == 1 || (logits_aux && cmasks), "net_forward: unet_cct needs logits_aux and cmasks");
  WSL_REQUIRE(!training || emasks, "net_forward: training needs the 5 dropout keep-masks");
  WSL_TRY(check_ws("net_forward", ws_bytes, P.total_floats * sizeof(float)));
  Ctx c{P, params, buffers, nbt, nullptr, static_cast<float*>(ws), stream, training};
  const int N = d->N;
  WSL_TRY(pack_all(c, training));
  for (int l = 0; l < 5; ++l) {
    const int H = P.H[l], W = P.W[l];
    WslSrc in;
    if (l == 0) {
      in = raw_src(x, d->in_chns, (int64_t)d->in_chns * H * W);
    } else {
      const WslSrc prev = feat_src(c, l - 1, nullptr);
      WSL_TRY(wsl_pool2_fwd(&prev, c.ws + P.pooled[l], N, P.H[l - 1], P.W[l - 1], stream));
      in = raw_src(c.ws + P.pooled[l], kFt[l - 1], (int64_t)kFt[l - 1] * H * W);
    }
    WSL_TRY(block_fwd(c, P.enc[l], P.wenc[l], &in, nullptr, l, training ? emasks[l] : nullptr, 1.f / (1.f - kDrop[l])));
  }
  void* side = d->n_dec == 2 ? side_stream(stream) : nullptr;
  if (side) {
    Ctx c2 = c;
    c2.stream = side, c2.si = 1;
    WSL_TRY(stream_fork(stream, side));
    WSL_TRY(decoder_fwd(c, 0, nullptr, logits_main));
    WSL_TRY(decoder_fwd(c2, 1, cmasks, logits_aux));
    return stream_join(stream, side);
  }
  WSL_TRY(decoder_fwd(c, 0, nullptr, logits_main));
  if (d->n_dec == 2) WSL_TRY(decoder_fwd(c, 1, cmasks, logits_aux));
  return WSL_OK;
}

extern "C" int wsl_net_backward(const WslNetDesc* d, const float* params, const float* x, const uint8_t* const* emasks,
                                const float* const* cmasks, const float* dlogits_main, const float* dlogits_aux,
                                float* grads, void* ws, size_t ws_bytes, int phase, void* stream) {
  Plan P;
  WSL_TRY(make_plan(d, P));
  WSL_REQUIRE(params && x && emasks && grads && ws, "net_backward: null argument");
  WSL_REQUIRE(phase >= 0 && phase <= 2, "net_backward: phase %d", phase);
  WSL_REQUIRE(phase == 2 || (dlogits_main && (d->n_dec == 1 || (dlogits_aux && cmasks))), "net_backward: missing dlogits");
  WSL_TRY(check_ws("net_backward", ws_bytes, P.total_floats * sizeof(float)));
  Ctx c{P, params, nullptr, nullptr, grads, static_cast<float*>(ws), stream, 1};
  WgBatch wb0, wb1;
  wb0.cap = wb1.cap = P.wg_bytes;
  c.wb = &wb0;
  if (phase == 0 || phase == 1) {
    void* side = d->n_dec == 2 ? side_stream(stream) : nullptr;
    if (side) {
      Ctx c2 = c;
      c2.stream = side, c2.si = 1, c2.wb = &wb1;
      WSL_TRY(stream_fork(stream, side));
      WSL_TRY(decoder_bwd(c, 0, nullptr, dlogits_main));
      WSL_TRY(decoder_bwd(c2, 1, cmasks, dlogits_aux));
      WSL_TRY(stream_join(stream, side));
    } else {
      WSL_TRY(decoder_bwd(c, 0, nullptr, dlogits_main));
      if (d->n_dec == 2) WSL_TRY(decoder_bwd(c, 1, cmasks, dlogits_aux));
    }
  }
  if (phase == 0 || phase == 2) WSL_TRY(encoder_bwd(c, x, emasks, cmasks));
  return WSL_OK;
}

namespace wsl {
__global__ __launch_bounds__(256) void dbg_sign_kernel(const float* y, const float* sc, const float* sh, unsigned char* out, int C, int HW) {
  const int c = blockIdx.y, n = blockIdx.z;
  const float a = sc[c], b = sh[c];
  const int64_t base = ((int64_t)n * C + c) * HW;
  for (int i = blockIdx.x * kThreads + threadIdx.x; i < HW; i += gridDim.x * kThreads) out[base + i] = fmaf(y[base + i], a, b) > 0.f ? 1 : 0;
}
__global__ __launch_bounds__(256) void dbg_argmax_kernel(const float* y, const float* sc, const float* sh, unsigned char* out, int C, int H,
                                                         int W) {
  const int c = blockIdx.y, n = blockIdx.z, Ho = H / 2, Wo = W / 2;
  const float a = sc[c], b = sh[c];
  const float* p = y + ((int64_t)n * C + c) * H * W;
  for (int o = blockIdx.x * kThreads + threadIdx.x; o < Ho * Wo; o += gridDim.x * kThreads) {
    const int oy = o / Wo, ox = o - oy * Wo;
    float best = 0.f;
    int arg = 0;
#pragma unroll
    for (int k = 0; k < 4; ++k) {
      const float v = leaky(fmaf(p[(int64_t)(2 * oy + (k >> 1)) * W + 2 * ox + (k & 1)], a, b));
      if (k == 0 || v > best) best = v, arg = k;
    }
    out[((int64_t)n * C + c) * Ho * Wo + o] = (unsigned char)arg;
  }
}
}

extern "C" int wsl_debug_net_ws_region(const WslNetDesc* d, int index, char* name, size_t name_len, size_t* off_floats, size_t* n_floats) {
  Plan P;
  P.want_regions = true;
  WSL_TRY(make_plan(d, P));
  WSL_REQUIRE(!P.regs_overflow, "debug_net_ws_region: more than 192 workspace regions (raise Plan::regs)");
  if (index < 0 || index >= P.nregs) return 1;
  WSL_REQUIRE(name && name_len > 0 && off_floats && n_floats, "debug_net_ws_region: null argument");
  snprintf(name, name_len, "%s", P.regs[index].name);
  *off_floats = P.regs[index].off, *n_floats = P.regs[index].n;
  return WSL_OK;
}

extern "C" int wsl_debug_net_decisions(const WslNetDesc* d, const void* ws, size_t ws_bytes, int which, int index, unsigned char* out,
                                       void* stream) {
  Plan P;
  WSL_TRY(make_plan(d, P));
  WSL_REQUIRE(ws && out && ws_bytes >= P.total_floats * sizeof(float), "debug_net_decisions: bad workspace");
  const float* w = static_cast<const float*>(ws);
  size_t y = 0, st = 0;
  int C = 0, l = 0;
  if (which == 0) {
    WSL_REQUIRE(index >= 0 && index < (int)P.n_bn, "debug_net_decisions: BatchNorm layer %d of %d", index, (int)P.n_bn);
    bool found = false;
    auto look = [&](const BlockRef& k, const BlkWs& bw, int lev) {
      if (k.b1.nbt == index) y = bw.y1, st = bw.st1, C = k.b1.C, l = lev, found = true;
      if (k.b2.nbt == index) y = bw.y2, st = bw.st2, C = k.b2.C, l = lev, found = true;
    };
    for (int lev = 0; lev < 5; ++lev) look(P.enc[lev], P.wenc[lev], lev);
    for (int k = 0; k < d->n_dec; ++k)
      for (int i = 0; i < 4; ++i) look(P.dec[k].blk[i], P.wdec[k].blk[i], 3 - i);
    WSL_REQUIRE(found, "debug_net_decisions: layer not found");
    const int HW = P.H[l] * P.W[l];
    WSL_LAUNCH(dbg_sign_kernel, dim3(cdiv(HW, 4 * kThreads), C, d->N), dim3(kThreads), 0, stream, w + y, w + st + 2 * C, w + st + 3 * C, out,
               C, HW);
    return check_launch("dbg_sign_kernel");
  }
  WSL_REQUIRE(which == 1 && index >= 1 && index <= 4, "debug_net_decisions: which %d index %d", which, index);
  l = index - 1, C = kFt[l];
  WSL_LAUNCH(dbg_argmax_kernel, dim3(cdiv(P.H[l] * P.W[l] / 4, 4 * kThreads), C, d->N), dim3(kThreads), 0, stream, w + P.wenc[l].y2,
             w + P.wenc[l].st2 + 2 * C, w + P.wenc[l].st2 + 3 * C, out, C, P.H[l], P.W[l]);
  return check_launch("dbg_argmax_kernel");
}

namespace wsl {

struct UpPlan {
  Plan P;
  ConvRef up;
  BlockRef blk;
  BlkWs wblk;
  size_t upt, dcat, tmp_out;
  int C1, C2, Co, h, w;
};

static int make_up_plan(const WslUpBlockDesc* d, UpPlan& U) {
  WSL_REQUIRE(d && d->N > 0 && d->C1 > 0 && d->C1 <= 256 && d->C2 > 0 && d->C2 <= 256 && d->Co > 0 && d->h > 0 && d->w > 0,
              "upblock_t: bad descriptor (C1, C2 <= 256)");
  WSL_REQUIRE(d->dropout_p >= 0.f && d->dropout_p < 1.f, "upblock_t: dropout_p %f", (double)d->dropout_p);
  Plan& P = U.P;
  memset(&P, 0, sizeof(P));
  P.d.in_chns = d->C1, P.d.n_class = 1, P.d.n_dec = 1, P.d.N = d->N, P.d.H = 2 * d->h, P.d.W = 2 * d->w;
  P.H[0] = 2 * d->h, P.W[0] = 2 * d->w;
  U.C1 = d->C1, U.C2 = d->C2, U.Co = d->Co, U.h = d->h, U.w = d->w;
  int64_t po = 0, bo = 0, nbn = 0;
  U.up.Ci = d->C1, U.up.Co = d->C2, U.up.ks = 2;
  U.up.w = po, po += (int64_t)d->C1 * d->C2 * 4;
  U.up.b = po, po += d->C2;
  plan_block(U.blk, 2 * d->C2, d->Co, po, bo, nbn);
  P.n_param = po, P.n_enc_param = 0, P.n_buf = bo, P.n_bn = nbn;
  Bump B;
  const size_t N = d->N, HW = (size_t)P.H[0] * P.W[0];
  const size_t e = N * d->Co * HW;
  U.wblk.y1 = B.take(e), U.wblk.y2 = B.take(e), U.wblk.st1 = B.take(4 * d->Co), U.wblk.st2 = B.take(4 * d->Co);
  U.upt = B.take(N * d->C2 * HW), U.dcat = B.take(N * 2 * d->C2 * HW), U.tmp_out = B.take(e);
  size_t max_stat = 0, max_cnt = 0, wg = 0, nb;
  for (const ConvRef* cv : {&U.blk.c1, &U.blk.c2}) wg += layer_need(P, *cv, 0, max_stat, max_cnt, nb);
  const size_t ct = wsl_convt2x2_wgrad_ws_bytes(d->N, d->C1, d->C2);
  P.wg_bytes = wg > ct ? wg : ct;
  P.bn_bytes = wsl_bnact_bwd_ws_bytes(d->N, d->Co, P.H[0], P.W[0]);
  P.bn_coef_bytes = sizeof(float) * (2 * (size_t)d->Co + 64);
  plan_scratch(B, P, 0, e, 0, max_stat, max_cnt);
  P.scr[1] = P.scr[0];
  P.packf = B.take(P.n_param), P.packd = B.take(P.n_param);
  P.winof = B.take(2 * P.n_param), P.winod = B.take(2 * P.n_param);
  P.total_floats = B.off;
  return WSL_OK;
}

static int up_pack(const Ctx& c, const UpPlan& U, int with_dgrad) {
  PackTable t;
  t.n = 0;
  for (const ConvRef* cv : {&U.blk.c1, &U.blk.c2}) t.e[t.n++] = PackEntry{cv->w, cv->Co, cv->Ci, 9, 0};
  WSL_TRY(conv2_pack_table(t, c.params, c.ws + U.P.packf, c.ws + U.P.packd, with_dgrad, c.stream));
  return wino_pack_table(t, c.params, c.ws + U.P.winof, c.ws + U.P.winod, with_dgrad, c.stream);
}

}

extern "C" int64_t wsl_upblock_t_param_count(const WslUpBlockDesc* d) {
  UpPlan U;
  return make_up_plan(d, U) ? -1 : U.P.n_param;
}
extern "C" size_t wsl_upblock_t_ws_bytes(const WslUpBlockDesc* d) {
  UpPlan U;
  return make_up_plan(d, U) ? 0 : U.P.total_floats * sizeof(float);
}

extern "C" int wsl_upblock_t_forward(const WslUpBlockDesc* d, const float* params, float* buffers, int64_t* nbt, const float* x1,
                                     const float* x2, const uint8_t* emask, int training, float* out, void* ws, size_t ws_bytes,
                                     void* stream) {
  UpPlan U;
  WSL_TRY(make_up_plan(d, U));
  WSL_REQUIRE(params && buffers && x1 && x2 && out && ws, "upblock_t_forward: null argument");
  WSL_REQUIRE(!(training && d->dropout_p > 0.f) || emask, "upblock_t_forward: training with dropout_p > 0 needs the keep mask");
  WSL_TRY(check_ws("upblock_t_forward", ws_bytes, U.P.total_floats * sizeof(float)));
  const Plan& P = U.P;
  Ctx c{P, params, buffers, nbt, nullptr, static_cast<float*>(ws), stream, training};
  const int H = P.H[0], W = P.W[0];
  WSL_TRY(up_pack(c, U, training));
  WSL_TRY(wsl_convt2x2_fwd(x1, params + U.up.w, params + U.up.b, c.ws + U.upt, d->N, U.C1, U.C2, U.h, U.w, stream));
  const WslSrc skip = raw_src(x2, U.C2, (int64_t)U.C2 * H * W);
  const WslSrc up = raw_src(c.ws + U.upt, U.C2, (int64_t)U.C2 * H * W);
  const float es = d->dropout_p > 0.f ? 1.f / (1.f - d->dropout_p) : 1.f;
  WSL_TRY(block_fwd(c, U.blk, U.wblk, &skip, &up, 0, d->dropout_p > 0.f ? emask : nullptr, es));
  const WslSrc act = act_src(c, U.wblk.y2, U.wblk.st2, U.Co, H * W, nullptr, 1.f, nullptr);
  return wsl_src_materialize(&act, out, (int64_t)U.Co * H * W, d->N, H, W, stream);
}

extern "C" int wsl_upblock_t_backward(const WslUpBlockDesc* d, const float* params, const float* x1, const float* x2,
                                      const uint8_t* emask, const float* dout, float* grads, float* dx1, float* dx2, void* ws,
                                      size_t ws_bytes, void* stream) {
  UpPlan U;
  WSL_TRY(make_up_plan(d, U));
  WSL_REQUIRE(params && x1 && x2 && dout && grads && ws, "upblock_t_backward: null argument");
  WSL_TRY(check_ws("upblock_t_backward", ws_bytes, U.P.total_floats * sizeof(float)));
  const Plan& P = U.P;
  Ctx c{P, params, nullptr, nullptr, grads, static_cast<float*>(ws), stream, 1};
  WgBatch wb;
  wb.cap = P.wg_bytes;
  c.wb = &wb;
  const int H = P.H[0], W = P.W[0];
  const int64_t HW = (int64_t)H * W;
  const WslSrc skip = raw_src(x2, U.C2, U.C2 * HW);
  const WslSrc up = raw_src(c.ws + U.upt, U.C2, U.C2 * HW);
  const float es = d->dropout_p > 0.f ? 1.f / (1.f - d->dropout_p) : 1.f;
  float* dcat = c.ws + U.dcat;
  WSL_TRY(block_bwd(c, U.blk, U.wblk, &skip, &up, 0, d->dropout_p > 0.f ? emask : nullptr, es, dout, U.Co * HW, GStats{}, dcat));
  WSL_TRY(wgrad_flush(c.wb, c.stream));
  const float* dup = dcat + U.C2 * HW;
  WSL_TRY(wsl_convt2x2_wgrad(x1, dup, 2 * U.C2 * HW, grads + U.up.w, grads + U.up.b, d->N, U.C1, U.C2, U.h, U.w,
                             c.ws + c.S().wg_ws, P.wg_bytes, stream));
  if (dx1) WSL_TRY(wsl_convt2x2_dgrad(dup, 2 * U.C2 * HW, params + U.up.w, dx1, d->N, U.C1, U.C2, U.h, U.w, stream));
// ... 7 lines not shown
```

Before: 4112 slices/s.

## Fuse weight gradients into level-0 classifier dgrad and first-layer BN backward

New measurement: 4151 slices/s (median of 6 runs). Within noise of the previous version (+0.9%).

```diff
diff --git a/include/wsl_hip.h b/include/wsl_hip.h
--- a/include/wsl_hip.h
+++ b/include/wsl_hip.h
@@ -95,6 +95,12 @@
 int wsl_conv2d_dgrad_bn_d(const WslSrc* dy, const float* w, float* g, int64_t g_bs, int N, int H, int W, int Co, int ks,
                           int wmode, const float* bn_y, const float* bn_st, const uint8_t* bn_emask, float bn_emask_scale,
                           float* bn_part, int* fused, void* stream);
+int wsl_conv2d_dgrad_bn_wgrad_ok(const WslSrc* dy, const float* g, int64_t g_bs, int N, int H, int W, int Co, int ks, int wmode,
+                                 const float* bn_y, const uint8_t* bn_emask);
+size_t wsl_conv2d_dgrad_bn_wgrad_ws_bytes(int N, int H, int W);
+int wsl_conv2d_dgrad_bn_wgrad(const WslSrc* dy, const float* w, float* g, int64_t g_bs, int N, int H, int W, int Co, int ks, int wmode,
+                              const float* bn_y, const float* bn_st, const uint8_t* bn_emask, float bn_emask_scale, float* bn_part,
+                              int* fused, float* dw, float* db, void* ws, size_t ws_bytes, WslWgradPending* pending, void* stream);
 int wsl_bnact_bwd_finish_d_amax(const float* dz, int64_t dz_bs, const float* y, const float* mean, const float* invstd,
                                 const float* gamma, const float* beta, float* dy, float* dgamma, float* dbeta, int N, int C, int H,
                                 int W, const float* part, int nblk, int channel_major, void* ws, size_t ws_bytes, uint32_t* dy_amax,
@@ -131,6 +137,13 @@
                               float* dgamma, float* dbeta, int N, int C, int H, int W, const float* part, int nblk,
                               int channel_major, void* ws, size_t ws_bytes, uint32_t* dy_amax, void* stream);
 
+size_t wsl_bnact_bwd_finish_wgrad1_ws_bytes(int N, int C, int H, int W);
+int wsl_bnact_bwd_finish_wgrad1(const float* g, int64_t g_bs, int g_is_d, const float* y, const float* mean, const float* invstd,
+                                const float* gamma, const float* beta, const uint8_t* emask, float emask_scale, float* dy,
+                                float* dgamma, float* dbeta, int N, int C, int H, int W, const float* part, int nblk,
+                                int channel_major, void* ws, size_t ws_bytes, const float* x, int64_t x_bs, float* dw, float* db,
+                                void* wg_ws, size_t wg_ws_bytes, WslWgradPending* pending, void* stream);
+
 int wsl_bilinear_up2_fwd(const float* u, float* out, int64_t out_bs, int N, int C, int h, int w, void* stream);
 int wsl_bilinear_up2_bwd(const float* dout, int64_t dout_bs, float* du, int N, int C, int h, int w, void* stream);
 
diff --git a/wsl4mis_amd/_lib.py b/wsl4mis_amd/_lib.py
--- a/wsl4mis_amd/_lib.py
+++ b/wsl4mis_amd/_lib.py
@@ -102,6 +102,10 @@
     "wsl_bnact_bwd_ws_bytes": (sz, [i32, i32, i32, i32]),
     "wsl_conv2d_dgrad_bn": (i32, [PS, c_fp, c_fp, i64, i32, i32, i32, i32, i32, i32, c_fp, c_fp, c_fp, f32, c_fp, C.POINTER(C.c_int), c_fp]),
     "wsl_conv2d_dgrad_bn_d": (i32, [PS, c_fp, c_fp, i64, i32, i32, i32, i32, i32, i32, c_fp, c_fp, c_fp, f32, c_fp, C.POINTER(C.c_int), c_fp]),
+    "wsl_conv2d_dgrad_bn_wgrad_ok": (i32, [PS, c_fp, i64, i32, i32, i32, i32, i32, i32, c_fp, c_fp]),
+    "wsl_conv2d_dgrad_bn_wgrad_ws_bytes": (sz, [i32, i32, i32]),
+    "wsl_conv2d_dgrad_bn_wgrad": (i32, [PS, c_fp, c_fp, i64, i32, i32, i32, i32, i32, i32, c_fp, c_fp, c_fp, f32, c_fp, C.POINTER(C.c_int),
+                                        c_fp, c_fp, c_fp, sz, C.POINTER(WslWgradPending), c_fp]),
     "wsl_bnact_bwd_finish_d_amax": (i32, [c_fp, i64, c_fp, c_fp, c_fp, c_fp, c_fp, c_fp, c_fp, c_fp, i32, i32, i32, i32,
                                           c_fp, i32, i32, c_fp, sz, c_fp, c_fp]),
     "wsl_feat_grad_combine_blocks": (i32, [i32, i32, i32]),
@@ -127,6 +131,9 @@
                                  c_fp, sz, c_fp, c_fp]),
     "wsl_bnact_bwd_finish_amax": (i32, [c_fp, i64, c_fp, c_fp, c_fp, c_fp, c_fp, c_fp, f32, c_fp, c_fp, c_fp, i32, i32, i32, i32,
                                         c_fp, i32, i32, c_fp, sz, c_fp, c_fp]),
+    "wsl_bnact_bwd_finish_wgrad1_ws_bytes": (sz, [i32, i32, i32, i32]),
+    "wsl_bnact_bwd_finish_wgrad1": (i32, [c_fp, i64, i32, c_fp, c_fp, c_fp, c_fp, c_fp, c_fp, f32, c_fp, c_fp, c_fp, i32, i32, i32, i32,
+                                          c_fp, i32, i32, c_fp, sz, c_fp, i64, c_fp, c_fp, c_fp, sz, C.POINTER(WslWgradPending), c_fp]),
     "wsl_bilinear_up2_fwd": (i32, [c_fp, c_fp, i64, i32, i32, i32, i32, c_fp]),
     "wsl_bilinear_up2_bwd": (i32, [c_fp, i64, c_fp, i32, i32, i32, i32, c_fp]),
     "wsl_softmax_fwd": (i32, [c_fp, c_fp, i32, i32, i32, c_fp]),
@@ -221,6 +228,7 @@
     "wsl_debug_conv_plan": (i32, [i32, i32, i32]),
     "wsl_debug_conv_wino": (i32, [i32]),
     "wsl_debug_wgrad_workgroups": (i32, [i32]),
+    "wsl_debug_l0_fused": (i32, [i32]),
     "wsl_debug_net_decisions": (i32, [PD, c_fp, sz, i32, i32, c_fp, c_fp]),
     "wsl_debug_mfma4_probe": (i32, [c_fp, c_fp, c_fp, c_fp]),
     "wsl_debug_lds_dma_probe": (i32, [c_fp, c_fp, c_fp]),
diff --git a/wsl4mis_amd/csrc/wsl_bn.hip b/wsl4mis_amd/csrc/wsl_bn.hip
--- a/wsl4mis_amd/csrc/wsl_bn.hip
+++ b/wsl4mis_amd/csrc/wsl_bn.hip
@@ -392,6 +392,71 @@
     if (pmax) m = fmaxf(fmaxf(m, fmaxf(fabsf(v.x), fabsf(v.y))), fmaxf(fabsf(v.z), fabsf(v.w)));
   }
   if (pmax) amax_block_store(m, pmax);
+}
+
+constexpr int kWg1MaxW = 512;
+struct Wg1P {
+  const float* x;
+  int64_t x_bs;
+  float* part_dw;
+  float* part_db;
+  int W;
+};
+__global__ __launch_bounds__(256) void bnact_bwd_apply4_wgrad1_kernel(BnBwdP p, const float* coef, Wg1P q) {
+  __shared__ __attribute__((aligned(16))) float xs[kChunk + 2 * kWg1MaxW + 8];
+  __shared__ float red[10 * 4];
+  const int c = blockIdx.y, n = blockIdx.z, W = q.W;
+  const float mean = p.mean[c], invstd = p.invstd[c];
+  const float sc = p.gamma[c] * invstd, sh = fmaf(-mean, sc, p.beta[c]);
+  const float c1 = coef[2 * c], c2 = coef[2 * c + 1];
+  const int base = blockIdx.x * kChunk;
+  const int cnt = p.HW - base < kChunk ? p.HW - base : kChunk;
+  const int lo = base - W - 4;
+  const int nst = (cnt + 2 * W + 8) >> 2;
+  const float* xb = q.x + n * q.x_bs;
+  for (int e = threadIdx.x; e < nst; e += kThreads) {
+    const int f = lo + 4 * e;
+    float4 v = make_float4(0.f, 0.f, 0.f, 0.f);
+    if (f >= 0 && f < p.HW) v = *reinterpret_cast<const float4*>(xb + f);
+    *reinterpret_cast<float4*>(xs + 4 * e) = v;
+  }
+  __syncthreads();
+  float acc[10];
+#pragma unroll
+  for (int k = 0; k < 10; ++k) acc[k] = 0.f;
+  for (int i = base + 4 * threadIdx.x; i < base + cnt; i += 4 * kThreads) {
+    float d[4], xh[4];
+    bn_dz4(p, n, c, i, sc, sh, mean, invstd, d, xh);
+    const float v[4] = {sc * (d[0] - c1 - xh[0] * c2), sc * (d[1] - c1 - xh[1] * c2), sc * (d[2] - c1 - xh[2] * c2),
+                        sc * (d[3] - c1 - xh[3] * c2)};
+    const int col = i % W;
+    const bool first = col == 0, last = col + 4 == W;
+    const float* ctr = xs + (i - lo);
+#pragma unroll
+    for (int ky = 0; ky < 3; ++ky) {
+      const float* rr = ctr + (ky - 1) * W;
+      const float4 m = *reinterpret_cast<const float4*>(rr);
+      const float xr[6] = {first ? 0.f : rr[-1], m.x, m.y, m.z, m.w, last ? 0.f : rr[4]};
+#pragma unroll
+      for (int kx = 0; kx < 3; ++kx)
+#pragma unroll
+        for (int k = 0; k < 4; ++k) acc[ky * 3 + kx] = fmaf(v[k], xr[k + kx], acc[ky * 3 + kx]);
+    }
+    acc[9] += (v[0] + v[1]) + (v[2] + v[3]);
+  }
+#pragma unroll
+  for (int k = 0; k < 10; ++k) {
+    const float s = wave_sum(acc[k]);
+    if ((threadIdx.x & 63) == 0) red[k * 4 + (threadIdx.x >> 6)] = s;
+  }
+  __syncthreads();
+  if (threadIdx.x < 10) {
+    const float* r = red + 4 * threadIdx.x;
+    const float s = (r[0] + r[1]) + (r[2] + r[3]);
+    const int64_t split = (int64_t)n * gridDim.x + blockIdx.x;
+    if (threadIdx.x < 9) q.part_dw[(split * 9 + threadIdx.x) * p.C + c] = s;
+    else q.part_db[split * p.C + c] = s;
+  }
 }
 
 __global__ __launch_bounds__(1024) void bnact_bwd_finalize_kernel(const float* part, int nblk, int C, int64_t sb, int64_t sc,
@@ -828,6 +893,56 @@
                                    nblk, channel_major, ws, ws_bytes, nullptr, stream);
 }
 
+namespace wsl {
+bool bnact_wgrad1_ok(const float* g, int64_t g_bs, const float* y, const uint8_t* emask, const float* x, int64_t x_bs, int H, int W) {
+  auto al16 = [](const void* q) { return (reinterpret_cast<uintptr_t>(q) & 15) == 0; };
+  return H > 0 && W > 0 && W % 4 == 0 && W <= kWg1MaxW && (int64_t)H * W < (int64_t(1) << 30) && (g_bs % 4) == 0 && (x_bs % 4) == 0 &&
+         g && y && x && al16(g) && al16(y) && al16(x) && (!emask || (reinterpret_cast<uintptr_t>(emask) & 3) == 0);
+}
+}
+
+extern "C" size_t wsl_bnact_bwd_finish_wgrad1_ws_bytes(int N, int C, int H, int W) {
+  if (N <= 0 || C <= 0 || H <= 0 || W <= 0) return 0;
+  return sizeof(float) * (size_t)N * cdiv(H * W, kChunk) * 10 * (size_t)C;
+}
+
+extern "C" int wsl_bnact_bwd_finish_wgrad1(const float* g, int64_t g_bs, int g_is_d, const float* y, const float* mean, const float* invstd,
+                                           const float* gamma, const float* beta, const uint8_t* emask, float emask_scale, float* dy,
+                                           float* dgamma, float* dbeta, int N, int C, int H, int W, const float* part, int nblk,
+                                           int channel_major, void* ws, size_t ws_bytes, const float* x, int64_t x_bs, float* dw,
+                                           float* db, void* wg_ws, size_t wg_ws_bytes, WslWgradPending* pending, void* stream) {
+  (void)dy;
+  WSL_REQUIRE(g && y && mean && invstd && gamma && beta && ws && part && x && dw && db && wg_ws && pending,
+              "bnact_bwd_finish_wgrad1: null argument");
+  WSL_REQUIRE(N > 0 && C > 0 && H > 0 && W > 0 && nblk > 0, "bnact_bwd_finish_wgrad1: bad shape");
+  WSL_REQUIRE(!g_is_d || !emask, "bnact_bwd_finish_wgrad1: the d form carries no keep mask");
+  WSL_REQUIRE(bnact_wgrad1_ok(g, g_bs, y, emask, x, x_bs, H, W),
+              "bnact_bwd_finish_wgrad1: needs W %% 4 == 0, W <= %d and 16-byte aligned tensors", kWg1MaxW);
+  WSL_REQUIRE(x_bs >= (int64_t)H * W && g_bs >= (int64_t)C * H * W, "bnact_bwd_finish_wgrad1: batch stride too small");
+  if (ws_bytes < wsl_bnact_bwd_finish_ws_bytes(N, C, H, W, 0)) {
+    set_error("bnact_bwd_finish_wgrad1: workspace %zu < %zu", ws_bytes, wsl_bnact_bwd_finish_ws_bytes(N, C, H, W, 0));
+    return WSL_EWORKSPACE;
+  }
+  if (wg_ws_bytes < wsl_bnact_bwd_finish_wgrad1_ws_bytes(N, C, H, W)) {
+    set_error("bnact_bwd_finish_wgrad1: weight-gradient workspace %zu < %zu", wg_ws_bytes, wsl_bnact_bwd_finish_wgrad1_ws_bytes(N, C, H, W));
+    return WSL_EWORKSPACE;
+  }
+  BnBwdP p{g, g_bs, y, mean, invstd, gamma, beta, emask, emask_scale, C, H * W, cdiv(H * W, kChunk)};
+  p.g_is_d = g_is_d;
+  const double el = (double)N * C * H * W;
+  ProfScope ps(PF_BN_BWD, 20.0 * el, el * (8.0 + (emask && !g_is_d ? 1.0 : 0.0)) + 4.0 * N * H * W, stream);
+  float* coef = static_cast<float*>(ws);
+  const int nsplit = N * p.chunks;
+  Wg1P q{x, x_bs, static_cast<float*>(wg_ws), static_cast<float*>(wg_ws) + (size_t)nsplit * 9 * C, W};
+  WSL_LAUNCH(bnact_bwd_finalize_kernel, dim3(C), dim3(finalize_threads(nblk)), 0, stream, part, nblk, C,
+             channel_major ? (int64_t)1 : (int64_t)C, channel_major ? (int64_t)nblk : (int64_t)1, (double)N * H * W, dgamma, dbeta,
+             coef);
+  WSL_LAUNCH(bnact_bwd_apply4_wgrad1_kernel, dim3(p.chunks, C, N), dim3(kThreads), 0, stream, p, coef, q);
+  pending->part_dw = q.part_dw, pending->part_db = q.part_db, pending->dw = dw, pending->db = db;
+  pending->Co = C, pending->Ci = 1, pending->KK = 9, pending->nsplit = nsplit;
+  return check_launch("bnact_bwd_finish_wgrad1");
+}
+
 extern "C" int wsl_feat_grad_combine_blocks(int N, int H, int W) {
   return N > 0 && H > 0 && W > 0 ? N * cdiv(((H + 1) / 2) * ((W + 1) / 2), kChunk) : 0;
 }
diff --git a/wsl4mis_amd/csrc/wsl_conv.hip b/wsl4mis_amd/csrc/wsl_conv.hip
--- a/wsl4mis_amd/csrc/wsl_conv.hip
+++ b/wsl4mis_amd/csrc/wsl_conv.hip
@@ -537,6 +537,9 @@
                      float* stat_part, float* stat_cnt, int slots, const BnBwdEpi* bn, int* bn_done, void* stream);
 int conv_cls_launch(const WslSrc& a, const float* wp, const float* bias, float* y, int64_t y_bs, int N, int H, int W,
                     void* stream);
+int conv_nk16_wg_workgroups(int N, int H, int W);
+int conv_nk16_wg_launch(const WslSrc& a, const float* wp, float* y, int64_t y_bs, int N, int H, int W, const BnBwdEpi& bn, float* part_dw,
+                        float* part_db, int wgs, void* stream);
 int wino_pack(const float* w, float* u, int Co, int Ci, int dgrad, void* stream);
 int wino_fwd(const WslSrc& a, const WslSrc* b, const float* u, const float* bias, float* y, int64_t y_bs, int N, int H,
              int W, int Co, int is_dgrad, float* stat_part, float* stat_cnt, int slots, void* stream,
@@ -673,6 +676,49 @@
                                      int ks, int wmode, const float* bn_y, const float* bn_st, const uint8_t* bn_emask,
                                      float bn_emask_scale, float* bn_part, int* fused, void* stream) {
   return dgrad_bn_impl(dy, w, g, g_bs, N, H, W, Co, ks, wmode, bn_y, bn_st, bn_emask, bn_emask_scale, bn_part, fused, true, stream);
+}
+
+extern "C" int wsl_conv2d_dgrad_bn_wgrad_ok(const WslSrc* dy, const float* g, int64_t g_bs, int N, int H, int W, int Co, int ks, int wmode,
+                                            const float* bn_y, const uint8_t* bn_emask) {
+  if (!dy || !dy->x || !g || !bn_y || N <= 0 || H <= 0 || W <= 0 || ks != 3 || wmode != 3 || Co != 16 || dy->C != 4 || bn_emask) return 0;
+  if (!conv2_eligible(*dy, nullptr, g, g_bs, W, dy->C)) return 0;
+  const FwdPlan f = fwd_plan(N, H, W, Co, dy->C, ks);
+  if (!conv_nk16_eligible(*dy, nullptr, g, g_bs, H, W, Co, ks, f.th, f.tw)) return 0;
+  return g_bs == (int64_t)Co * H * W && (reinterpret_cast<uintptr_t>(bn_y) & 15) == 0 ? 1 : 0;
+}
+
+extern "C" size_t wsl_conv2d_dgrad_bn_wgrad_ws_bytes(int N, int H, int W) {
+  if (N <= 0 || H < 8 || W < 64) return 0;
+  return sizeof(float) * (size_t)conv_nk16_wg_workgroups(N, H, W) * (9 * 4 * 16 + 4);
+}
+
+extern "C" int wsl_conv2d_dgrad_bn_wgrad(const WslSrc* dy, const float* w, float* g, int64_t g_bs, int N, int H, int W, int Co, int ks,
+                                         int wmode, const float* bn_y, const float* bn_st, const uint8_t* bn_emask, float bn_emask_scale,
+                                         float* bn_part, int* fused, float* dw, float* db, void* ws, size_t ws_bytes,
+                                         WslWgradPending* pending, void* stream) {
+  if (fused) *fused = 0;
+  WSL_REQUIRE(dy && w && g && bn_y && bn_st && bn_part && fused && dw && db && ws && pending, "conv2d_dgrad_bn_wgrad: null argument");
+  if (!wsl_conv2d_dgrad_bn_wgrad_ok(dy, g, g_bs, N, H, W, Co, ks, wmode, bn_y, bn_emask)) {
+    set_error("conv2d_dgrad_bn_wgrad: not a shape of the fused launch (4 raw classes -> 16 channels, 3x3, packed data-gradient image, "
+              "H %% 8 == 0, W %% 64 == 0, no keep mask): take wsl_conv2d_wgrad_partial + wsl_conv2d_dgrad_bn_d");
+    return WSL_EUNSUPPORTED;
+  }
+  if (int rc = check_src(dy, H * W, "conv2d_dgrad_bn_wgrad(dy)")) return rc;
+  const size_t need = wsl_conv2d_dgrad_bn_wgrad_ws_bytes(N, H, W);
+  if (ws_bytes < need) {
+    set_error("conv2d_dgrad_bn_wgrad: workspace %zu < %zu", ws_bytes, need);
+    return WSL_EWORKSPACE;
+  }
+  BnBwdEpi e;
+  e.y = bn_y, e.st = bn_st, e.emask = nullptr, e.es = bn_emask_scale, e.part = bn_part, e.store_d = false;
+  const int wgs = conv_nk16_wg_workgroups(N, H, W);
+  float* part_dw = static_cast<float*>(ws);
+  float* part_db = part_dw + (size_t)wgs * 9 * 4 * 16;
+  if (int rc = conv_nk16_wg_launch(*dy, w, g, g_bs, N, H, W, e, part_dw, part_db, wgs, stream)) return rc;
+  *fused = 1;
+  pending->part_dw = part_dw, pending->part_db = part_db, pending->dw = dw, pending->db = db;
+  pending->Co = 4, pending->Ci = 16, pending->KK = 9, pending->nsplit = wgs;
+  return WSL_OK;
 }
 
 extern "C" size_t wsl_conv2d_wgrad_ws_bytes(int N, int H, int W, int Ci, int Co, int ks) {
diff --git a/wsl4mis_amd/csrc/wsl_conv4.hip b/wsl4mis_amd/csrc/wsl_conv4.hip
--- a/wsl4mis_amd/csrc/wsl_conv4.hip
+++ b/wsl4mis_amd/csrc/wsl_conv4.hip
@@ -395,6 +395,11 @@
   BnBwdEpi bn;
 };
 
+struct NkWgP : NkP {
+  float* part_dw;
+  float* part_db;
+};
+
 template <int CI, int TH_ = 8, int TW_ = 64>
 struct NkCfg {
   static constexpr int TH = TH_, TW = TW_, SEGW = TW / 16;
@@ -406,9 +411,10 @@
 };
 
 constexpr int kNk16MinW = 2;
-template <int CI, int TH = 8, int TW = 64, bool NHWC = false>
-__global__ __launch_bounds__(256, kNk16MinW) void conv_nk16_kernel(NkP p) {
+template <int CI, int TH = 8, int TW = 64, bool NHWC = false, bool WG = false>
+__global__ __launch_bounds__(256, kNk16MinW) void conv_nk16_kernel(std::conditional_t<WG, NkWgP, NkP> p) {
   using C = NkCfg<CI, TH, TW>;
+  static_assert(!WG || (CI == 4 && !NHWC), "the fused weight gradient is the classifier's (4 classes)");
   WSL_DYN_SMEM(smem);
   float* in_t = reinterpret_cast<float*>(smem);
   float* red = in_t + CI * C::PLANE;
@@ -434,6 +440,20 @@
   const int pty = tid / C::ROWP4, ptx4 = tid - pty * C::ROWP4;
   const bool owner = tid < C::POS;
   const int loff = pty * C::ROWP + ptx4 * 4;
+  int boff[3];
+  v4f accw[3];
+  float dbacc[4] = {0.f, 0.f, 0.f, 0.f};
+  const bool interior = pty >= 1 && pty <= C::TH && ptx4 >= 1 && ptx4 <= C::TW / 4;
+  if constexpr (WG) {
+#pragma unroll
+    for (int t = 0; t < 3; ++t) {
+      const int jj = t * 16 + c16;
+      const int tap = jj < 36 ? jj / 4 : 4, co = jj < 36 ? jj % 4 : 0;
+      const int ky = tap / 3, kx = tap - 3 * ky;
+      boff[t] = co * C::PLANE + (2 - ky) * C::ROWP + C::PADL + 1 - kx + 4 * k4;
+      accw[t] = v4f{0.f, 0.f, 0.f, 0.f};
+    }
+  }
   const int it0 = (int)((int64_t)blockIdx.x * p.items / gridDim.x), it1 = (int)((int64_t)(blockIdx.x + 1) * p.items / gridDim.x);
   float4 pre[CI];
   bool pok = false;
@@ -460,6 +480,12 @@
       for (int i = 0; i < CI; ++i)
         *reinterpret_cast<float4*>(in_t + i * C::PLANE + loff) = pok ? pre[i] : make_float4(0.f, 0.f, 0.f, 0.f);
     }
+    if constexpr (WG) {
+      if (interior) {
+#pragma unroll
+        for (int i = 0; i < CI; ++i) dbacc[i] += (pre[i].x + pre[i].y) + (pre[i].z + pre[i].w);
+      }
+    }
   };
 
   if (it0 < it1) issue(it0);
@@ -496,10 +522,25 @@
       const float mean = p.bn.st[c16], invstd = p.bn.st[16 + c16], sc = p.bn.st[32 + c16], sh = p.bn.st[48 + c16];
       const int64_t base = ((int64_t)n * 16 + c16) * HW + (int64_t)y0 * W + x0 + 4 * k4;
       BnBwdAcc ba;
+      if constexpr (WG) {
+#pragma unroll
+        for (int sg = 0; sg < 8; ++sg) {
+          const int srow = (8 * wave + sg) / C::SEGW, scol = 16 * ((8 * wave + sg) % C::SEGW);
+          const float4 yv = *reinterpret_cast<const float4*>(p.bn.y + base + srow * W + scol);
+          bn_bwd_acc4v(p.bn, yv, 0u, acc[sg][0], acc[sg][1], acc[sg][2], acc[sg][3], mean, invstd, sc, sh, ba);
+          const float av[4] = {leaky(fmaf(yv.x, sc, sh)), leaky(fmaf(yv.y, sc, sh)), leaky(fmaf(yv.z, sc, sh)), leaky(fmaf(yv.w, sc, sh))};
+          const float* bb = in_t + srow * C::ROWP + scol;
+#pragma unroll
+          for (int r = 0; r < 4; ++r)
+#pragma unroll
+            for (int t = 0; t < 3; ++t) accw[t] = WSL_MFMA16(av[r], bb[boff[t] + r], accw[t]);
+        }
+      } else {
 #pragma unroll
       for (int sg = 0; sg < 8; ++sg)
         bn_bwd_acc4(p.bn, base + ((8 * wave + sg) / C::SEGW) * W + 16 * ((8 * wave + sg) % C::SEGW), acc[sg][0], acc[sg][1], acc[sg][2], acc[sg][3], mean, invstd, sc,
                     sh, ba);
+      }
       float s1[1], s2[1];
       bn_bwd_fold(ba, s1[0], s2[0]);
       bn_bwd_store<1, 16>(p.bn, s1, s2, red, 0, 16, item, p.items);
@@ -535,6 +576,36 @@
       }
     }
     __syncthreads();
+  }
+  if constexpr (WG) {
+    static_assert(3 * 12 * 64 <= CI * C::PLANE, "merge area");
+    if (wave > 0) {
+#pragma unroll
+      for (int t = 0; t < 3; ++t)
+#pragma unroll
+        for (int r = 0; r < 4; ++r) in_t[((wave - 1) * 12 + t * 4 + r) * 64 + lane] = accw[t][r];
+    }
+#pragma unroll
+    for (int i = 0; i < 4; ++i) {
+      const float sdb = wave_sum(dbacc[i]);
+      if (lane == 0) red[wave * 4 + i] = sdb;
+    }
+    __syncthreads();
+    const int64_t split = blockIdx.x;
+    if (wave == 0) {
+#pragma unroll
+      for (int t = 0; t < 3; ++t) {
+        const int jj = t * 16 + c16;
+#pragma unroll
+        for (int r = 0; r < 4; ++r) {
+          float v = accw[t][r];
+#pragma unroll
+          for (int w = 0; w < 3; ++w) v += in_t[(w * 12 + t * 4 + r) * 64 + lane];
+          if (jj < 36) p.part_dw[((split * 9 + jj / 4) * 4 + jj % 4) * 16 + 4 * k4 + r] = v;
+        }
+      }
+      if (lane < 4) p.part_db[split * 4 + lane] = ((red[lane] + red[4 + lane]) + red[8 + lane]) + red[12 + lane];
+    }
   }
 }
 
@@ -586,6 +657,34 @@
   if (wide && W % 128 == 0) return a.C == 4 ? launch_nk16<4, 4, 128>(p, dgrad, stream) : launch_nk16<1, 4, 128>(p, dgrad, stream);
 #endif
   return a.C == 4 ? launch_nk16<4, 8, 64>(p, dgrad, stream) : launch_nk16<1, 8, 64>(p, dgrad, stream);
+}
+
+int conv_nk16_wg_workgroups(int N, int H, int W) {
+  int wgs = forced_wgrad_wgs() > 0 ? forced_wgrad_wgs() : kNk16MinW * device_cu_count();
+  const int64_t items = (int64_t)N * (H / 8) * (W / 64);
+  return items < wgs ? (int)items : wgs;
+}
+
+int conv_nk16_wg_launch(const WslSrc& a, const float* wp, float* y, int64_t y_bs, int N, int H, int W, const BnBwdEpi& bn, float* part_dw,
+                        float* part_db, int wgs, void* stream) {
+  using C = NkCfg<4, 8, 64>;
+  NkWgP p;
+  p.x = a.x, p.x_bs = a.bs, p.wp = wp, p.bias = nullptr, p.y = y, p.y_bs = y_bs;
+  p.N = N, p.H = H, p.W = W, p.tiles_x = W / 64, p.tiles_y = H / 8, p.items = N * p.tiles_x * p.tiles_y;
+  p.stat_part = nullptr, p.stat_cnt = nullptr, p.slots = 1;
+  p.bn = bn;
+  p.part_dw = part_dw, p.part_db = part_db;
+  auto kern = conv_nk16_kernel<4, 8, 64, false, true>;
+  static bool attr_done = false;
+  if (!attr_done) {
+    (void)WSL_SET_MAX_DYN_SMEM(kern, C::SMEM);
+    attr_done = true;
+  }
+  const double px = (double)N * H * W;
+  void* tok = prof_begin(PF_CONV_DGRAD, 2.0 * 2.0 * px * 4 * 16 * 9, 4.0 * px * (16 + 4) + bn_epi_bytes(p.bn, px * 16), stream);
+  WSL_LAUNCH(kern, dim3(wgs), dim3(kThreads), C::SMEM, stream, p);
+  prof_end(tok, stream);
+  return check_launch("conv_nk16_kernel(wgrad)");
 }
 
 #ifdef WSL_EXPERIMENTS
diff --git a/wsl4mis_amd/csrc/wsl_debug.h b/wsl4mis_amd/csrc/wsl_debug.h
--- a/wsl4mis_amd/csrc/wsl_debug.h
+++ b/wsl4mis_amd/csrc/wsl_debug.h
@@ -15,6 +15,7 @@
 int wsl_debug_conv_plan(int th, int tw, int co_t);
 int wsl_debug_conv_wino(int on);
 int wsl_debug_wgrad_workgroups(int n);
+int wsl_debug_l0_fused(int mask);
 
 int wsl_debug_mfma4_probe(const float* a, const float* b, float* d, void* stream);
 int wsl_debug_mfma_stream(int shape, int blocks, int iters, float* out, void* stream);
diff --git a/wsl4mis_amd/csrc/wsl_net.hip b/wsl4mis_amd/csrc/wsl_net.hip
--- a/wsl4mis_amd/csrc/wsl_net.hip
+++ b/wsl4mis_amd/csrc/wsl_net.hip
@@ -6,6 +6,16 @@
 
 int sp_pack_table(const PackTable& t, const int64_t* img_off_bytes, const float* params, void* imgf, void* imgd, uint32_t* amax,
                   int with_dgrad, void* stream);
+
+bool bnact_wgrad1_ok(const float* g, int64_t g_bs, const float* y, const uint8_t* emask, const float* x, int64_t x_bs, int H,
+                     int W);
+
+#ifdef WSL_EXPERIMENTS
+static std::atomic<int> g_l0_fused{3};
+static inline bool l0_fused_on(int bit) { return (g_l0_fused.load() & bit) != 0; }
+#else
+static constexpr bool l0_fused_on(int) { return true; }
+#endif
 
 static const int kFt[5] = {16, 32, 64, 128, 256};
 static const float kDrop[5] = {0.05f, 0.1f, 0.2f, 0.3f, 0.5f};
@@ -150,6 +160,12 @@
     plan_blkws(P.wenc[l], P.enc[l], l);
     P.pooled[l] = l ? B.take(N * kFt[l - 1] * P.H[l] * P.W[l], "pooled") : 0;
   }
+  if (d->in_chns == 1) {
+    size_t ms = max_stat, mc = max_cnt, nb;
+    const size_t plain = layer_need(P, P.enc[0].c1, 0, ms, mc, nb);
+    const size_t fused = (wsl_bnact_bwd_finish_wgrad1_ws_bytes(d->N, kFt[0], P.H[0], P.W[0]) + 255) & ~(size_t)255;
+    if (fused > plain) wg_enc += fused - plain;
+  }
   for (int k = 0; k < d->n_dec; ++k) {
     wg_dec = 0, wg_acc = &wg_dec;
     for (int i = 0; i < 4; ++i) {
@@ -162,7 +178,11 @@
       wg_add(wg_dec, wsl_conv2d_wgrad_ws_bytes(d->N, P.H[l + 1], P.W[l + 1], kFt[l + 1], c2, 1));
     }
     P.wdec[k].glow4 = B.take(N * kFt[4] * P.H[4] * P.W[4], "glow4");
-    wg_add(wg_dec, wsl_conv2d_wgrad_ws_bytes(d->N, P.H[0], P.W[0], kFt[0], d->n_class, 3));
+    {
+      const size_t plain = wsl_conv2d_wgrad_ws_bytes(d->N, P.H[0], P.W[0], kFt[0], d->n_class, 3);
+      const size_t fused = d->n_class == 4 ? wsl_conv2d_dgrad_bn_wgrad_ws_bytes(d->N, P.H[0], P.W[0]) : 0;
+      wg_add(wg_dec, fused > plain ? fused : plain);
+    }
   }
   P.wg_bytes = wg_enc > wg_dec ? wg_enc : wg_dec;
   const size_t big = N * kFt[0] * P.H[0] * P.W[0];
@@ -379,6 +399,18 @@
   WSL_TRY(wgrad_layer(c, &mid, nullptr, dy, CHW, c.grads + k.c2.w, c.grads + k.c2.b, H, W, C, 3, sp_dymax(c, k.b2)));
   GStats g1s;
   WSL_TRY(conv_dgrad_bn(c, k.c2, dy, g1, H, W, w.y1, w.st1, emask, es, &g1s, sp_dymax(c, k.b2)));
+  const uint8_t* em1 = g1s.g_is_d ? nullptr : emask;
+  if (l0_fused_on(2) && !dgrad_out && !b && a->C == 1 && !a->scale && !a->emask && !a->cmask && g1s.nblk &&
+      bnact_wgrad1_ok(g1, CHW, c.ws + w.y1, em1, a->x, a->bs, H, W)) {
+    const float* s = c.ws + w.st1;
+    const size_t need = (wsl_bnact_bwd_finish_wgrad1_ws_bytes(P.d.N, C, H, W) + 255) & ~(size_t)255;
+    return wgrad_push(c.wb, "net", c.ws + c.S().wg_ws, need, [&](void* ws, size_t n, WslWgradPending* q) {
+      return wsl_bnact_bwd_finish_wgrad1(g1, CHW, g1s.g_is_d, c.ws + w.y1, s, s + C, c.params + k.b1.gamma, c.params + k.b1.beta, em1, es,
+                                         nullptr, c.grads + k.b1.gamma, c.grads + k.b1.beta, P.d.N, C, H, W, c.ws + c.S().bn_ws, g1s.nblk,
+                                         g1s.channel_major, c.ws + c.S().bn_coef, P.bn_coef_bytes, a->x, a->bs, c.grads + k.c1.w,
+                                         c.grads + k.c1.b, ws, n, q, c.stream);
+    });
+  }
   WSL_TRY(bn_bwd(c, g1, CHW, w.y1, w.st1, k.b1, emask, es, dy, H, W, g1s));
   WSL_TRY(wgrad_layer(c, a, b, dy, CHW, c.grads + k.c1.w, c.grads + k.c1.b, H, W, C, 3, sp_dymax(c, k.b1), raw_amax));
   if (dgrad_out) {
@@ -422,9 +454,23 @@
   float* g = c.ws + c.S().tmp_g;
   const ConvRef& oc = P.dec[k].out;
   const WslSrc last = act_src(c, P.wdec[k].blk[3].y2, P.wdec[k].blk[3].st2, kFt[0], H0 * W0, nullptr, 1.f, nullptr);
-  WSL_TRY(wgrad_layer(c, &last, nullptr, dlogits, (int64_t)oc.Co * H0 * W0, c.grads + oc.w, c.grads + oc.b, H0, W0, oc.Co, 3));
   GStats gs;
-  WSL_TRY(conv_dgrad_bn(c, oc, dlogits, g, H0, W0, P.wdec[k].blk[3].y2, P.wdec[k].blk[3].st2, nullptr, 1.f, &gs));
+  const WslSrc dls = raw_src(dlogits, oc.Co, (int64_t)oc.Co * H0 * W0);
+  const int64_t g_bs0 = (int64_t)kFt[0] * H0 * W0;
+  if (l0_fused_on(1) && wsl_conv2d_fast_ok(&dls, nullptr, g, g_bs0, W0) && !wsl_conv2d_wino_ok(N, H0, W0, oc.Co, 0, kFt[0], 3) &&
+      wsl_conv2d_dgrad_bn_wgrad_ok(&dls, g, g_bs0, N, H0, W0, kFt[0], 3, 3, c.ws + P.wdec[k].blk[3].y2, nullptr)) {
+    const size_t need = (wsl_conv2d_dgrad_bn_wgrad_ws_bytes(N, H0, W0) + 255) & ~(size_t)255;
+    int fused = 0;
+    WSL_TRY(wgrad_push(c.wb, "net", c.ws + c.S().wg_ws, need, [&](void* ws, size_t n, WslWgradPending* q) {
+      return wsl_conv2d_dgrad_bn_wgrad(&dls, c.ws + c.P.packd + oc.w, g, g_bs0, N, H0, W0, kFt[0], 3, 3, c.ws + P.wdec[k].blk[3].y2,
+                                       c.ws + P.wdec[k].blk[3].st2, nullptr, 1.f, c.ws + c.S().bn_ws, &fused, c.grads + oc.w,
+                                       c.grads + oc.b, ws, n, q, c.stream);
+    }));
+    gs.nblk = wsl_conv2d_stat_blocks(N, H0, W0, oc.Co, kFt[0], 3), gs.channel_major = 1, gs.g_is_d = 0;
+  } else {
+    WSL_TRY(wgrad_layer(c, &last, nullptr, dlogits, (int64_t)oc.Co * H0 * W0, c.grads + oc.w, c.grads + oc.b, H0, W0, oc.Co, 3));
+    WSL_TRY(conv_dgrad_bn(c, oc, dlogits, g, H0, W0, P.wdec[k].blk[3].y2, P.wdec[k].blk[3].st2, nullptr, 1.f, &gs));
+  }
   for (int i = 3; i >= 0; --i) {
     const int l = 3 - i, c1 = kFt[l + 1], c2 = kFt[l];
     const int h = P.H[l + 1], w = P.W[l + 1], H = P.H[l], W = P.W[l];
@@ -633,6 +679,13 @@
   }
 }
 }
+
+#ifdef WSL_EXPERIMENTS
+extern "C" int wsl_debug_l0_fused(int mask) {
+  g_l0_fused = mask < 0 ? 3 : (mask & 3);
+  return WSL_OK;
+}
+#endif
 
 extern "C" int wsl_debug_net_ws_region(const WslNetDesc* d, int index, char* name, size_t name_len, size_t* off_floats, size_t* n_floats) {
   Plan P;
```
